# deadskull7/One-Stop-for-COVID-19-Infection-and-Lung-Segmentation-plus-Classification

Measured on AMD Instinct MI355X. Metric: CT images/sec (fwd+bwd) U-Net 512x512x1 bs16, higher is better.
Workload: dtype f32 storage / accumulate / parameters; conv products as a two-term fp16 split (3 fp16 MFMAs per multiply, ~2^-22 per product; --algo 2 = strict fp32); 1 GPU; U-Net infection seg (task1 graph T1:853-916), 512x512x1, batch 16/GPU, fp32, fwd+loss+bwd+Keras-Adam; BASELINE.json configs[1]; storage=fp32, global_batch=16, parallelism=dp1, deterministic=False, bn_fold=2

## Files before the change

### include/unet_hip.h

```cpp
#ifndef UNET_HIP_H
#define UNET_HIP_H
#include <stddef.h>
#include <stdint.h>

#ifdef __cplusplus
extern "C" {
#endif

#define UNET_ABI_VERSION 16

typedef struct unet_ctx unet_ctx;
typedef struct unet_model unet_model;
typedef uint16_t unet_bf16;
enum { UNET_DTYPE_F32 = 0, UNET_DTYPE_BF16 = 1 };

enum { UNET_OK = 0, UNET_E_ARG = -1, UNET_E_HIP = -2, UNET_E_SHAPE = -3, UNET_E_STATE = -4, UNET_E_NODEV = -5 };

enum { UNET_ALGO_AUTO = 0, UNET_ALGO_NAIVE = 1, UNET_ALGO_MFMA = 2 };

int32_t unet_abi_version(void);
int32_t unet_ctx_create(int32_t device_id, unet_ctx** out);
void unet_ctx_destroy(unet_ctx* ctx);
const char* unet_last_error(const unet_ctx* ctx);
int32_t unet_ctx_set_profiling(unet_ctx* ctx, int32_t on);
enum { UNET_OPT_RELU_BITS = 1, UNET_OPT_BN_FOLD = 2, UNET_OPT_ENC_BN_FUSED = 3, UNET_OPT_BN_CONCAT_ANALYTIC = 4, UNET_OPT_BN_FUSE_STATS = 5, UNET_OPT_DETERMINISTIC = 6,
       UNET_OPT_HEAD_FUSED = 7, UNET_OPT_SKIP_RAW = 8, UNET_OPT_POOL_SUMS_FUSED = 9, UNET_OPT_HEAD_BWD_FUSED = 10, UNET_OPT_CONV_PP = 13 };
int32_t unet_ctx_set_option(unet_ctx* ctx, int32_t option, int32_t value);
int32_t unet_ctx_get_option(unet_ctx* ctx, int32_t option);

enum { UNET_ACT_NONE = 0, UNET_ACT_RELU = 1, UNET_ACT_ELU = 2 };
enum { UNET_MASK_NONE = 0, UNET_MASK_RELU = 1, UNET_MASK_ELU = 2, UNET_MASK_ELU_DROP = 3, UNET_MASK_RELU_BITS = 9  };

size_t unet_conv3x3_w_ws_floats(int32_t cin, int32_t cout);
int32_t unet_conv3x3_pick_algo(int32_t algo, int32_t wd, int32_t cin, int32_t cout);
double unet_conv3x3_exec_ratio(int32_t algo, int32_t h, int32_t wd, int32_t cin, int32_t cout);
double unet_conv3x3_wgrad_exec_ratio(int32_t algo, int32_t h, int32_t wd, int32_t cin, int32_t cout);
int32_t unet_request_bn_stats(unet_ctx*, int32_t c);
int32_t unet_relu_bits_supported(int32_t algo, int32_t h, int32_t wd, int32_t cin, int32_t cout);
size_t unet_relu_bits_bytes(int32_t n, int32_t h, int32_t wd, int32_t c);
int32_t unet_request_relu_bits(unet_ctx*, void* bits);
int32_t unet_allow_k_slices(unet_ctx*);
int32_t unet_ctx_max_kernel_scratch_bytes(unet_ctx*);
int32_t unet_conv3x3_fwd(unet_ctx*, const float* x, const float* w, const float* bias, float* y,
                         int32_t n, int32_t h, int32_t wd, int32_t cin, int32_t cout,
                         int32_t act, float drop_rate, uint64_t drop_seed, int32_t algo, float* w_ws, void* stream);
int32_t unet_conv3x3_fwd_ld(unet_ctx*, const float* x, const float* w, const float* bias, float* y, int32_t ldy,
                            int32_t n, int32_t h, int32_t wd, int32_t cin, int32_t cout, int32_t act, int32_t algo, float* w_ws, void* stream);
int32_t unet_conv3x3_bwd_data(unet_ctx*, const float* dy, const float* w, const float* mask_src,
                              int32_t mask_mode, float mask_rate, uint64_t mask_seed,
                              float* dx, float* wt_ws, int32_t n, int32_t h, int32_t wd,
                              int32_t cin, int32_t cout, int32_t algo, void* stream);
int32_t unet_conv3x3_bnfold_supported(int32_t algo, int32_t h, int32_t wd, int32_t cin, int32_t cout);
size_t unet_conv3x3_bnfold_ws_floats(int32_t n, int32_t cin, int32_t cout);
int32_t unet_conv3x3_bnfold_fwd(unet_ctx*, const float* x, const float* bnp, const float* w, const float* bias, float* y, int32_t n, int32_t h,
                                int32_t wd, int32_t cin, int32_t cout, int32_t act, int32_t algo, float* ws, void* stream);
int32_t unet_conv3x3_bnfold_bwd_weights(unet_ctx*, const float* x, const float* bnp, const float* dy, const float* w, float* dw, float* db,
                                        double* bn_bwd_sums, void* gws, size_t gws_bytes, float* ws, int32_t n, int32_t h, int32_t wd,
                                        int32_t cin, int32_t cout, int32_t algo, void* stream);
size_t unet_conv3x3_bwd_weights_ws_bytes(int32_t n, int32_t h, int32_t wd, int32_t cin, int32_t cout);
int32_t unet_conv3x3_bwd_weights(unet_ctx*, const float* x, const float* dy, float* dw, float* db,
                                 void* ws, size_t ws_bytes, int32_t n, int32_t h, int32_t wd,
                                 int32_t cin, int32_t cout, int32_t algo, void* stream);

int32_t unet_convT2x2_fwd(unet_ctx*, const float* x, const float* w, const float* bias, float* y,
                          int32_t ldy, int32_t n, int32_t h, int32_t wd, int32_t cin, int32_t cout,
                          int32_t algo, void* stream);
int32_t unet_convT2x2_bwd_data(unet_ctx*, const float* dy, int32_t lddy, const float* w,
                               const float* relu_src, float* dx, int32_t n, int32_t h, int32_t wd,
                               int32_t cin, int32_t cout, int32_t algo, void* stream);
size_t unet_convT2x2_bwd_weights_ws_bytes(int32_t n, int32_t h, int32_t wd, int32_t cin, int32_t cout);
int32_t unet_convT2x2_bwd_weights(unet_ctx*, const float* x, const float* dy, int32_t lddy,
                                  float* dw, float* db, void* ws, size_t ws_bytes, int32_t n,
                                  int32_t h, int32_t wd, int32_t cin, int32_t cout, int32_t algo,
                                  void* stream);

int32_t unet_bn_stats(unet_ctx*, const float* x, int32_t ldx, double* sums, int64_t pixels,
                      int32_t c, void* stream);
int32_t unet_bn_stats_concat(unet_ctx*, const float* x_up, int32_t ldx, const double* src_sums, double src_count, const float* src_gamma,
                             const float* src_beta, double* sums, int64_t pixels, int32_t c_up, int32_t c_skip, void* stream);
int32_t unet_bn_finalize_train(unet_ctx*, const double* sums, double count, const float* gamma,
                               const float* beta, float* moving_mean, float* moving_var,
                               float* bnp, int32_t c, void* stream);
int32_t unet_bn_finalize_infer(unet_ctx*, const float* gamma, const float* beta,
                               const float* moving_mean, const float* moving_var, float* bnp,
                               int32_t c, void* stream);
int32_t unet_bn_apply(unet_ctx*, const float* x, int32_t ldx, const float* bnp, float* y,
                      int32_t ldy, int64_t pixels, int32_t c, void* stream);
int32_t unet_bn_bwd_stats(unet_ctx*, const float* dy, int32_t lddy, const float* x, int32_t ldx,
                          const float* bnp, double* sums, int64_t pixels, int32_t c, void* stream);
int32_t unet_bn_bwd_param_grads(unet_ctx*, const double* sums, float* dgamma, float* dbeta,
                                int32_t c, void* stream);
int32_t unet_bn_bwd_apply(unet_ctx*, const float* dy, int32_t lddy, const float* x, int32_t ldx,
                          const float* bnp, const double* sums, double count, int32_t mask_mode,
                          float mask_rate, uint64_t mask_seed, float* dx, int32_t lddx, int64_t pixels,
                          int32_t c, void* stream);

int32_t unet_maxpool2x2_dropout_fwd(unet_ctx*, const float* x, int32_t ldx, float* y, int32_t n,
                                    int32_t h, int32_t wd, int32_t c, float rate, uint64_t seed,
                                    void* stream);
int32_t unet_maxpool2x2_dropout_bwd(unet_ctx*, const float* x, int32_t ldx, const float* dy,
                                    float* dx, int32_t lddx, int32_t n, int32_t h, int32_t wd,
                                    int32_t c, float rate, uint64_t seed, int32_t accumulate,
                                    void* stream);

int32_t unet_bn_apply_maxpool_dropout_fwd(unet_ctx*, const float* x, int32_t ldx, const float* bnp, float* y,
                                          int32_t ldy, float* pooled, int32_t n, int32_t h, int32_t wd,
                                          int32_t c, float rate, uint64_t seed, void* stream);
int32_t unet_maxpool2x2_dropout_bwd_bnstats(unet_ctx*, const float* y, int32_t ldy, const float* dy, float* dx,
                                            int32_t lddx, const float* gamma, const float* beta, double* sums,
                                            int32_t n, int32_t h, int32_t wd, int32_t c, float rate,
                                            uint64_t seed, void* stream);
int32_t unet_maxpool2x2_dropout_bwd_sums(unet_ctx*, const float* pooled, const float* dy_pooled, const float* gamma, const float* beta, double* sums,
                                         int32_t n, int32_t h, int32_t wd, int32_t c, float rate, uint64_t seed, void* stream);
int32_t unet_bn_bwd_skip_term(unet_ctx*, double* sums, const double* dec_sum_dyxhat, const float* dec_invstd, const float* dec_gamma,
                              const float* gamma, int32_t c, double frac, void* stream);
int32_t unet_bn_maxpool_bwd_apply(unet_ctx*, const float* x, int32_t ldx, const float* bnp, const double* sums, double count, const float* g_skip,
                                  int32_t ldg, const float* dy_pooled, float* dx, int32_t lddx, int32_t n, int32_t h, int32_t wd, int32_t c,
                                  float rate, uint64_t seed, void* stream);

enum { UNET_LOSS_BCE_DICE = 0, UNET_LOSS_BCE = 1, UNET_LOSS_DICE = 2, UNET_LOSS_TVERSKY = 3, UNET_LOSS_WEIGHTED_BCE_DICE = 4 };
int32_t unet_loss_weight_map(unet_ctx*, const float* y_true, float* weight, int32_t n, int32_t h, int32_t wd, void* stream);
int32_t unet_head_fwd_ex(unet_ctx*, const float* x, const float* w, const float* bias, float* p, const float* y_true, const float* weight_map, double* loss_sums,
                         int64_t pixels, int32_t cin, void* stream);
int32_t unet_head_fwd_bf16_ex(unet_ctx*, const unet_bf16* x, const float* w, const float* bias, float* p, const float* y_true, const float* weight_map,
                              double* loss_sums, int64_t pixels, int32_t cin, void* stream);

int32_t unet_head_fwd(unet_ctx*, const float* x, const float* w, const float* bias, float* p,
                      const float* y_true, double* loss_sums, int64_t pixels, int32_t cin,
                      void* stream);
int32_t unet_loss_finalize(unet_ctx*, const double* loss_sums, double count, float* loss_out,
                           void* stream);
int32_t unet_head_bwd(unet_ctx*, const float* x, const float* w, const float* p, const float* y_true,
                      const double* loss_sums, double count, float* dx, float* dw, float* db,
                      int64_t pixels, int32_t cin, int32_t relu_mask, void* stream);
int32_t unet_loss_finalize_ex(unet_ctx*, const double* loss_sums, double count, int32_t loss, float alpha, float beta, float* loss_out, void* stream);
int32_t unet_head_bwd_ex(unet_ctx*, const float* x, const float* w, const float* p, const float* y_true, const double* loss_sums, double count,
                         int32_t loss, float alpha, float beta, const float* weight_map, float* dx, float* dw, float* db, int64_t pixels, int32_t cin, int32_t relu_mask,
                         void* stream);

int32_t unet_conv3x3_bwd_data_pool_sums_supported(unet_ctx*, int32_t algo, int32_t wd, int32_t cin, int32_t cout);
int32_t unet_conv3x3_bwd_data_pool_sums(unet_ctx*, const float* dy, const float* w, const float* pooled, const float* gamma, const float* beta, float rate,
                                        float* dx, double* sums, float* wt_ws, int32_t n, int32_t h, int32_t wd, int32_t cin, int32_t cout, void* stream);

int32_t unet_conv3x3_head_supported(unet_ctx*, int32_t algo, int32_t w, int32_t cin, int32_t cout);
int32_t unet_conv3x3_head_fwd(unet_ctx*, const float* x, const float* w, const float* bias, float* y, const float* w_head, const float* b_head, float* p,
                              const float* y_true, double* loss_sums, double* head_sums, int32_t n, int32_t h, int32_t wd, int32_t cin, float* w_ws, void* stream);
int32_t unet_head_dy(unet_ctx*, const float* p, const float* y_true, const double* loss_sums, double count, const double* head_sums, const float* w_head,
                     const void* relu_bits, const float* y, float* dy, float* dw_head, float* db_head, int32_t n, int32_t h, int32_t wd, void* stream);
int32_t unet_head_bwd_stream_supported(unet_ctx*, int32_t algo, int32_t wd, int32_t cin);
int32_t unet_head_dzm(unet_ctx*, const float* p, const float* y_true, const double* loss_sums, double count, const double* head_sums, const void* relu_bits, void* dzm,
                      float* dw_head, float* db_head, int32_t n, int32_t h, int32_t wd, void* stream);
int32_t unet_conv3x3_head_fwd_ex(unet_ctx*, const float* x, const float* w, const float* bias, float* y, const float* w_head, const float* b_head, float* p,
                                 const float* y_true, const float* weight_map, double* loss_sums, double* head_sums, int32_t n, int32_t h, int32_t wd, int32_t cin,
                                 float* w_ws, void* stream);
int32_t unet_head_dy_ex(unet_ctx*, const float* p, const float* y_true, const double* loss_sums, double count, const double* head_sums, int32_t loss, float alpha,
                        float beta, const float* weight_map, const float* w_head, const void* relu_bits, const float* y, float* dy, float* dw_head, float* db_head, int32_t n, int32_t h,
                        int32_t wd, void* stream);
int32_t unet_head_dzm_ex(unet_ctx*, const float* p, const float* y_true, const double* loss_sums, double count, const double* head_sums, int32_t loss, float alpha,
                         float beta, const float* weight_map, const void* relu_bits, void* dzm, float* dw_head, float* db_head, int32_t n, int32_t h, int32_t wd, void* stream);
int32_t unet_conv3x3_bwd_data_dzm(unet_ctx*, const void* dzm, const float* w, const float* w_head, const void* relu_bits_in, float* dx, float* wt_ws, int32_t n, int32_t h,
                                  int32_t wd, int32_t cin, void* stream);
int32_t unet_conv3x3_bwd_weights_dzm(unet_ctx*, const float* x, const void* dzm, const float* w_head, float* dw, float* db, void* ws, size_t ws_bytes, int32_t n, int32_t h,
                                     int32_t wd, int32_t cin, void* stream);

int32_t unet_adam_keras(unet_ctx*, float* p, const float* g, float* m, float* v, int64_t count,
                        float lr_t, float b1, float b2, float eps, float grad_scale, void* stream);

int32_t unet_seg_metrics_sweep(unet_ctx*, const float* p, const float* gt, const float* thresholds,
                               int32_t nthr, double* out, int64_t count, void* stream);

int32_t unet_gather_samples(unet_ctx*, const float* src, const int64_t* idx, float* dst, int64_t n,
                            int64_t sample_floats, void* stream);

int32_t unet_augment_samples(unet_ctx*, const float* src_img, const float* src_mask, const int64_t* idx, const float* mats, float* dst_img, float* dst_mask,
                             int64_t n, int32_t h, int32_t w, int32_t c, void* stream);

enum { UNET_FEAT_OUT_F32 = 0, UNET_FEAT_OUT_F64 = 1 };
int32_t unet_feat_col_mean(unet_ctx*, const float* x, int64_t ldx, int64_t n, int64_t d, double* mu, void* stream);
size_t unet_feat_gemm_nt_workspace(int64_t m, int64_t p, int64_t d, int32_t sym);
int32_t unet_feat_gemm_nt(unet_ctx*, const float* a, int64_t lda, const double* mu_a, const float* b, int64_t ldb, const double* mu_b, int64_t m,
                          int64_t p, int64_t d, int32_t sym, void* c, int64_t ldc, int32_t c_dtype, void* ws, size_t ws_bytes, void* stream);
size_t unet_feat_gemm_tn_workspace(int64_t k, int64_t d, int64_t n);
int32_t unet_feat_gemm_tn(unet_ctx*, const float* w, int64_t ldw, const float* x, int64_t ldx, const double* mu, int64_t n, int64_t k, int64_t d,
                          void* out, int64_t ldo, int32_t out_dtype, void* ws, size_t ws_bytes, void* stream);
int32_t unet_kmeans_step(unet_ctx*, const float* pts, int64_t ldp, int64_t n, int64_t p, const double* centres, int32_t k, int32_t* labels,
                         double* dist, double* sums, int64_t* counts, double* inertia, void* stream);
size_t unet_cluster_route_workspace(int64_t n, int64_t d, int32_t k);
int32_t unet_cluster_route(unet_ctx*, const void* tap, int32_t tap_bf16, int64_t n, int32_t h, int32_t w, int32_t c, int64_t ld,
                           const float* comps_hwc, const float* mu_hwc, int32_t k, const double* centres, int32_t nc,
                           float* proj, int32_t* labels, double* dist, void* ws, size_t ws_bytes, void* stream);

int32_t unet_zero(unet_ctx*, void* ptr, size_t bytes, void* stream);
int32_t unet_copy_slice(unet_ctx*, const float* src, int32_t lds, float* dst, int32_t ldd, int64_t pixels, int32_t c, void* stream);
int32_t unet_accum_slices(unet_ctx*, const float* const* srcs, const int32_t* lds, int32_t nsrc, float* dst, int32_t ldd,
                          int64_t pixels, int32_t c, int32_t accumulate, void* stream);

int32_t unet_cast_f32_to_bf16(unet_ctx*, const float* src, unet_bf16* dst, int64_t count, void* stream);
int32_t unet_cast_bf16_to_f32(unet_ctx*, const unet_bf16* src, float* dst, int64_t count, void* stream);
int32_t unet_conv3x3_fwd_bf16(unet_ctx*, const unet_bf16* x, const float* w, const float* bias, unet_bf16* y, int32_t n, int32_t h, int32_t wd,
                              int32_t cin, int32_t cout, int32_t act, float drop_rate, uint64_t drop_seed, void* w_ws, void* stream);
int32_t unet_conv3x3_first_fwd_bf16(unet_ctx*, const float* x, const float* w, const float* bias, unet_bf16* y, int32_t n, int32_t h,
                                    int32_t wd, int32_t cout, int32_t act, float drop_rate, uint64_t drop_seed, void* stream);
int32_t unet_conv3x3_bwd_data_bf16(unet_ctx*, const unet_bf16* dy, const float* w, const unet_bf16* mask_src, int32_t mask_mode, float mask_rate,
                                   uint64_t mask_seed, unet_bf16* dx, void* w_ws, int32_t n, int32_t h, int32_t wd, int32_t cin, int32_t cout,
                                   void* stream);
size_t unet_conv3x3_bwd_weights_ws_bytes_bf16(int32_t n, int32_t h, int32_t wd, int32_t cin, int32_t cout);
int32_t unet_conv3x3_bwd_weights_bf16(unet_ctx*, const unet_bf16* x, const unet_bf16* dy, float* dw, float* db, void* ws, size_t ws_bytes,
                                      int32_t n, int32_t h, int32_t wd, int32_t cin, int32_t cout, void* stream);
int32_t unet_conv3x3_first_bwd_weights_bf16(unet_ctx*, const float* x, const unet_bf16* dy, float* dw, float* db, void* ws, size_t ws_bytes,
                                            int32_t n, int32_t h, int32_t wd, int32_t cout, void* stream);
int32_t unet_convT2x2_fwd_bf16(unet_ctx*, const unet_bf16* x, const float* w, const float* bias, unet_bf16* y, int32_t ldy, int32_t n, int32_t h,
                               int32_t wd, int32_t cin, int32_t cout, void* w_ws, void* stream);
int32_t unet_convT2x2_bwd_data_bf16(unet_ctx*, const unet_bf16* dy, int32_t lddy, const float* w, const unet_bf16* relu_src, unet_bf16* dx,
                                    int32_t n, int32_t h, int32_t wd, int32_t cin, int32_t cout, void* w_ws, void* stream);
size_t unet_convT2x2_bwd_weights_ws_bytes_bf16(int32_t n, int32_t h, int32_t wd, int32_t cin, int32_t cout);
int32_t unet_convT2x2_bwd_weights_bf16(unet_ctx*, const unet_bf16* x, const unet_bf16* dy, int32_t lddy, float* dw, float* db, void* ws,
                                       size_t ws_bytes, int32_t n, int32_t h, int32_t wd, int32_t cin, int32_t cout, void* stream);
int32_t unet_bn_stats_bf16(unet_ctx*, const unet_bf16* x, int32_t ldx, double* sums, int64_t pixels, int32_t c, void* stream);
int32_t unet_bn_stats_concat_bf16(unet_ctx*, const unet_bf16* x_up, int32_t ldx, const double* src_sums, double src_count, const float* src_gamma,
                                  const float* src_beta, double* sums, int64_t pixels, int32_t c_up, int32_t c_skip, void* stream);
int32_t unet_bn_apply_bf16(unet_ctx*, const unet_bf16* x, int32_t ldx, const float* bnp, unet_bf16* y, int32_t ldy, int64_t pixels, int32_t c,
                           void* stream);
int32_t unet_bn_bwd_stats_bf16(unet_ctx*, const unet_bf16* dy, int32_t lddy, const unet_bf16* x, int32_t ldx, const float* bnp, double* sums,
                               int64_t pixels, int32_t c, void* stream);
int32_t unet_bn_bwd_apply_bf16(unet_ctx*, const unet_bf16* dy, int32_t lddy, const unet_bf16* x, int32_t ldx, const float* bnp, const double* sums,
// ... 191 lines not shown
```

### one-stop-for-covid-19-infection-and-lung-segmentation-plus-classification_amd/_lib.py

```python
from __future__ import annotations

import ctypes as C
import os

_HERE = os.path.dirname(os.path.abspath(__file__))
LIB_PATH = os.environ.get("COVIDSEG_AMD_LIB") or os.path.join(_HERE, "libunet_hip.so")
ABI_VERSION = 16
COMM_HANDLE_BYTES, COMM_MAX_WORLD, COMM_MAX_DOUBLES = 64, 8, 2048

ALGO_AUTO, ALGO_NAIVE, ALGO_MFMA = 0, 1, 2
OPTIONS = {"relu_bits": 1, "bn_fold": 2, "enc_bn_fused": 3, "bn_concat_analytic": 4, "bn_fuse_stats": 5, "deterministic": 6, "head_fused": 7, "skip_raw": 8, "pool_sums_fused": 9, "head_bwd_fused": 10, "conv_pp": 13}
ARCH_UNET, ARCH_UNETPP, ARCH_CLASSIFIER = 0, 1, 2
LOSSES = {"bce_dice_loss": 0, "binary_crossentropy": 1, "dice_loss": 2, "tversky_loss": 3, "weighted_bce_dice_loss": 4}
DTYPE_F32, DTYPE_BF16 = 0, 1
ACT_NONE, ACT_RELU, ACT_ELU = 0, 1, 2
MORPH_OPS = {"dilate": 0, "erode": 1, "open": 2, "close": 3}
MORPH_MAX_ITERATIONS = 64
INTENSITY_MAX_EDGES = 63
MASK_NONE, MASK_RELU, MASK_ELU, MASK_ELU_DROP = 0, 1, 2, 3
PROG_FWD_TRAIN, PROG_BWD, PROG_FWD_INFER = 0, 1, 2
SYNC_BN_FWD, SYNC_LOSS, SYNC_BN_BWD, SYNC_GRAD_BUCKET = 0, 1, 2, 3

f32p = C.POINTER(C.c_float)
f64p = C.POINTER(C.c_double)
vp = C.c_void_p
i32, i64, u64, f32, f64, sz = C.c_int32, C.c_int64, C.c_uint64, C.c_float, C.c_double, C.c_size_t


class SyncPoint(C.Structure):
    _fields_ = [("after_op", i32), ("kind", i32), ("ptr", vp), ("count", i64), ("use_op", i32), ("reserved", i32)]


RENDER_MAX_TILES, RENDER_MAX_LAYERS = 64, 4


class RenderTile(C.Structure):
    _fields_ = [("axis", i32), ("index", i32), ("x0", i32), ("y0", i32), ("w", i32), ("h", i32)]


class RenderLayer(C.Structure):
    _fields_ = [("labels", vp), ("palette", vp), ("dtype", i32), ("palette_size", i32), ("fill_alpha", i32), ("outline_alpha", i32)]


_PROTOS = {
    "unet_abi_version": (i32, []),
    "unet_ctx_create": (i32, [i32, C.POINTER(vp)]),
    "unet_ctx_destroy": (None, [vp]),
    "unet_last_error": (C.c_char_p, [vp]),
    "unet_ctx_set_profiling": (i32, [vp, i32]),
    "unet_ctx_set_option": (i32, [vp, i32, i32]),
    "unet_ctx_get_option": (i32, [vp, i32]),
    "unet_conv3x3_w_ws_floats": (sz, [i32, i32]),
    "unet_conv3x3_pick_algo": (i32, [i32, i32, i32, i32]),
    "unet_conv3x3_exec_ratio": (f64, [i32, i32, i32, i32, i32]),
    "unet_conv3x3_wgrad_exec_ratio": (f64, [i32, i32, i32, i32, i32]),
    "unet_request_bn_stats": (i32, [vp, i32]),
    "unet_relu_bits_supported": (i32, [i32, i32, i32, i32, i32]),
    "unet_relu_bits_bytes": (sz, [i32, i32, i32, i32]),
    "unet_request_relu_bits": (i32, [vp, vp]),
    "unet_allow_k_slices": (i32, [vp]),
    "unet_ctx_max_kernel_scratch_bytes": (i32, [vp]),
    "unet_conv3x3_fwd": (i32, [vp, vp, vp, vp, vp, i32, i32, i32, i32, i32, i32, f32, u64, i32, vp, vp]),
    "unet_conv3x3_fwd_ld": (i32, [vp, vp, vp, vp, vp, i32, i32, i32, i32, i32, i32, i32, i32, vp, vp]),
    "unet_conv3x3_bwd_data": (i32, [vp, vp, vp, vp, i32, f32, u64, vp, vp, i32, i32, i32, i32, i32, i32, vp]),
    "unet_conv3x3_bwd_weights_ws_bytes": (sz, [i32, i32, i32, i32, i32]),
    "unet_conv3x3_bwd_weights": (i32, [vp, vp, vp, vp, vp, vp, sz, i32, i32, i32, i32, i32, i32, vp]),
    "unet_convT2x2_fwd": (i32, [vp, vp, vp, vp, vp, i32, i32, i32, i32, i32, i32, i32, vp]),
    "unet_convT2x2_bwd_data": (i32, [vp, vp, i32, vp, vp, vp, i32, i32, i32, i32, i32, i32, vp]),
    "unet_convT2x2_bwd_weights_ws_bytes": (sz, [i32, i32, i32, i32, i32]),
    "unet_convT2x2_bwd_weights": (i32, [vp, vp, vp, i32, vp, vp, vp, sz, i32, i32, i32, i32, i32, i32, vp]),
    "unet_cast_f32_to_bf16": (i32, [vp, vp, vp, i64, vp]),
    "unet_cast_bf16_to_f32": (i32, [vp, vp, vp, i64, vp]),
    "unet_conv3x3_fwd_bf16": (i32, [vp, vp, vp, vp, vp, i32, i32, i32, i32, i32, i32, f32, u64, vp, vp]),
    "unet_conv3x3_first_fwd_bf16": (i32, [vp, vp, vp, vp, vp, i32, i32, i32, i32, i32, f32, u64, vp]),
    "unet_conv3x3_bwd_data_bf16": (i32, [vp, vp, vp, vp, i32, f32, u64, vp, vp, i32, i32, i32, i32, i32, vp]),
    "unet_conv3x3_bwd_weights_ws_bytes_bf16": (sz, [i32, i32, i32, i32, i32]),
    "unet_conv3x3_bwd_weights_bf16": (i32, [vp, vp, vp, vp, vp, vp, sz, i32, i32, i32, i32, i32, vp]),
    "unet_conv3x3_first_bwd_weights_bf16": (i32, [vp, vp, vp, vp, vp, vp, sz, i32, i32, i32, i32, vp]),
    "unet_convT2x2_fwd_bf16": (i32, [vp, vp, vp, vp, vp, i32, i32, i32, i32, i32, i32, vp, vp]),
    "unet_convT2x2_bwd_data_bf16": (i32, [vp, vp, i32, vp, vp, vp, i32, i32, i32, i32, i32, vp, vp]),
    "unet_convT2x2_bwd_weights_ws_bytes_bf16": (sz, [i32, i32, i32, i32, i32]),
    "unet_convT2x2_bwd_weights_bf16": (i32, [vp, vp, vp, i32, vp, vp, vp, sz, i32, i32, i32, i32, i32, vp]),
    "unet_bn_stats": (i32, [vp, vp, i32, vp, i64, i32, vp]),
    "unet_bn_stats_bf16": (i32, [vp, vp, i32, vp, i64, i32, vp]),
    "unet_conv3x3_bnfold_supported": (i32, [i32, i32, i32, i32, i32]),
    "unet_conv3x3_bnfold_ws_floats": (sz, [i32, i32, i32]),
    "unet_conv3x3_bnfold_fwd": (i32, [vp, vp, vp, vp, vp, vp, i32, i32, i32, i32, i32, i32, i32, vp, vp]),
    "unet_conv3x3_bnfold_bwd_weights": (i32, [vp, vp, vp, vp, vp, vp, vp, vp, vp, sz, vp, i32, i32, i32, i32, i32, i32, vp]),
    "unet_bn_stats_concat": (i32, [vp, vp, i32, vp, f64, vp, vp, vp, i64, i32, i32, vp]),
    "unet_bn_stats_concat_bf16": (i32, [vp, vp, i32, vp, f64, vp, vp, vp, i64, i32, i32, vp]),
    "unet_bn_finalize_train": (i32, [vp, vp, f64, vp, vp, vp, vp, vp, i32, vp]),
    "unet_bn_finalize_infer": (i32, [vp, vp, vp, vp, vp, vp, i32, vp]),
    "unet_bn_apply": (i32, [vp, vp, i32, vp, vp, i32, i64, i32, vp]),
    "unet_bn_apply_bf16": (i32, [vp, vp, i32, vp, vp, i32, i64, i32, vp]),
    "unet_bn_bwd_stats": (i32, [vp, vp, i32, vp, i32, vp, vp, i64, i32, vp]),
    "unet_bn_bwd_stats_bf16": (i32, [vp, vp, i32, vp, i32, vp, vp, i64, i32, vp]),
    "unet_bn_bwd_param_grads": (i32, [vp, vp, vp, vp, i32, vp]),
    "unet_bn_bwd_apply": (i32, [vp, vp, i32, vp, i32, vp, vp, f64, i32, f32, u64, vp, i32, i64, i32, vp]),
    "unet_bn_bwd_apply_bf16": (i32, [vp, vp, i32, vp, i32, vp, vp, f64, i32, f32, u64, vp, i32, i64, i32, vp]),
    "unet_maxpool2x2_dropout_fwd": (i32, [vp, vp, i32, vp, i32, i32, i32, i32, f32, u64, vp]),
    "unet_maxpool2x2_dropout_fwd_bf16": (i32, [vp, vp, i32, vp, i32, i32, i32, i32, f32, u64, vp]),
    "unet_maxpool2x2_dropout_bwd": (i32, [vp, vp, i32, vp, vp, i32, i32, i32, i32, i32, f32, u64, i32, vp]),
    "unet_maxpool2x2_dropout_bwd_bf16": (i32, [vp, vp, i32, vp, vp, i32, i32, i32, i32, i32, f32, u64, i32, vp]),
    "unet_bn_apply_maxpool_dropout_fwd": (i32, [vp, vp, i32, vp, vp, i32, vp, i32, i32, i32, i32, f32, u64, vp]),
    "unet_bn_apply_maxpool_dropout_fwd_bf16": (i32, [vp, vp, i32, vp, vp, i32, vp, i32, i32, i32, i32, f32, u64, vp]),
    "unet_maxpool2x2_dropout_bwd_bnstats": (i32, [vp, vp, i32, vp, vp, i32, vp, vp, vp, i32, i32, i32, i32, f32, u64, vp]),
    "unet_maxpool2x2_dropout_bwd_sums": (i32, [vp, vp, vp, vp, vp, vp, i32, i32, i32, i32, f32, u64, vp]),
    "unet_maxpool2x2_dropout_bwd_sums_bf16": (i32, [vp, vp, vp, vp, vp, vp, i32, i32, i32, i32, f32, u64, vp]),
    "unet_bn_maxpool_bwd_apply_bf16": (i32, [vp, vp, i32, vp, vp, f64, vp, i32, vp, vp, i32, i32, i32, i32, i32, f32, u64, vp]),
    "unet_bn_bwd_skip_term": (i32, [vp, vp, vp, vp, vp, vp, i32, f64, vp]),
    "unet_bn_maxpool_bwd_apply": (i32, [vp, vp, i32, vp, vp, f64, vp, i32, vp, vp, i32, i32, i32, i32, i32, f32, u64, vp]),
    "unet_maxpool2x2_dropout_bwd_bnstats_bf16": (i32, [vp, vp, i32, vp, vp, i32, vp, vp, vp, i32, i32, i32, i32, f32, u64, vp]),
    "unet_head_fwd": (i32, [vp, vp, vp, vp, vp, vp, vp, i64, i32, vp]),
    "unet_head_fwd_bf16": (i32, [vp, vp, vp, vp, vp, vp, vp, i64, i32, vp]),
    "unet_loss_finalize": (i32, [vp, vp, f64, vp, vp]),
    "unet_head_bwd": (i32, [vp, vp, vp, vp, vp, vp, f64, vp, vp, vp, i64, i32, i32, vp]),
    "unet_head_bwd_bf16": (i32, [vp, vp, vp, vp, vp, vp, f64, vp, vp, vp, i64, i32, i32, vp]),
    "unet_loss_finalize_ex": (i32, [vp, vp, f64, i32, f32, f32, vp, vp]),
    "unet_head_bwd_ex": (i32, [vp, vp, vp, vp, vp, vp, f64, i32, f32, f32, vp, vp, vp, vp, i64, i32, i32, vp]),
    "unet_head_bwd_bf16_ex": (i32, [vp, vp, vp, vp, vp, vp, f64, i32, f32, f32, vp, vp, vp, vp, i64, i32, i32, vp]),
    "unet_head_fwd_ex": (i32, [vp, vp, vp, vp, vp, vp, vp, vp, i64, i32, vp]),
    "unet_head_fwd_bf16_ex": (i32, [vp, vp, vp, vp, vp, vp, vp, vp, i64, i32, vp]),
    "unet_loss_weight_map": (i32, [vp, vp, vp, i32, i32, i32, vp]),
    "unet_conv3x3_head_fwd_ex": (i32, [vp, vp, vp, vp, vp, vp, vp, vp, vp, vp, vp, vp, i32, i32, i32, i32, vp, vp]),
    "unet_adam_keras": (i32, [vp, vp, vp, vp, vp, i64, f32, f32, f32, f32, f32, vp]),
    "unet_seg_metrics_sweep": (i32, [vp, vp, vp, vp, i32, vp, i64, vp]),
    "unet_gather_samples": (i32, [vp, vp, vp, vp, i64, i64, vp]),
    "unet_augment_samples": (i32, [vp, vp, vp, vp, vp, vp, vp, i64, i32, i32, i32, vp]),
    "unet_feat_col_mean": (i32, [vp, vp, i64, i64, i64, vp, vp]),
    "unet_feat_gemm_nt_workspace": (sz, [i64, i64, i64, i32]),
    "unet_feat_gemm_nt": (i32, [vp, vp, i64, vp, vp, i64, vp, i64, i64, i64, i32, vp, i64, i32, vp, sz, vp]),
    "unet_feat_gemm_tn_workspace": (sz, [i64, i64, i64]),
    "unet_feat_gemm_tn": (i32, [vp, vp, i64, vp, i64, vp, i64, i64, i64, vp, i64, i32, vp, sz, vp]),
    "unet_kmeans_step": (i32, [vp, vp, i64, i64, i64, vp, i32, vp, vp, vp, vp, vp, vp]),
    "unet_cluster_route_workspace": (sz, [i64, i64, i32]),
    "unet_cluster_route": (i32, [vp, vp, i32, i64, i32, i32, i32, i64, vp, vp, i32, vp, i32, vp, vp, vp, vp, sz, vp]),
    "unet_conv3x3_head_supported": (i32, [vp, i32, i32, i32, i32]),
    "unet_conv3x3_head_fwd": (i32, [vp, vp, vp, vp, vp, vp, vp, vp, vp, vp, vp, i32, i32, i32, i32, vp, vp]),
    "unet_conv3x3_bwd_data_pool_sums_supported": (i32, [vp, i32, i32, i32, i32]),
    "unet_conv3x3_bwd_data_pool_sums": (i32, [vp, vp, vp, vp, vp, vp, f32, vp, vp, vp, i32, i32, i32, i32, i32, vp]),
    "unet_head_dy": (i32, [vp, vp, vp, vp, f64, vp, vp, vp, vp, vp, vp, vp, i32, i32, i32, vp]),
    "unet_head_bwd_stream_supported": (i32, [vp, i32, i32, i32]),
    "unet_head_dzm": (i32, [vp, vp, vp, vp, f64, vp, vp, vp, vp, vp, i32, i32, i32, vp]),
    "unet_head_dy_ex": (i32, [vp, vp, vp, vp, f64, vp, i32, f32, f32, vp, vp, vp, vp, vp, vp, vp, i32, i32, i32, vp]),
    "unet_head_dzm_ex": (i32, [vp, vp, vp, vp, f64, vp, i32, f32, f32, vp, vp, vp, vp, vp, i32, i32, i32, vp]),
    "unet_conv3x3_bwd_data_dzm": (i32, [vp, vp, vp, vp, vp, vp, vp, i32, i32, i32, i32, vp]),
    "unet_conv3x3_bwd_weights_dzm": (i32, [vp, vp, vp, vp, vp, vp, vp, sz, i32, i32, i32, i32, vp]),
    "unet_zero": (i32, [vp, vp, sz, vp]),
    "unet_comm_create": (i32, [vp, i32, i32, vp, vp]),
    "unet_comm_connect": (i32, [vp, vp]),
    "unet_comm_set_timeout_ms": (i32, [vp, i32]),
    "unet_comm_allreduce_f64": (i32, [vp, vp, i32, vp]),
    "unet_comm_status": (i32, [vp, vp, vp]),
    "unet_comm_destroy": (None, [vp]),
    "unet_copy_slice": (i32, [vp, vp, i32, vp, i32, i64, i32, vp]),
    "unet_copy_slice_bf16": (i32, [vp, vp, i32, vp, i32, i64, i32, vp]),
    "unet_accum_slices": (i32, [vp, C.POINTER(vp), C.POINTER(i32), i32, vp, i32, i64, i32, i32, vp]),
    "unet_accum_slices_bf16": (i32, [vp, C.POINTER(vp), C.POINTER(i32), i32, vp, i32, i64, i32, i32, vp]),
    "unet_dense_ws_bytes": (sz, [i32, i32, i32]),
    "unet_dense_fwd": (i32, [vp, vp, vp, vp, vp, i32, i32, i32, i32, f32, u64, vp, sz, vp]),
    "unet_dense_fwd_bf16": (i32, [vp, vp, vp, vp, vp, i32, i32, i32, i32, f32, u64, vp, sz, vp]),
    "unet_dense_bwd": (i32, [vp, vp, vp, vp, vp, vp, i32, i32, i32, vp]),
    "unet_dense_bwd_bf16": (i32, [vp, vp, vp, vp, vp, vp, i32, i32, i32, vp]),
    "unet_cls_head_fwd": (i32, [vp, vp, vp, vp, vp, vp, f32, f32, vp, i32, i32, vp]),
    "unet_cls_loss_finalize": (i32, [vp, vp, f64, vp, vp]),
    "unet_cls_head_bwd": (i32, [vp, vp, vp, vp, vp, f32, f32, f64, f32, vp, vp, vp, vp, i32, i32, vp]),
    "unet_pre_minmax_ws_bytes": (sz, [i32]),
    "unet_pre_minmax_to_u8": (i32, [vp, vp, vp, i32, i64, vp, sz, vp]),
    "unet_pre_unit_to_u8": (i32, [vp, vp, vp, i64, vp]),
    "unet_pre_u8_to_unit": (i32, [vp, vp, vp, i64, vp]),
    "unet_pre_clahe_ws_bytes": (sz, [i32, i32, i32]),
    "unet_pre_clahe_u8": (i32, [vp, vp, vp, i32, i32, i32, f32, i32, i32, vp, sz, vp]),
    "unet_pre_resize_u8": (i32, [vp, vp, i32, i32, i32, vp, vp, i32, i32, i32, i32, i32, vp]),
    "unet_pre_contours_u8": (i32, [vp, vp, i32, i32, i32, i32, vp, vp, vp, i32]),
    "unet_vol_slices_ws_bytes": (sz, [i32, i32]),
    "unet_vol_slices_f64": (i32, [vp, vp, i32, i32, i32, i32, i32, f64, f64, i32, i32, i32, vp, vp, vp, vp, vp, vp, sz, vp]),
    "unet_vol_paste_back": (i32, [vp, vp, i32, i32, vp, vp, i32, vp]),
    "unet_vol_unslice": (i32, [vp, vp, i32, f32, i32, i32, i32, i32, i32, vp, vp, vp]),
    "unet_vol_label_ws_bytes": (sz, [i32, i32, i32]),
    "unet_vol_label": (i32, [vp, vp, i32, i32, i32, i32, vp, vp, vp, sz, vp]),
    "unet_vol_component_stats": (i32, [vp, vp, i32, i32, i32, i32, vp, vp]),
    "unet_vol_filter_components": (i32, [vp, vp, vp, i32, i32, i32, i32, i32, i32, vp, vp, vp]),
    "unet_vol_confusion": (i32, [vp, vp, vp, i32, i32, i32, vp, vp]),
    "unet_vol_surface": (i32, [vp, vp, i32, i32, i32, i32, vp, vp, vp]),
    "unet_vol_edt_ws_bytes": (sz, [i32, i32, i32]),
    "unet_vol_edt_sq": (i32, [vp, vp, i32, i32, i32, i32, vp, vp, vp, sz, vp]),
    "unet_vol_sqrt_f64": (i32, [vp, vp, i64, vp]),
    "unet_vol_surface_distances": (i32, [vp, vp, vp, i32, i32, i32, vp, vp, i64, vp, sz, vp]),
    "unet_vol_lesion_overlap": (i32, [vp, vp, i32, vp, i32, i32, i32, i32, vp, vp, vp]),
    "unet_vol_label_planar": (i32, [vp, vp, i32, i32, i32, i32, vp, vp, vp, sz, vp]),
    "unet_vol_morph_ws_bytes": (sz, [i32, i32, i32]),
    "unet_vol_morph": (i32, [vp, vp, i32, i32, i32, i32, i32, i32, i32, i32, vp, vp, vp, sz, vp]),
    "unet_vol_ball": (i32, [vp, vp, i32, i32, i32, f64, i32, vp, vp, vp]),
    "unet_vol_fill_holes_ws_bytes": (sz, [i32, i32, i32]),
    "unet_vol_fill_holes": (i32, [vp, vp, i32, i32, i32, i32, i32, vp, vp, vp, sz, vp]),
    "unet_vol_dihedral": (i32, [vp, vp, i32, i32, i32, vp, vp]),
    "unet_vol_canvas_axpy": (i32, [vp, vp, f32, vp, i64, i32, vp]),
    "unet_vol_canvas_div": (i32, [vp, vp, f32, i64, vp]),
    "unet_vol_unslice_prob": (i32, [vp, vp, i32, i32, i32, i32, i32, i32, vp, vp]),
    "unet_vol_vote_pack": (i32, [vp, vp, i32, i32, vp, i64, vp]),
    "unet_vol_vote_reduce": (i32, [vp, vp, i32, i32, i32, i32, i32, vp, vp, vp, vp, vp, vp, vp]),
    "unet_vol_intensity_bands": (i32, [vp, vp, i32, i32, i32, i32, i32, f64, f64, vp, vp, i32, vp, vp, i32, vp, vp, vp, vp]),
    "unet_vol_intensity_gather": (i32, [vp, vp, i32, i32, i32, i32, i32, f64, f64, vp, vp, i32, vp, vp, vp, i64, vp, vp]),
    "unet_vol_group_moments_ws_bytes": (sz, [i64, i32]),
    "unet_vol_group_moments": (i32, [vp, vp, vp, i32, vp, vp, sz, vp]),
    "unet_vol_side_assign": (i32, [vp, vp, vp, vp, i32, i32, i32, i32, i32, vp, vp, vp]),
    "unet_vol_side_table": (i32, [vp, vp, vp, vp, i32, i32, i32, i32, vp, vp, vp, vp]),
    "unet_vol_project": (i32, [vp, vp, i32, i32, i32, i32, i32, f64, f64, i32, i32, i32, i32, vp, vp, vp, i32, vp, vp]),
    "unet_vol_render": (i32, [vp, vp, i32, i32, i32, i32, i32, f64, f64, vp, f64, f64, vp, i32, i32, i32, vp, i32, vp, i32, vp, i32, i32, vp]),
    "unet_vol_resample_nearest": (i32, [vp, vp, i32, i32, i32, i32, vp, i32, u64, vp, i32, i32, i32, vp]),
    "unet_vol_resample_linear": (i32, [vp, vp, i32, i32, i32, i32, i32, f64, f64, vp, i32, f64, vp, i32, i32, i32, i32, vp]),
    "unet_model_create": (i32, [vp, i32, i32, i32, i32, i32, i32, i32, i32, C.POINTER(vp)]),
    "unet_model_dtype": (i32, [vp]),
    "unet_model_tap_elem_bytes": (i32, [vp, C.c_char_p, i32]),
    "unet_model_destroy": (None, [vp]),
    "unet_model_set_loss_out": (C.c_int32, [vp, vp]),
    "unet_model_param_count": (i64, [vp]),
    "unet_model_state_count": (i64, [vp]),
    "unet_model_workspace_bytes": (sz, [vp, i32]),
    "unet_model_tensor_info": (i32, [vp, C.c_char_p, C.POINTER(i32), C.POINTER(i64), C.POINTER(i64)]),
    "unet_model_bind": (i32, [vp, vp, vp, vp, vp, vp, vp, sz]),
    "unet_model_set_io": (i32, [vp, vp, vp, vp]),
    "unet_model_set_dropout": (i32, [vp, f32, u64]),
    "unet_model_set_class_weights": (i32, [vp, f32, f32]),
    "unet_model_set_loss": (i32, [vp, i32, f32, f32]),
    "unet_model_num_ops": (i32, [vp, i32]),
    "unet_model_sync_points": (i32, [vp, i32, C.POINTER(SyncPoint), i32]),
    "unet_model_run": (i32, [vp, i32, i32, i32, vp]),
# ... 92 lines not shown
```

### one-stop-for-covid-19-infection-and-lung-segmentation-plus-classification_amd/csrc/common.h

```cpp
#pragma once
#include <hip/hip_runtime.h>
#include <stdint.h>
#include <stdio.h>
#include <set>
#include <string>

#include "../../include/unet_hip.h"

constexpr int UNET_BN_SLOTS = 64, UNET_BN_SLOTS_DET = 1024, UNET_BN_SLOT_DOUBLES = 2048;
struct unet_loss_sel { int32_t kind = UNET_LOSS_BCE_DICE; float alpha = 0.5f, beta = 0.5f; };
inline bool unet_loss_sel_ok(const unet_loss_sel& ls, const float* wm = nullptr, bool need_map = true) {
  if (ls.kind < UNET_LOSS_BCE_DICE || ls.kind > UNET_LOSS_WEIGHTED_BCE_DICE) return false;
  if (ls.kind == UNET_LOSS_TVERSKY && !(ls.alpha > 0.0f && ls.beta > 0.0f && ls.alpha < 1e30f && ls.beta < 1e30f)) return false;
  return !need_map || (ls.kind == UNET_LOSS_WEIGHTED_BCE_DICE) == (wm != nullptr);
}
constexpr int UNET_HEAD_SUMS = 100;
struct unet_ctx {
  int device = 0;
  int num_cu = 256;
  int profiling = 0;
  int opt_relu_bits = 1;
  int opt_bn_fold = 2;
  int opt_enc_bn_fused = 1;
  int opt_bn_concat_analytic = 1;
  int opt_bn_fuse_stats = 1;
  int opt_pool_sums_fused = 1;
  int opt_skip_raw = 1;
  int opt_head_fused = 1;
  int opt_head_bwd_fused = 1;
  int opt_conv_pp = 1;
  int opt_deterministic = 0;
  double* bn_slots = nullptr;
  int bn_nslots() const { return opt_deterministic ? UNET_BN_SLOTS_DET : UNET_BN_SLOTS; }
  void* convt_img = nullptr;
  size_t convt_img_bytes = 0;
  int k_slices_ok = 0;
  void* splitk_ws = nullptr;
  size_t splitk_ws_bytes = 0;
  int stats_req_c = 0;
  const void* stats_in_slots = nullptr;
  int stats_in_slots_c = 0;
  bool stats_in_slots_xs = false;
  unsigned long long* signs_req = nullptr;
  const void* signs_done = nullptr;
  std::set<const void*> big_lds_kernels;
  std::set<const void*> noted_kernels;
  int max_scratch_bytes = 0;
  std::string err;
};

#define UNET_FAIL(ctx, code, ...)                         \
  do {                                                    \
    char _b[512];                                         \
    snprintf(_b, sizeof(_b), __VA_ARGS__);                \
    if (ctx) (ctx)->err = _b;                             \
    return (code);                                        \
  } while (0)

#define UNET_CHECK_LAUNCH(ctx, what)                                              \
  do {                                                                            \
    hipError_t _e = hipGetLastError();                                            \
    if (_e != hipSuccess) UNET_FAIL(ctx, UNET_E_HIP, "%s: %s", what, hipGetErrorString(_e)); \
  } while (0)

#define UNET_HIP(ctx, expr)                                                       \
  do {                                                                            \
    hipError_t _e = (expr);                                                       \
    if (_e != hipSuccess) UNET_FAIL(ctx, UNET_E_HIP, "%s: %s", #expr, hipGetErrorString(_e)); \
  } while (0)

static inline int32_t unet_big_lds(unet_ctx* ctx, const void* kernel, size_t bytes, const char* what) {
  if (ctx->big_lds_kernels.count(kernel)) return UNET_OK;
  if (hipFuncSetAttribute(kernel, hipFuncAttributeMaxDynamicSharedMemorySize, (int)bytes) != hipSuccess) UNET_FAIL(ctx, UNET_E_HIP, "%s: cannot reserve %zu bytes of LDS", what, bytes);
  ctx->big_lds_kernels.insert(kernel);
  return UNET_OK;
}
static inline void unet_note_kernel(unet_ctx* ctx, const void* kernel) {
  if (ctx->noted_kernels.count(kernel)) return;
  ctx->noted_kernels.insert(kernel);
  hipFuncAttributes at;
  if (hipFuncGetAttributes(&at, kernel) == hipSuccess && (int)at.localSizeBytes > ctx->max_scratch_bytes) ctx->max_scratch_bytes = (int)at.localSizeBytes;
}
#define UNET_BIG_LDS(ctx, kern, bytes, what) do { int32_t _r = unet_big_lds(ctx, reinterpret_cast<const void*>(kern), bytes, what); if (_r) return _r; } while (0)

static inline hipStream_t as_stream(void* s) { return reinterpret_cast<hipStream_t>(s); }
static inline int64_t cdiv64(int64_t a, int64_t b) { return (a + b - 1) / b; }

__device__ __forceinline__ float wave_sum(float v) {
#pragma unroll
  for (int o = 32; o > 0; o >>= 1) v += __shfl_xor(v, o, 64);
  return v;
}

constexpr int UNET_XW = 4;
__device__ __forceinline__ void xsum_add(double* row, int idx, float t) {
  unsigned long long* acc = reinterpret_cast<unsigned long long*>(row) + (size_t)UNET_XW * idx;
  const int eb = (int)((__float_as_uint(t) >> 23) & 0xFF);
  if (eb == 0) return;
  const int e = eb - 127;
  if (e >= 60) { atomicMax(reinterpret_cast<long long*>(acc + 3), 1LL << 62); return; }
  if (e >= 39) {
    atomicAdd(acc + 3, (unsigned long long)__double2ll_rd((double)t * (1.0 / 65536.0)));
    return;
  }
  const int w = min(max((e - 23 + 80) >> 5, 0), 2);
  const double sc = __longlong_as_double((long long)(1023 + 80 - 32 * w) << 52);
  const long long q = __double2ll_rd((double)t * sc);
  atomicAdd(acc + w, (unsigned long long)(q & 0xFFFFFFFFll));
  atomicAdd(acc + w + 1, (unsigned long long)(q >> 32));
}
__device__ __forceinline__ double xsum_take(double* slots, int idx, int nslots) {
  long long S0 = 0, S1 = 0, S2 = 0, S3 = 0; bool bad = false;
// ... 60 lines not shown
__device__ __forceinline__ __amdgpu_buffer_rsrc_t make_rsrc(const float* base, long long bytes) {
  return __builtin_amdgcn_make_buffer_rsrc(const_cast<float*>(base), 0, (int)bytes, 0x00020000);
}

typedef __bf16 unet_bf16x8 __attribute__((ext_vector_type(8)));
typedef __bf16 unet_bf16x2 __attribute__((ext_vector_type(2)));
typedef float unet_f32x2 __attribute__((ext_vector_type(2)));
typedef float unet_f32x16 __attribute__((ext_vector_type(16)));
__device__ __forceinline__ unsigned pack_bf16x2(float lo, float hi) {
  return __builtin_bit_cast(unsigned, __builtin_convertvector((unet_f32x2){lo, hi}, unet_bf16x2));
}
__device__ __forceinline__ float bf16_lo(unsigned u) { return __uint_as_float(u << 16); }
__device__ __forceinline__ float bf16_hi(unsigned u) { return __uint_as_float(u & 0xFFFF0000u); }
__device__ __forceinline__ float4 ld4(const float* p) { return *reinterpret_cast<const float4*>(p); }
__device__ __forceinline__ void st4(float* p, float4 v) { *reinterpret_cast<float4*>(p) = v; }
__device__ __forceinline__ float4 ld4(const unet_bf16* p) {
  const uint2 u = *reinterpret_cast<const uint2*>(p);
  return make_float4(bf16_lo(u.x), bf16_hi(u.x), bf16_lo(u.y), bf16_hi(u.y));
}
__device__ __forceinline__ void st4(unet_bf16* p, float4 v) { *reinterpret_cast<uint2*>(p) = make_uint2(pack_bf16x2(v.x, v.y), pack_bf16x2(v.z, v.w)); }
__device__ __forceinline__ float ld1(const float* p) { return *p; }
__device__ __forceinline__ float ld1(const unet_bf16* p) { return __uint_as_float((unsigned)*p << 16); }
__device__ __forceinline__ void st1(float* p, float v) { *p = v; }
__device__ __forceinline__ void st1(unet_bf16* p, float v) { *p = (unet_bf16)(pack_bf16x2(v, 0.f) & 0xFFFFu); }

__device__ __forceinline__ uint4 philox4x32(uint64_t ctr, uint64_t seed) {
  uint32_t c0 = (uint32_t)ctr, c1 = (uint32_t)(ctr >> 32), c2 = 0x243F6A88u, c3 = 0x85A308D3u;
  uint32_t k0 = (uint32_t)seed, k1 = (uint32_t)(seed >> 32);
#pragma unroll
  for (int r = 0; r < 10; ++r) {
    uint32_t hi0 = __umulhi(0xD2511F53u, c0), lo0 = 0xD2511F53u * c0;
    uint32_t hi1 = __umulhi(0xCD9E8D57u, c2), lo1 = 0xCD9E8D57u * c2;
    uint32_t n0 = hi1 ^ c1 ^ k0, n1 = lo1, n2 = hi0 ^ c3 ^ k1, n3 = lo0;
    c0 = n0; c1 = n1; c2 = n2; c3 = n3;
    k0 += 0x9E3779B9u; k1 += 0xBB67AE85u;
  }
  return make_uint4(c0, c1, c2, c3);
}
__device__ __forceinline__ float u32_to_unit(uint32_t u) { return (float)(u >> 8) * (1.0f / 16777216.0f); }

__device__ __forceinline__ float4 keep_scale(long long quad_idx, float rate, uint64_t seed) {
  uint4 r = philox4x32((uint64_t)quad_idx, seed);
  float s = 1.0f / (1.0f - rate);
  return make_float4(u32_to_unit(r.x) >= rate ? s : 0.f, u32_to_unit(r.y) >= rate ? s : 0.f,
                     u32_to_unit(r.z) >= rate ? s : 0.f, u32_to_unit(r.w) >= rate ? s : 0.f);
}

enum { ACT_NONE = 0, ACT_RELU = 1, ACT_ELU = 2 };
__device__ __forceinline__ float apply_act(float v, int act) {
  if (act == ACT_RELU) return fmaxf(v, 0.0f);
  if (act == ACT_ELU) return v > 0.0f ? v : expm1f(v);
  return v;
}
enum { MASK_NONE = 0, MASK_RELU = 1, MASK_ELU = 2, MASK_ELU_DROP = 3 };
enum { MASK_BIAS_TAB = 4 };
enum { MASK_BN_BWD = 5 };
enum { MASK_BN_BWD_ELU = 6, MASK_BN_BWD_ELU_DROP = 7 };
enum { MASK_BN_BWD_RELU = 8 };
enum { MASK_RELU_BITS = 9 };
enum { MASK_POOL_SUMS = 10 };
int32_t k_bn_bwd_coef(unet_ctx*, const float* bnp, const double* sums, double count, float* coef, int c, hipStream_t s);
__device__ __forceinline__ float mask_factor(float m, int mode, float ks , float rate) {
  if (mode == MASK_RELU) return m > 0.0f ? 1.0f : 0.0f;
  if (mode == MASK_ELU) return m > 0.0f ? 1.0f : m + 1.0f;
  if (mode == MASK_ELU_DROP) { const float a = m * (1.0f - rate); return ks * (a > 0.0f ? 1.0f : a + 1.0f); }
  return 1.0f;
}

size_t bn_fold_scratch_floats(int cin, int cout);
int32_t k_bn_fold_prepare(unet_ctx*, const float* w, const float* bias, const float* scale, const float* shift, int cin, int cout, float* scratch, hipStream_t s, bool want_scaled = true);
size_t wgrad_bn_fold_scratch_floats(int n, int cout);
bool wgrad_bn_fold_supported(int cout);
int32_t k_wgrad_bn_fold_fix(unet_ctx*, const float* dy, int n, int h, int wd, int cin, int cout, const float* scale, const float* shift, float* dw, const float* db, float* scratch,
                            hipStream_t s, const float* w = nullptr, const float* mean = nullptr, const float* istd = nullptr, double* bn_bwd_sums = nullptr,
                            const float* pre_s = nullptr, const float* pre_t = nullptr,
                            float* dgamma = nullptr, float* dbeta = nullptr);
int32_t k_wgrad_bn_fold_fix_bf16(unet_ctx*, const unet_bf16* dy, int n, int h, int wd, int cin, int cout, const float* scale, const float* shift, float* dw, const float* db,
                                 float* scratch, hipStream_t s, const float* w = nullptr, const float* mean = nullptr, const float* istd = nullptr, double* bn_bwd_sums = nullptr);
constexpr int UNET_PREP_MAX = 36;
bool h2_conv3x3_selected(int algo, int K, int M);
bool pp_conv3x3_selected(const unet_ctx* ctx, int K, int M, int n, int h, int wd, const float* mask, int mask_mode, int act, float rate, int ldy);
int32_t k_conv3x3_pp_fwd(unet_ctx*, const float* x, const void* wimg, const float* bias, const float* mask, int mask_mode, float* y, int ldy, int n, int h, int wd, int K, int M,
                         int act, hipStream_t s, bool vdy = false);
size_t h2_wimg_bytes(int K, int M);
int32_t k_h2_weights(unet_ctx*, const float* w, void* img, int cin, int cout, int flip, hipStream_t s, const float* cs = nullptr);
int32_t k_h2_weights_multi(unet_ctx*, const float* const* w, void* const* img, const int* cin, const int* cout, const int* flip, int count, hipStream_t s);
int32_t k_h2_weights_bound(unet_ctx*, const float* w, const float* cs, void* img, int cin, int cout, hipStream_t s);
int32_t k_h2_prep_multi(unet_ctx*, const float* const* w, const float* const* cs, void* const* img, const int* cin, const int* cout, const int* kind, int count, hipStream_t s);
size_t h2_convT_img_bytes(int cin, int cout);
int32_t k_conv3x3_h2_fwd(unet_ctx*, const float* x, const void* wimg, const float* bias, const float* mask, int mask_mode, float* y, int n, int h, int wd, int K, int M,
                         int act, float rate, uint64_t seed, hipStream_t s, int mask_climit = 1 << 30, int ldy = 0);
int32_t k_slot_fold(unet_ctx*, double* sums, int count, hipStream_t s, bool xs = false);
int32_t k_enc_tail_finish(unet_ctx*, double* sums, const double* dec_sum_dyxhat, const float* dec_invstd, const float* dec_gamma, const float* gamma, float* dgamma, float* dbeta, int c,
                          double frac, hipStream_t s);
bool h2_pool_sums_selected(const unet_ctx* ctx, int algo, int wd, int K, int M);
int32_t k_conv3x3_h2_dgrad_pool_sums(unet_ctx*, const float* dy, const void* wimg, const float* pooled, const float* gamma, const float* beta, float rate, float* dx, double* sums,
                                     int n, int h, int wd, int K, int M, hipStream_t s);
int32_t k_bn_finalize_compose(unet_ctx*, int training, const double* sums, double count, const float* gamma, const float* beta, float* mm, float* mv, float* bnp, int c,
                              const float* enc_bnp, float* comp, hipStream_t s);
int32_t k_loss_finalize(unet_ctx*, const double* loss_sums, double count, float* loss_out, float* loss_out2, hipStream_t s, unet_loss_sel ls = {});
int32_t k_cls_loss_finalize(unet_ctx*, const double* sums, double count, float* out, float* out2, hipStream_t s);
int32_t k_bn_compose(unet_ctx*, const float* bnp_dec, const float* bnp_enc, float* comp, int c, hipStream_t s);
struct h2_head_args { const float* w = nullptr; const float* b = nullptr; float* p = nullptr; const float* t = nullptr; double* slots = nullptr; float aux = 0.0f; const float* wm = nullptr; };
bool h2_conv3x3_head_selected(const unet_ctx* ctx, int algo, int wd, int K, int M);
int32_t k_conv3x3_h2_head_fwd(unet_ctx*, const float* x, const void* wimg, const float* bias, float* y, const float* wh, const float* bh, float* p, const float* t,
                              int n, int h, int wd, int K, hipStream_t s, const float* wm = nullptr);
int32_t k_head_fold(unet_ctx*, double* loss_sums, double* head_sums, hipStream_t s, bool weighted = false);
int32_t k_loss_weight_map(unet_ctx*, const float* y_true, float* weight, int n, int h, int wd, hipStream_t s);
int32_t k_head_dy(unet_ctx*, const float* p, const float* t, const double* loss_sums, double count, const double* head_sums, const float* w, const unsigned long long* bits,
                  const float* y, float* dy, float* dw, float* db, int n, int h, int wd, hipStream_t s, unet_loss_sel ls = {}, const float* wm = nullptr);
int32_t k_bn_maxpool_bwd_apply_k1(unet_ctx*, const float* x, int ldx, const float* bnp, const double* sums, double count, const float* g_skip, int ldg, const float* skip_k1,
                                  const float* dy_pooled, float* dx, int lddx, int n, int h, int wd, int c, float rate, uint64_t seed, hipStream_t s);
bool h2_convT_selected(const unet_ctx* ctx, int algo, int cin, int cout);
int32_t k_convT_h2_fwd(unet_ctx*, const float* x, const float* w, const float* bias, float* y, int ldy, int n, int h, int wd, int cin, int cout, hipStream_t s, const void* prepared = nullptr);
int32_t k_convT_h2_dgrad(unet_ctx*, const float* dy, int lddy, const float* w, const float* mask, float* dx, int n, int h, int wd, int cin, int cout, hipStream_t s, int mask_bits = 0,
                         const void* prepared = nullptr);
bool h2_wgrad_selected(int algo, int cin, int cout);
bool h2_wgrad_c16_selected(int algo, int wd, int cin, int cout);
size_t h2_wgrad_c16_ws_bytes(int n, int h, int wd);
int32_t k_wgrad_c16_gather(unet_ctx*, const float* G, float* dw, float* db, hipStream_t s);
int32_t k_conv3x3_h2_wgrad_c16(unet_ctx*, const float* x, const float* dy, float* dw, float* db, void* ws, size_t ws_bytes, int n, int h, int wd, hipStream_t s);
size_t h2_wgrad_ws_bytes(int n, int h, int wd, int cin, int cout);
int32_t k_conv3x3_h2_wgrad(unet_ctx*, const float* x, const float* dy, float* dw, float* db, void* ws, size_t ws_bytes, int n, int h, int wd, int cin, int cout, hipStream_t s);
int32_t k_head_dzm(unet_ctx*, const float* p, const float* t, const double* loss_sums, double count, const double* head_sums, const unsigned long long* bits, void* dzm, float* dw,
                   float* db, int n, int h, int wd, hipStream_t s, unet_loss_sel ls = {}, const float* wm = nullptr);
bool h2_head_bwd_selected(const unet_ctx* ctx, int algo, int wd, int cin);
int32_t k_conv3x3_h2_dgrad_dzm(unet_ctx*, const void* dzm, const void* wimg, const float* mask, int mask_mode, float* dx, int n, int h, int wd, int M, hipStream_t s);
int32_t k_conv3x3_h2_wgrad_dzm(unet_ctx*, const float* x, const void* dzm, const float* w_head, float* dw, float* db, void* ws, size_t ws_bytes, int n, int h, int wd, int cin,
                               hipStream_t s);
int32_t k_conv3x3_naive_fwd(unet_ctx*, const float* x, const float* w, const float* bias, const float* mask, int mask_mode,
                            float* y, int n, int h, int wd, int cin, int cout, int act, float rate, uint64_t seed, hipStream_t s);
bool c1_relu_bits_supported(int wd, int cout);
int32_t k_conv3x3_c1_fwd_bits(unet_ctx*, const float* x, const float* w, const float* bias, float* y, unsigned long long* signs, int n, int h, int wd, int cout, hipStream_t s);
int32_t k_conv3x3_c1_fwd(unet_ctx*, const float* x, const float* w, const float* bias, float* y, int n, int h,
                         int wd, int cout, int act, float rate, uint64_t seed, hipStream_t s);
size_t c1_wgrad_ws_bytes(int cout);
int32_t k_conv3x3_c1_wgrad(unet_ctx*, const float* x, const float* dy, float* dw, float* db, void* ws, size_t ws_bytes, int n, int h,
                           int wd, int cout, hipStream_t s);
int32_t k_flip_transpose_w3x3(unet_ctx*, const float* w, float* wt, int cin, int cout, hipStream_t s);
int32_t k_conv3x3_naive_wgrad(unet_ctx*, const float* x, const float* dy, float* dw, float* db, int n, int h,
                              int wd, int cin, int cout, hipStream_t s);
int32_t k_convT_naive_fwd(unet_ctx*, const float* x, const float* w, const float* bias, float* y, int ldy, int n,
                          int h, int wd, int cin, int cout, hipStream_t s);
int32_t k_convT_naive_dgrad(unet_ctx*, const float* dy, int lddy, const float* w, const float* mask, float* dx,
                            int n, int h, int wd, int cin, int cout, hipStream_t s);
int32_t k_convT_naive_wgrad(unet_ctx*, const float* x, const float* dy, int lddy, float* dw, float* db, int n,
                            int h, int wd, int cin, int cout, hipStream_t s);
bool mfma_conv3x3_supported(int cin, int cout);
int32_t k_conv3x3_mfma_fwd(unet_ctx*, const float* x, const float* w, const float* bias, const float* mask, int mask_mode,
                           float* y, int n, int h, int wd, int cin, int cout, int act, float rate, uint64_t seed, hipStream_t s);
bool mfma_wgrad_supported(int ca, int cb);
bool mfma_convT_supported(int cin, int cout);
int32_t k_convT_mfma_fwd(unet_ctx*, const float* x, const float* w, const float* bias, float* y, int ldy, int n, int h, int wd,
                         int cin, int cout, hipStream_t s);
int32_t k_convT_mfma_dgrad(unet_ctx*, const float* dy, int lddy, const float* w, const float* mask, float* dx, int n, int h, int wd,
                           int cin, int cout, hipStream_t s);
size_t mfma_convT_wgrad_ws_bytes(int n, int h, int wd, int cin, int cout);
bool h2_convT_wgrad_selected(int algo, int cin, int cout);
size_t h2_convT_wgrad_ws_bytes(int n, int h, int wd, int cin, int cout);
int32_t k_convT_h2_wgrad(unet_ctx*, const float* x, const float* dy, int lddy, float* dw, float* db, void* ws, size_t ws_bytes, int n, int h, int wd, int cin, int cout,
                         hipStream_t s);
int32_t k_convT_mfma_wgrad(unet_ctx*, const float* x, const float* dy, int lddy, float* dw, float* db, void* ws, size_t ws_bytes, int n,
                           int h, int wd, int cin, int cout, hipStream_t s);
size_t mfma_wgrad_ws_bytes(int n, int h, int wd, int cin, int cout);
int32_t k_conv3x3_mfma_wgrad(unet_ctx*, const float* x, const float* dy, float* dw, float* db, void* ws,
                             size_t ws_bytes, int n, int h, int wd, int cin, int cout, hipStream_t s);
bool bf16_conv3x3_supported(int cin, int cout);
bool bf16_convT_supported(int cin, int cout);
bool bf16_wgrad_supported(int ca, int cb);
int32_t k_conv3x3_bf16_fwd(unet_ctx*, const unet_bf16* x, const float* w, const float* bias, const unet_bf16* mask, int mask_mode, unet_bf16* y, int n, int h,
                           int wd, int cin, int cout, int act, float rate, uint64_t seed, unet_bf16* wimg, int flip, hipStream_t s,
                           const unet_bf16* prepared = nullptr);
struct unet_wimg_prep { const float* w; unet_bf16* img; long long tap_stride, sk, sm, total8; int nb, nchunks, flip, m; };
struct unet_wimg_prep_list { unet_wimg_prep item[UNET_PREP_MAX]; int n; };
int32_t k_wimg_multi(unet_ctx*, unet_wimg_prep_list* L, const int* cin, const int* cout, hipStream_t s);
int32_t k_convT_bf16_fwd(unet_ctx*, const unet_bf16* x, const float* w, const float* bias, unet_bf16* y, int ldy, int n, int h, int wd, int cin, int cout,
                         unet_bf16* wimg, hipStream_t s);
int32_t k_convT_bf16_dgrad(unet_ctx*, const unet_bf16* dy, int lddy, const float* w, const unet_bf16* mask, unet_bf16* dx, int n, int h, int wd, int cin,
                           int cout, unet_bf16* wimg, hipStream_t s);
size_t bf16_wgrad_ws_bytes(int n, int h, int wd, int cin, int cout);
size_t bf16_convT_wgrad_ws_bytes(int n, int h, int wd, int cin, int cout);
int32_t k_conv3x3_bf16_wgrad(unet_ctx*, const unet_bf16* x, const unet_bf16* dy, float* dw, float* db, void* ws, size_t ws_bytes, int n, int h, int wd,
                             int cin, int cout, hipStream_t s);
int32_t k_convT_bf16_wgrad(unet_ctx*, const unet_bf16* x, const unet_bf16* dy, int lddy, float* dw, float* db, void* ws, size_t ws_bytes, int n, int h,
                           int wd, int cin, int cout, hipStream_t s);
size_t wgrad_reduce_scratch_floats(int taps, int ca, int cb, int cbias, int nslabs);
int32_t k_wgrad_reduce(unet_ctx*, float* part, int nslabs, int taps, int ca, int cb, int cbias, float* dw, float* db, hipStream_t s);
int32_t k_vol_label(unet_ctx*, const uint8_t* mask, int X, int Y, int Z, int connectivity, int planar, int invert, int32_t* labels, int32_t* n_out, void* ws, size_t ws_bytes,
                    hipStream_t s);
int32_t k_conv3x3_c1_fwd_bf16(unet_ctx*, const float* x, const float* w, const float* bias, unet_bf16* y, int n, int h, int wd, int cout, int act,
                              float rate, uint64_t seed, hipStream_t s);
int32_t k_conv3x3_c1_wgrad_bf16(unet_ctx*, const float* x, const unet_bf16* dy, float* dw, float* db, void* ws, size_t ws_bytes, int n, int h, int wd,
                                int cout, hipStream_t s);
```

### one-stop-for-covid-19-infection-and-lung-segmentation-plus-classification_amd/csrc/kernels_conv_naive.hip

```cpp
#include "common.h"

namespace {
constexpr int TPB = 256;

__global__ __launch_bounds__(TPB) void conv3x3_naive_kernel(const float* __restrict__ x, const float* __restrict__ w,
                                                            const float* __restrict__ bias, const float* __restrict__ mask, int mask_mode,
                                                            float* __restrict__ y, int N, int H, int W, int Cin, int Cout, int act,
                                                            float rate, unsigned long long seed) {
  const long long total = (long long)N * H * W * Cout;
  for (long long idx = (long long)blockIdx.x * TPB + threadIdx.x; idx < total; idx += (long long)gridDim.x * TPB) {
    int co = (int)(idx % Cout); long long pix = idx / Cout;
    int j = (int)(pix % W); long long t = pix / W; int i = (int)(t % H); long long n = t / H;
    float acc = bias ? bias[co] : 0.0f;
    for (int a = 0; a < 3; ++a) {
      int ii = i + a - 1; if (ii < 0 || ii >= H) continue;
      for (int b = 0; b < 3; ++b) {
        int jj = j + b - 1; if (jj < 0 || jj >= W) continue;
        const float* xp = x + ((n * H + ii) * W + jj) * (long long)Cin;
        const float* wp = w + (long long)((a * 3 + b) * Cin) * Cout + co;
        for (int ci = 0; ci < Cin; ++ci) acc = fmaf(xp[ci], wp[(long long)ci * Cout], acc);
      }
    }
    acc = apply_act(acc, act);
    float ks = 1.0f;
// ... 329 lines not shown
}

int32_t k_conv3x3_naive_fwd(unet_ctx* ctx, const float* x, const float* w, const float* bias, const float* mask, int mask_mode, float* y,
                            int n, int h, int wd, int cin, int cout, int act, float rate, uint64_t seed, hipStream_t s) {
  long long total = (long long)n * h * wd * cout;
  if (!mask) mask_mode = MASK_NONE;
  hipLaunchKernelGGL(conv3x3_naive_kernel, dim3(grid_for(total, 1 << 20)), dim3(TPB), 0, s, x, w, bias, mask, mask_mode, y, n, h, wd, cin, cout, act,
                     rate, (unsigned long long)seed);
  UNET_CHECK_LAUNCH(ctx, "conv3x3_naive_fwd"); return UNET_OK;
}

template <typename T>
static int32_t c1_fwd_impl(unet_ctx* ctx, const float* x, const float* w, const float* bias, T* y, int n, int h, int wd,
                         int cout, int act, float rate, uint64_t seed, hipStream_t s) {
  if ((cout & 3) || TPB % (cout / 4) || (long long)n * h * wd >= (1LL << 31)) UNET_FAIL(ctx, UNET_E_SHAPE, "conv3x3_c1: cout=%d / %d x %d x %d pixels unsupported", cout, n, h, wd);
  long long threads = (long long)n * h * wd * (cout / 4);
  if ((wd & 3) == 0) {
    hipLaunchKernelGGL(conv3x3_c1x4_kernel<T>, dim3(grid_for(threads / 4, 4096)), dim3(TPB), 0, s, x, w, bias, y, n, h, wd, cout, act, rate, (unsigned long long)seed);
    UNET_CHECK_LAUNCH(ctx, "conv3x3_c1x4_fwd"); return UNET_OK;
  }
  hipLaunchKernelGGL(conv3x3_c1_kernel<T>, dim3(grid_for(threads / 2 + 1, 2048)), dim3(TPB), 0, s, x, w, bias, y, n, h, wd, cout, act, rate,
                     (unsigned long long)seed);
  UNET_CHECK_LAUNCH(ctx, "conv3x3_c1_fwd"); return UNET_OK;
}
int32_t k_conv3x3_c1_fwd(unet_ctx* ctx, const float* x, const float* w, const float* bias, float* y, int n, int h, int wd, int cout, int act, float rate,
                         uint64_t seed, hipStream_t s) { return c1_fwd_impl(ctx, x, w, bias, y, n, h, wd, cout, act, rate, seed, s); }
bool c1_relu_bits_supported(int wd, int cout) { return cout == 32 && wd >= 8 && (wd & 7) == 0; }
int32_t k_conv3x3_c1_fwd_bits(unet_ctx* ctx, const float* x, const float* w, const float* bias, float* y, unsigned long long* signs, int n, int h, int wd, int cout, hipStream_t s) {
  if (!c1_relu_bits_supported(wd, cout) || !signs || (long long)n * h * wd >= (1LL << 31)) UNET_FAIL(ctx, UNET_E_SHAPE, "conv3x3_c1 + sign bits: cout=%d W=%d unsupported", cout, wd);
  const long long items = (long long)n * ((h + 3) / 4) * (wd / 8);
  hipLaunchKernelGGL(conv3x3_c1_bits_kernel, dim3(grid_for(items * 64, 4096)), dim3(TPB), 0, s, x, w, bias, y, signs, n, h, wd);
  UNET_CHECK_LAUNCH(ctx, "conv3x3_c1_bits_fwd"); return UNET_OK;
}
int32_t k_conv3x3_c1_fwd_bf16(unet_ctx* ctx, const float* x, const float* w, const float* bias, unet_bf16* y, int n, int h, int wd, int cout, int act,
                              float rate, uint64_t seed, hipStream_t s) { return c1_fwd_impl(ctx, x, w, bias, y, n, h, wd, cout, act, rate, seed, s); }

int32_t k_flip_transpose_w3x3(unet_ctx* ctx, const float* w, float* wt, int cin, int cout, hipStream_t s) {
  hipLaunchKernelGGL(flip_transpose_kernel, dim3(grid_for(9LL * cin * cout, 2048)), dim3(TPB), 0, s, w, wt, cin, cout);
  UNET_CHECK_LAUNCH(ctx, "flip_transpose"); return UNET_OK;
}

int32_t k_conv3x3_naive_wgrad(unet_ctx* ctx, const float* x, const float* dy, float* dw, float* db, int n, int h, int wd,
                              int cin, int cout, hipStream_t s) {
  UNET_HIP(ctx, hipMemsetAsync(dw, 0, sizeof(float) * 9 * cin * cout, s));
  UNET_HIP(ctx, hipMemsetAsync(db, 0, sizeof(float) * cout, s));
  long long outs = (long long)(9 * cin + 1) * cout, pixels = (long long)n * h * wd;
  int gx = (int)cdiv64(outs, TPB);
  long long want = (1 << 18) / (outs < 1 ? 1 : outs) + 1;
  int gy = (int)std::min<long long>(std::max<long long>(want, 1), std::max<long long>(pixels / 64, 1));
  hipLaunchKernelGGL(conv3x3_naive_wgrad_kernel, dim3(gx, gy), dim3(TPB), 0, s, x, dy, dw, db, n, h, wd, cin, cout);
  UNET_CHECK_LAUNCH(ctx, "conv3x3_naive_wgrad"); return UNET_OK;
}

int32_t k_convT_naive_fwd(unet_ctx* ctx, const float* x, const float* w, const float* bias, float* y, int ldy, int n, int h,
                          int wd, int cin, int cout, hipStream_t s) {
  long long total = (long long)n * 4 * h * wd * cout;
  hipLaunchKernelGGL(convT_naive_fwd_kernel, dim3(grid_for(total, 1 << 20)), dim3(TPB), 0, s, x, w, bias, y, ldy, n, h, wd, cin, cout);
  UNET_CHECK_LAUNCH(ctx, "convT_naive_fwd"); return UNET_OK;
}

int32_t k_convT_naive_dgrad(unet_ctx* ctx, const float* dy, int lddy, const float* w, const float* mask, float* dx, int n,
                            int h, int wd, int cin, int cout, hipStream_t s) {
  long long total = (long long)n * h * wd * cin;
  dim3 g(grid_for(total, 1 << 20)), b(TPB);
  if (mask) hipLaunchKernelGGL(convT_naive_dgrad_kernel<true>, g, b, 0, s, dy, lddy, w, mask, dx, n, h, wd, cin, cout);
  else hipLaunchKernelGGL(convT_naive_dgrad_kernel<false>, g, b, 0, s, dy, lddy, w, mask, dx, n, h, wd, cin, cout);
  UNET_CHECK_LAUNCH(ctx, "convT_naive_dgrad"); return UNET_OK;
}

int32_t k_convT_naive_wgrad(unet_ctx* ctx, const float* x, const float* dy, int lddy, float* dw, float* db, int n, int h,
                            int wd, int cin, int cout, hipStream_t s) {
  UNET_HIP(ctx, hipMemsetAsync(dw, 0, sizeof(float) * 4 * cin * cout, s));
  UNET_HIP(ctx, hipMemsetAsync(db, 0, sizeof(float) * cout, s));
  long long outs = 4LL * cout * (cin + 1), pixels = (long long)n * h * wd;
  int gx = (int)cdiv64(outs, TPB);
  long long want = (1 << 18) / outs + 1;
  int gy = (int)std::min<long long>(std::max<long long>(want, 1), std::max<long long>(pixels / 64, 1));
  hipLaunchKernelGGL(convT_naive_wgrad_kernel, dim3(gx, gy), dim3(TPB), 0, s, x, dy, lddy, dw, db, n, h, wd, cin, cout);
  UNET_CHECK_LAUNCH(ctx, "convT_naive_wgrad"); return UNET_OK;
}

size_t c1_wgrad_ws_bytes(int cout) { return (size_t)(C1_BLOCKS + 32) * 10 * cout * sizeof(float); }

template <typename T>
static int32_t c1_wgrad_impl(unet_ctx* ctx, const float* x, const T* dy, float* dw, float* db, void* ws, size_t ws_bytes, int n, int h,
                           int wd, int cout, hipStream_t s) {
  if ((cout & 3) || TPB % (cout / 4) || (cout / 4) > 64 || (long long)n * h * wd >= (1LL << 31)) UNET_FAIL(ctx, UNET_E_SHAPE, "conv3x3_c1_wgrad: cout=%d unsupported", cout);
  if (!ws || ws_bytes < c1_wgrad_ws_bytes(cout)) UNET_FAIL(ctx, UNET_E_ARG, "conv3x3_c1_wgrad: workspace too small");
  long long groups = ((long long)n * h * wd * (cout / 4) + TPB - 1) / TPB;
  int blocks = (int)std::min<long long>(C1_BLOCKS, std::max<long long>(groups, 1));
  if ((wd & 3) == 0) hipLaunchKernelGGL((conv3x3_c1_wgrad_kernel<T, true>), dim3(blocks), dim3(TPB), 0, s, x, dy, static_cast<float*>(ws), n, h, wd, cout);
  else hipLaunchKernelGGL((conv3x3_c1_wgrad_kernel<T, false>), dim3(blocks), dim3(TPB), 0, s, x, dy, static_cast<float*>(ws), n, h, wd, cout);
  float* part = static_cast<float*>(ws); float* part2 = part + (size_t)C1_BLOCKS * 10 * cout;
  const int ngroups = (blocks + 31) / 32;
  hipLaunchKernelGGL(reduce_c1_kernel, dim3((10 * cout + 127) / 128, ngroups), dim3(128), 0, s, part, part2, nullptr, blocks, 32, cout, 0);
  hipLaunchKernelGGL(reduce_c1_kernel, dim3((10 * cout + 127) / 128, 1), dim3(128), 0, s, part2, dw, db, ngroups, ngroups, cout, 1);
  UNET_CHECK_LAUNCH(ctx, "conv3x3_c1_wgrad"); return UNET_OK;
}
int32_t k_conv3x3_c1_wgrad(unet_ctx* ctx, const float* x, const float* dy, float* dw, float* db, void* ws, size_t ws_bytes, int n, int h, int wd, int cout,
                           hipStream_t s) { return c1_wgrad_impl(ctx, x, dy, dw, db, ws, ws_bytes, n, h, wd, cout, s); }
int32_t k_conv3x3_c1_wgrad_bf16(unet_ctx* ctx, const float* x, const unet_bf16* dy, float* dw, float* db, void* ws, size_t ws_bytes, int n, int h, int wd,
                                int cout, hipStream_t s) { return c1_wgrad_impl(ctx, x, dy, dw, db, ws, ws_bytes, n, h, wd, cout, s); }
```

### one-stop-for-covid-19-infection-and-lung-segmentation-plus-classification_amd/csrc/kernels_conv_pp.hip

```cpp
#include <type_traits>

#include "common.h"

#ifndef PP_TRACE
#define PP_TRACE 0
#endif
#ifndef PP_MID
#define PP_MID 2
#endif
#ifndef PP_STORE_AUX
#define PP_STORE_AUX 2
#endif
#ifndef PP_EXP
#define PP_EXP 0
#endif
#if PP_TRACE
__device__ unsigned long long pp_trace[256 * 2 * 40 * 12];
#define PP_STAMP(i) do { if (lane == 0 && wave == 0 && it < 40 && blockIdx.x < 256) pp_trace[((blockIdx.x * 2 + half) * 40 + it) * 12 + (i)] = __builtin_readcyclecounter(); } while (0)
extern "C" int32_t unet_debug_pp_trace(unsigned long long* host, int n) { return hipMemcpyFromSymbol(host, HIP_SYMBOL(pp_trace), (size_t)n * 8) == hipSuccess ? 0 : 1; }
#else
#define PP_STAMP(i) do { } while (0)
#endif

namespace {

typedef _Float16 f16x8 __attribute__((ext_vector_type(8)));
typedef unet_f32x16 f32x16;
constexpr int PP_HEADER = 256;

__device__ __forceinline__ float pp_pow2f(int e) { return __uint_as_float((unsigned)(e + 127) << 23); }
__device__ __forceinline__ f16x8 pp_frag(const char* p) { return *reinterpret_cast<const f16x8*>(p); }
__device__ __forceinline__ int pp_cell(int p, int c) { return p * 128 + ((c ^ (p & 7)) << 4); }

template <int KC, bool BITS, bool VDY>
__global__ __launch_bounds__(512, 2) void conv_pp_kernel(const float* __restrict__ x, const unet_bf16* __restrict__ wimg_hdr, const float* __restrict__ bias,
                                                         const float* __restrict__ mask, float* __restrict__ y, int ldy, int N, int H, int W, int act, int mask_mode,
                                                         int tiles_x, int tiles_y, int total_tiles, double* __restrict__ stats, int stats_c,
                                                         unsigned long long* __restrict__ signs, int xs) {
  constexpr int RW = 2, TH = 8, PWD = 34, NPIX = (TH + 2) * PWD, K = 16 * KC, M = 32;
  constexpr int HS = NPIX * 16;
  constexpr int PLANE = 2 * HS, CHUNK = 2 * PLANE + 32;
  constexpr int IN_HALF = KC * CHUNK;
  constexpr int W_BYTES = 9 * 2048, W_ALL = KC * W_BYTES;
  constexpr int PPC = 4 * KC, PPIECES = NPIX * PPC, PL = (PPIECES + 255) / 256;
  static_assert(256 % PPC == 0, "a thread's pieces are the same 16 bytes of 256 / PPC pixels apart");
  extern __shared__ __attribute__((aligned(16))) char smem[];
  const int tid = threadIdx.x & 255, lane = threadIdx.x & 63, l31 = lane & 31, hi = lane >> 5;
  const int wave8 = __builtin_amdgcn_readfirstlane(threadIdx.x >> 6);
  const int half = wave8 >> 2, wave = wave8 & 3;
  char* const s_w = smem;
  char* const s_in = smem + W_ALL + half * IN_HALF;
  char* const s_out = smem + W_ALL + 2 * IN_HALF + wave * 4096;
  float* const s_amax = reinterpret_cast<float*>(smem + W_ALL + 2 * IN_HALF + 4 * 4096) + half * 4;
  float* const s_bias = reinterpret_cast<float*>(smem + W_ALL + 2 * IN_HALF + 4 * 4096) + 8;
  float* const s_stat = s_bias + 32;
  float* const s_tab = s_stat + 8 * 2 * 32;

  const int per = gridDim.x >> 3, xcd = blockIdx.x & 7, j = blockIdx.x >> 3;
  const int tpx = (total_tiles + 7) >> 3;
  const int t_beg = xcd * tpx, t_end = min(t_beg + tpx, total_tiles);
  const int slots = 2 * per, iters = (tpx + slots - 1) / slots;
  const int t0 = t_beg + j * 2 + half;

  const int pc = tid % PPC, pix0 = tid / PPC;
  const int dst0 = (pc >> 2) * CHUNK + ((pc & 3) >> 1) * HS + pix0 * 16 + (pc & 1) * 8;
  int rel[PL];
#pragma unroll
  for (int k = 0; k < PL; ++k) {
    const int pix = pix0 + k * (256 / PPC), r = pix / PWD, col = pix - r * PWD;
    rel[k] = pix < NPIX ? (VDY ? (r * W + col) * 8 : ((r * W + col) * K + pc * 4) * 4) : UNET_OOB;
  }
  constexpr int XPP = VDY ? 2 : K;
  const long long lead = (long long)(W + 1) * XPP;
  const __amdgpu_buffer_rsrc_t rs_x = make_rsrc(x - lead, ((long long)N * H * W * XPP + lead) * 4);
  const __amdgpu_buffer_rsrc_t rs_y = make_rsrc(y, (((long long)N * H * W - 1) * ldy + M) * 4);
  const int st_lane = ((lane >> 3) * ldy + (lane & 7) * 4) * 4;

  unet_u32x4 pregA[PL];
  struct pos { int n, y0, x0; };
  auto tile_pos = [&](int t) __attribute__((always_inline)) {
    pos p; const int tx = t % tiles_x; const int t2 = t / tiles_x;
    const int ty = t2 % tiles_y; p.n = t2 / tiles_y; p.x0 = tx * 32; p.y0 = ty * TH;
    return p;
  };
  const int d_x = (slots % tiles_x) * 32, d_y = ((slots / tiles_x) % tiles_y) * TH, d_n = slots / (tiles_x * tiles_y);
  auto advance = [&](pos p) __attribute__((always_inline)) {
    p.x0 += d_x; if (p.x0 >= tiles_x * 32) { p.x0 -= tiles_x * 32; p.y0 += TH; }
    p.y0 += d_y; if (p.y0 >= tiles_y * TH) { p.y0 -= tiles_y * TH; p.n += 1; }
    p.n += d_n;
    return p;
  };
  auto issue_loads = [&](pos p, unet_u32x4 (&preg)[PL]) __attribute__((always_inline)) {
    const int soff = (((p.n * H + p.y0) * W + p.x0) * XPP) * 4;
    int off[PL];
    if (p.y0 > 0 && p.y0 + TH < H && p.x0 > 0 && p.x0 + 32 < W) {
#pragma unroll
      for (int k = 0; k < PL; ++k) off[k] = rel[k];
    } else {
#pragma unroll
      for (int k = 0; k < PL; ++k) {
        const int pix = pix0 + k * (256 / PPC), r = pix / PWD, col = pix - r * PWD;
        const bool ok = (unsigned)(p.y0 - 1 + r) < (unsigned)H && (unsigned)(p.x0 - 1 + col) < (unsigned)W;
        off[k] = ok ? rel[k] : UNET_OOB;
      }
    }
#pragma unroll
    for (int k = 0; k < PL; ++k) {
      asm volatile("" : "+v"(off[k]));
      if (VDY) { const unet_u32x2 v = __builtin_amdgcn_raw_buffer_load_b64(rs_x, off[k], soff, 0); preg[k][0] = v[0]; preg[k][1] = v[1]; }
      else preg[k] = __builtin_amdgcn_raw_buffer_load_b128(rs_x, off[k], soff, 0);
    }
  };

  {
    const __amdgpu_buffer_rsrc_t rs_w = __builtin_amdgcn_make_buffer_rsrc(const_cast<unet_bf16*>(wimg_hdr), 0, PP_HEADER + W_ALL, 0x00020000);
    constexpr int WP = W_ALL / 16;
#pragma unroll
    for (int k = 0; k < (WP + 511) / 512; ++k) {
      const int idx = (int)threadIdx.x + k * 512;
      const unet_u32x4 v = __builtin_amdgcn_raw_buffer_load_b128(rs_w, idx < WP ? PP_HEADER + idx * 16 : UNET_OOB, 0, 0);
      if (idx < WP) *reinterpret_cast<unet_u32x4*>(s_w + idx * 16) = v;
    }
    if (threadIdx.x < 32) s_bias[threadIdx.x] = bias ? bias[threadIdx.x] : 0.f;
    if (!BITS && mask_mode == MASK_BIAS_TAB) s_tab[threadIdx.x] = mask[threadIdx.x];
  }
  const float w_unscale = *reinterpret_cast<const float*>(wimg_hdr);
  pos p_prev = {0, 0, 0}, p_cur = tile_pos(t0), p_next = advance(p_cur);
  if (t0 < t_end) issue_loads(p_cur, pregA);
  __syncthreads();
  if (half) { __builtin_amdgcn_s_barrier(); __builtin_amdgcn_s_barrier(); }

  f32x16 acc[RW];
#pragma unroll
  for (int r = 0; r < RW; ++r)
#pragma unroll
    for (int i = 0; i < 16; ++i) acc[r][i] = 0.f;
  float vprev[RW][16];
  float4 st1 = make_float4(0.f, 0.f, 0.f, 0.f), st2 = st1;
  int e_prev = 0, e_cur = 0;
  constexpr bool bits_mask = BITS;
  const bool tab_mask = !BITS && mask_mode == MASK_BIAS_TAB;
  unsigned mpre[BITS ? RW : 1][4];
  const __amdgpu_buffer_rsrc_t rs_m = make_rsrc(mask, BITS ? (long long)N * H * (W >> 3) * 32 : 0);
  float4 t4s[4];
  int sg_lo = 0, sg_hi = 0;

  auto eslice = [&](const int sl) __attribute__((always_inline)) {
    const int pn = p_prev.n, py0 = p_prev.y0, px0 = p_prev.x0;
    const int r = sl < 9 ? 0 : 1, q = sl - r * 9;
    const int py = py0 + wave * RW + r;
    if (py >= H) return;
    if (q == 0) {
#pragma unroll
      for (int qq = 0; qq < 4; ++qq)
        *reinterpret_cast<float4*>(s_out + pp_cell(l31, hi * 4 + qq)) = make_float4(vprev[r][qq * 4], vprev[r][qq * 4 + 1], vprev[r][qq * 4 + 2], vprev[r][qq * 4 + 3]);
    } else if (q == 1) {
#pragma unroll
      for (int jj = 0; jj < 4; ++jj) t4s[jj] = *reinterpret_cast<const float4*>(s_out + pp_cell(jj * 8 + (lane >> 3), lane & 7));
    }
    if (q >= 2 && (q & 1) == 0) {
      const int jj = (q - 2) >> 1;
      const int pxj = px0 + jj * 8 + (lane >> 3);
      const float4 t4 = t4s[jj];
      if (signs) {
        const unsigned long long b[4] = {__builtin_amdgcn_ballot_w64(t4.x > 0.f), __builtin_amdgcn_ballot_w64(t4.y > 0.f), __builtin_amdgcn_ballot_w64(t4.z > 0.f), __builtin_amdgcn_ballot_w64(t4.w > 0.f)};
#pragma unroll
        for (int k = 0; k < 4; ++k) {
          unet_writelane(sg_lo, (unsigned)b[k], jj * 4 + k);
          unet_writelane(sg_hi, (unsigned)(b[k] >> 32), jj * 4 + k);
        }
        if (jj == 3) {
          const int cells = min(4, (W - px0) >> 3);
          if (lane < 4 * cells)
            signs[(((long long)pn * H + py) * (W >> 3) + (px0 >> 3)) * 4 + lane] = ((unsigned long long)(unsigned)sg_hi << 32) | (unsigned)sg_lo;
        }
      }
      const bool ok = pxj < W;
      const int row_off = (((pn * H + py) * W + px0 + jj * 8) * ldy) * 4;
      __builtin_amdgcn_raw_buffer_store_b128(__builtin_bit_cast(unet_u32x4, t4), rs_y, ok ? st_lane : UNET_OOB, row_off, PP_STORE_AUX);
      if (stats) {
        const float kf = ok ? 1.f : 0.f;
        st1.x = fmaf(kf, t4.x, st1.x); st1.y = fmaf(kf, t4.y, st1.y); st1.z = fmaf(kf, t4.z, st1.z); st1.w = fmaf(kf, t4.w, st1.w);
        const float ux = kf * t4.x, uy = kf * t4.y, uz = kf * t4.z, uw = kf * t4.w;
        st2.x = fmaf(ux, t4.x, st2.x); st2.y = fmaf(uy, t4.y, st2.y); st2.z = fmaf(uz, t4.z, st2.z); st2.w = fmaf(uw, t4.w, st2.w);
      }
    }
  };

  auto mphase = [&](auto HC_, auto HP_, const int it) __attribute__((always_inline)) {
    constexpr bool HC = decltype(HC_)::value, HP = decltype(HP_)::value;
    f16x8 px[2][RW + 2], wf[2][2];
    auto ld_row = [&](int ch, int kx, int rr) __attribute__((always_inline)) {
#pragma unroll
      for (int p = 0; p < 2; ++p) px[p][rr] = pp_frag(s_in + ch * CHUNK + p * PLANE + hi * HS + ((wave * RW + rr) * PWD + l31 + kx) * 16);
    };
    auto ld_w = [&](int s_) __attribute__((always_inline)) {
      const int ch = s_ / 9, kx = (s_ / 3) % 3, ky = s_ % 3;
#pragma unroll
      for (int p = 0; p < 2; ++p) wf[s_ & 1][p] = pp_frag(s_w + ch * W_BYTES + (((ky * 3 + kx) * 2 + p) * 2 + hi) * 512 + l31 * 16);
    };
    if (HC) {
#pragma unroll
      for (int r = 0; r < RW; ++r)
#pragma unroll
        for (int i = 0; i < 16; ++i) acc[r][i] = 0.f;
      ld_row(0, 0, 0); ld_row(0, 0, 1); ld_w(0);
    }
#pragma unroll
    for (int s_ = 0; s_ < 9 * KC; ++s_) {
      if (HC) {
        const int ky = s_ % 3;
        if (s_ + 1 < 9 * KC) {
          const int s1 = s_ + 1, ch1 = s1 / 9, kx1 = (s1 / 3) % 3, ky1 = s1 % 3;
          ld_w(s1);
          if (ky1 == 0) { ld_row(ch1, kx1, 0); ld_row(ch1, kx1, 1); }
          else ld_row(ch1, kx1, ky1 + 1);
        }
#pragma unroll
        for (int pr = 0; pr < 3; ++pr) {
          constexpr int PW[3] = {0, 1, 0}, PX[3] = {1, 0, 0};
#pragma unroll
          for (int r = 0; r < RW; ++r) acc[r] = __builtin_amdgcn_mfma_f32_32x32x16_f16(wf[s_ & 1][PW[pr]], px[PX[pr]][r + ky], acc[r], 0, 0, 0);
        }
      }
      if (HP) eslice(s_ * 18 / (9 * KC));
      __builtin_amdgcn_sched_barrier(0);
      if (s_ == PP_MID) {
        PP_STAMP(7);
        __builtin_amdgcn_s_barrier();
        PP_STAMP(8);
        __builtin_amdgcn_sched_barrier(0);
      }
    }
  };

  auto body = [&](const int it, unet_u32x4 (&preg)[PL]) __attribute__((always_inline)) {
    const int t_cur = t0 + it * slots, t_next = t_cur + slots, t_prev = t_cur - slots;
    const bool have_cur = it < iters && t_cur < t_end, have_next = it + 1 < iters && t_next < t_end, have_prev = it >= 1 && t_prev < t_end;
    auto output_values = [&]() __attribute__((always_inline)) {
    {
        const int py0 = p_prev.y0, px0 = p_prev.x0;
        const float unscale = pp_pow2f(-e_prev) * w_unscale;
        const int px_ = px0 + l31;
        const bool border = tab_mask && (py0 == 0 || py0 + TH >= H || px0 == 0 || px0 + 32 >= W);
        float bv[16];
#pragma unroll
        for (int q = 0; q < 4; ++q) {
          const float4 b4 = *reinterpret_cast<const float4*>(s_bias + hi * 16 + q * 4);
          bv[q * 4] = b4.x; bv[q * 4 + 1] = b4.y; bv[q * 4 + 2] = b4.z; bv[q * 4 + 3] = b4.w;
        }
#pragma unroll
        for (int r = 0; r < RW; ++r) {
          const int py = py0 + wave * RW + r;
          if (border && (py == 0 || py == H - 1 || px_ == 0 || px_ == W - 1)) {
            const int cls = (((py == 0) | ((py == H - 1) << 1)) << 2) | ((px_ == 0) | ((px_ == W - 1) << 1));
            const float* tb = s_tab + cls * M + hi * 16;
#pragma unroll
            for (int q = 0; q < 4; ++q) {
              const float4 b4 = *reinterpret_cast<const float4*>(tb + q * 4);
              vprev[r][q * 4] = fmaf(acc[r][q * 4], unscale, b4.x); vprev[r][q * 4 + 1] = fmaf(acc[r][q * 4 + 1], unscale, b4.y);
              vprev[r][q * 4 + 2] = fmaf(acc[r][q * 4 + 2], unscale, b4.z); vprev[r][q * 4 + 3] = fmaf(acc[r][q * 4 + 3], unscale, b4.w);
            }
          } else {
#pragma unroll
            for (int i = 0; i < 16; ++i) vprev[r][i] = fmaf(acc[r][i], unscale, bv[i]);
          }
          if (act == ACT_RELU) {
#pragma unroll
            for (int i = 0; i < 16; ++i) vprev[r][i] = fmaxf(vprev[r][i], 0.f);
          }
          if (bits_mask) {
            const unsigned sh = (l31 & 3) * 8 + hi * 4;
#pragma unroll
            for (int qq = 0; qq < 4; ++qq)
#pragma unroll
              for (int k = 0; k < 4; ++k) vprev[r][qq * 4 + k] = __uint_as_float(__float_as_uint(vprev[r][qq * 4 + k]) & (unsigned)__builtin_amdgcn_sbfe((int)mpre[BITS ? r : 0][k], sh + qq, 1u));
          }
        }
      }
    };
    PP_STAMP(0);
    if (have_cur) {
      float mx = 0.f;
#pragma unroll
      for (int k = 0; k < PL; ++k) {
        if (VDY) { mx = fmaxf(mx, preg[k][1] ? fabsf(__uint_as_float(preg[k][0])) : 0.f); continue; }
        asm("v_max3_f32 %0, |%1|, |%2|, %0" : "+v"(mx) : "v"(preg[k][0]), "v"(preg[k][1]));
        asm("v_max3_f32 %0, |%1|, |%2|, %0" : "+v"(mx) : "v"(preg[k][2]), "v"(preg[k][3]));
      }
      mx = wave_max_nonneg(mx);
      if (lane == 0) s_amax[wave] = mx;
    }
    asm volatile("s_waitcnt lgkmcnt(0)" ::: "memory");
    PP_STAMP(1);
    __builtin_amdgcn_s_barrier();
    PP_STAMP(2);
    if (BITS && have_prev) output_values();
    if (have_cur) {
      const float4 m4 = *reinterpret_cast<const float4*>(s_amax);
      const float mx = fmaxf(fmaxf(m4.x, m4.y), fmaxf(m4.z, m4.w));
      const int eb = __builtin_amdgcn_readfirstlane((int)((__float_as_uint(mx) >> 23) & 0xFF));
      e_cur = min(138 - eb, 120);
      const float sc = pp_pow2f(e_cur);
#pragma unroll
      for (int k = 0; k < PL; ++k) {
        if (pix0 + k * (256 / PPC) < NPIX) {
          unsigned h0, m0, h1, m1;
          if (VDY) {
            unsigned hh, mm;
            split2_scaled(__uint_as_float(preg[k][0]), __uint_as_float(preg[k][0]), sc, hh, mm);
            const unsigned nib = preg[k][1] >> (pc * 4);
            const unsigned k01 = h2_pair_mask(nib, 0), k23 = h2_pair_mask(nib, 2);
            h0 = hh & k01; h1 = hh & k23; m0 = mm & k01; m1 = mm & k23;
          } else {
          split2_scaled(__uint_as_float(preg[k][0]), __uint_as_float(preg[k][1]), sc, h0, m0);
          split2_scaled(__uint_as_float(preg[k][2]), __uint_as_float(preg[k][3]), sc, h1, m1);
          }
          *reinterpret_cast<uint2*>(s_in + dst0 + k * (256 / PPC) * 16) = make_uint2(h0, h1);
          *reinterpret_cast<uint2*>(s_in + dst0 + k * (256 / PPC) * 16 + PLANE) = make_uint2(m0, m1);
        }
      }
    }
    PP_STAMP(3);
    if (bits_mask && have_cur) {
#pragma unroll
      for (int r = 0; r < RW; ++r) {
        const int py = p_cur.y0 + wave * RW + r;
        const bool ok = py < H && p_cur.x0 + (l31 & ~7) < W;
        const int mo = ok ? (((p_cur.n * H + py) * (W >> 3) + (p_cur.x0 >> 3) + (l31 >> 3)) * 32 + ((l31 >> 2) & 1) * 4) : UNET_OOB;
#pragma unroll
        for (int k = 0; k < 4; ++k) mpre[BITS ? r : 0][k] = __builtin_amdgcn_raw_buffer_load_b32(rs_m, mo, k * 8, 0);
      }
    }
    __builtin_amdgcn_sched_barrier(0);
    if (have_next && (PP_EXP & 2) == 0) issue_loads(p_next, preg);
    __builtin_amdgcn_sched_barrier(0);
    PP_STAMP(4);
    if (!BITS && have_prev) output_values();
    asm volatile("s_waitcnt lgkmcnt(0)" ::: "memory");
    PP_STAMP(5);
    __builtin_amdgcn_s_barrier();
    PP_STAMP(6);
    __builtin_amdgcn_sched_barrier(0);
    if (have_cur && have_prev) mphase(std::true_type{}, std::true_type{}, it);
    else if (have_cur) mphase(std::true_type{}, std::false_type{}, it);
    else if (have_prev) mphase(std::false_type{}, std::true_type{}, it);
    else { PP_STAMP(7); __builtin_amdgcn_s_barrier(); PP_STAMP(8); }
    asm volatile("s_waitcnt lgkmcnt(0)" ::: "memory");
    __builtin_amdgcn_sched_barrier(0);
    PP_STAMP(9);
    __builtin_amdgcn_s_barrier();
    PP_STAMP(10);
    e_prev = e_cur; p_prev = p_cur; p_cur = p_next; p_next = advance(p_next);
  };
  for (int it = 0; it <= iters; ++it) body(it, pregA);
  if (!half) { __builtin_amdgcn_s_barrier(); __builtin_amdgcn_s_barrier(); }

  if (stats) {
    float sv[8] = {st1.x, st1.y, st1.z, st1.w, st2.x, st2.y, st2.z, st2.w};
#pragma unroll
    for (int i = 0; i < 8; ++i) { sv[i] += __shfl_xor(sv[i], 8); sv[i] += __shfl_xor(sv[i], 16); sv[i] += __shfl_xor(sv[i], 32); }
    if (lane < 8) {
#pragma unroll
      for (int i = 0; i < 4; ++i) { s_stat[(wave8 * 2 + 0) * 32 + lane * 4 + i] = sv[i]; s_stat[(wave8 * 2 + 1) * 32 + lane * 4 + i] = sv[4 + i]; }
    }
    __syncthreads();
    if (threadIdx.x < 64) {
      const int kind = threadIdx.x >> 5, c32 = threadIdx.x & 31;
      float t = 0.f;
#pragma unroll
      for (int wv = 0; wv < 8; ++wv) t += s_stat[(wv * 2 + kind) * 32 + c32];
      double* const row = stats + (size_t)(blockIdx.x % UNET_BN_SLOTS) * UNET_BN_SLOT_DOUBLES;
      if (xs) xsum_add(row, (kind ? stats_c : 0) + c32, t); else atomicAdd(row + (kind ? stats_c : 0) + c32, (double)t);
    }
  }
}

}

bool pp_conv3x3_selected(const unet_ctx* ctx, int K, int M, int n, int h, int wd, const float* mask, int mask_mode, int act, float rate, int ldy) {
  if (!ctx || !ctx->opt_conv_pp) return false;
  if (K != 32 || M != 32 || rate != 0.0f || (act != ACT_NONE && act != ACT_RELU)) return false;
  if (mask && mask_mode != MASK_BIAS_TAB && mask_mode != MASK_RELU_BITS) return false;
  if (mask && mask_mode == MASK_RELU_BITS && (wd & 7)) return false;
  if (ldy < M || (ldy & 3)) return false;
  const long long tiles = (long long)((wd + 31) / 32) * ((h + 7) / 8) * n;
  if (tiles < 4LL * 2 * ctx->num_cu && ctx->opt_conv_pp < 2) return false;
  if ((long long)n * h * wd * K * 4 + (long long)(wd + 1) * K * 4 >= (1LL << 31)) return false;
  if ((long long)n * h * wd * ldy * 4 >= (1LL << 31)) return false;
  return true;
}

int32_t k_conv3x3_pp_fwd(unet_ctx* ctx, const float* x, const void* wimg, const float* bias, const float* mask, int mask_mode, float* y, int ldy, int n, int h, int wd, int K, int M,
                         int act, hipStream_t s, bool vdy) {
  if (K != 32 || M != 32) UNET_FAIL(ctx, UNET_E_SHAPE, "conv pp: K=%d M=%d", K, M);
  constexpr int KC = 2;
  ctx->k_slices_ok = 0;
  if (!mask) mask_mode = MASK_NONE;
  const int tiles_x = (wd + 31) / 32, tiles_y = (h + 7) / 8;
  const long long total = (long long)tiles_x * tiles_y * n;
  double* stats = nullptr; int stats_c = 0;
  if (ctx->stats_req_c > 0) {
    const int c = ctx->stats_req_c; ctx->stats_req_c = 0;
    const int xw = ctx->opt_deterministic ? UNET_XW : 1;
    if ((mask_mode == MASK_NONE || mask_mode == MASK_BIAS_TAB) && 2 * c * xw <= UNET_BN_SLOT_DOUBLES && c == M && ctx->bn_slots) {
      stats = ctx->bn_slots; stats_c = c; ctx->stats_in_slots = y; ctx->stats_in_slots_c = c; ctx->stats_in_slots_xs = ctx->opt_deterministic != 0;
    }
  }
  unsigned long long* signs = nullptr;
  if (ctx->signs_req) {
    unsigned long long* q = ctx->signs_req; ctx->signs_req = nullptr;
    if (act == ACT_RELU && (mask_mode == MASK_NONE || mask_mode == MASK_BIAS_TAB) && !(wd & 7)) { signs = q; ctx->signs_done = q; }
  }
  constexpr int NPIX = 340, CHUNK = 4 * NPIX * 16 + 32;
  constexpr size_t smem = (size_t)KC * 9 * 2048 + 2 * (size_t)KC * CHUNK + 4 * 4096 + 32 + 128 + 8 * 2 * 32 * 4 + 16 * 32 * 4;
  if (vdy && (stats || signs || bias || act != ACT_NONE || mask_mode == MASK_BIAS_TAB)) UNET_FAIL(ctx, UNET_E_ARG, "conv pp behind the head's {dz, mask} stream: a plain data-gradient launch only");
  auto kern = vdy ? (mask_mode == MASK_RELU_BITS ? conv_pp_kernel<KC, true, true> : conv_pp_kernel<KC, false, true>)
                  : (mask_mode == MASK_RELU_BITS ? conv_pp_kernel<KC, true, false> : conv_pp_kernel<KC, false, false>);
  UNET_BIG_LDS(ctx, kern, smem, "conv_pp");
  unet_note_kernel(ctx, reinterpret_cast<const void*>(kern));
  const unsigned grid = (unsigned)(ctx->num_cu & ~7);
  hipLaunchKernelGGL(kern, dim3(grid), dim3(512), smem, s, x, static_cast<const unet_bf16*>(wimg), bias, mask, y, ldy, n, h, wd, act, mask_mode, tiles_x, tiles_y, (int)total, stats,
                     stats_c, signs, ctx->opt_deterministic ? 1 : 0);
  UNET_CHECK_LAUNCH(ctx, "conv_pp");
  return UNET_OK;
}
```

### one-stop-for-covid-19-infection-and-lung-segmentation-plus-classification_amd/csrc/model.hip

```cpp
#include <algorithm>
#include <functional>
#include <map>
#include <set>
#include <string>
#include <vector>

#include "common.h"

extern "C" {

int32_t unet_abi_version(void) { return UNET_ABI_VERSION; }

int32_t unet_ctx_create(int32_t device_id, unet_ctx** out) {
  if (!out) return UNET_E_ARG;
  *out = nullptr;
  int ndev = 0;
  if (hipGetDeviceCount(&ndev) != hipSuccess || ndev <= 0 || device_id < 0 || device_id >= ndev) return UNET_E_NODEV;
  hipDeviceProp_t prop;
  if (hipGetDeviceProperties(&prop, device_id) != hipSuccess) return UNET_E_NODEV;
  if (std::string(prop.gcnArchName).rfind("gfx950", 0) != 0) return UNET_E_NODEV;
  unet_ctx* c = new unet_ctx();
  c->device = device_id;
  c->num_cu = prop.multiProcessorCount;
  const size_t sb = sizeof(double) * UNET_BN_SLOTS_DET * UNET_BN_SLOT_DOUBLES;
  int prev = 0;
  (void)hipGetDevice(&prev);
  if (hipSetDevice(device_id) != hipSuccess || hipMalloc(reinterpret_cast<void**>(&c->bn_slots), sb) != hipSuccess ||
      hipMemset(c->bn_slots, 0, sb) != hipSuccess) { (void)hipSetDevice(prev); delete c; return UNET_E_HIP; }
  c->convt_img_bytes = (size_t)8 << 20;
  if (hipMalloc(&c->convt_img, c->convt_img_bytes) != hipSuccess) { c->convt_img = nullptr; c->convt_img_bytes = 0; }
  c->splitk_ws_bytes = (size_t)32 << 20;
  if (hipMalloc(&c->splitk_ws, c->splitk_ws_bytes) != hipSuccess) { c->splitk_ws = nullptr; c->splitk_ws_bytes = 0; }
  (void)hipSetDevice(prev);
  *out = c;
  return UNET_OK;
}

void unet_ctx_destroy(unet_ctx* ctx) {
  if (ctx && ctx->bn_slots) (void)hipFree(ctx->bn_slots);
  if (ctx && ctx->convt_img) (void)hipFree(ctx->convt_img);
  if (ctx && ctx->splitk_ws) (void)hipFree(ctx->splitk_ws);
  delete ctx;
}
const char* unet_last_error(const unet_ctx* ctx) { return ctx ? ctx->err.c_str() : "null ctx"; }
int32_t unet_ctx_set_profiling(unet_ctx* ctx, int32_t on) { if (!ctx) return UNET_E_ARG; ctx->profiling = on; return UNET_OK; }

static int* ctx_option(unet_ctx* ctx, int32_t option) {
  switch (option) {
    case UNET_OPT_RELU_BITS: return &ctx->opt_relu_bits;
    case UNET_OPT_BN_FOLD: return &ctx->opt_bn_fold;
    case UNET_OPT_ENC_BN_FUSED: return &ctx->opt_enc_bn_fused;
    case UNET_OPT_BN_CONCAT_ANALYTIC: return &ctx->opt_bn_concat_analytic;
    case UNET_OPT_BN_FUSE_STATS: return &ctx->opt_bn_fuse_stats;
    case UNET_OPT_DETERMINISTIC: return &ctx->opt_deterministic;
    case UNET_OPT_HEAD_FUSED: return &ctx->opt_head_fused;
    case UNET_OPT_SKIP_RAW: return &ctx->opt_skip_raw;
    case UNET_OPT_POOL_SUMS_FUSED: return &ctx->opt_pool_sums_fused;
    case UNET_OPT_HEAD_BWD_FUSED: return &ctx->opt_head_bwd_fused;
    case UNET_OPT_CONV_PP: return &ctx->opt_conv_pp;
    default: return nullptr;
  }
}
int32_t unet_ctx_set_option(unet_ctx* ctx, int32_t option, int32_t value) {
  if (!ctx) return UNET_E_ARG;
  int* p = ctx_option(ctx, option);
  const int hi = option == UNET_OPT_BN_FOLD ? 3 : option == UNET_OPT_CONV_PP ? 2 : 1;
  if (!p || value < 0 || value > hi) UNET_FAIL(ctx, UNET_E_ARG, "ctx_set_option: option %d value %d", option, value);
  *p = value;
  return UNET_OK;
}
int32_t unet_ctx_get_option(unet_ctx* ctx, int32_t option) {
  if (!ctx) return UNET_E_ARG;
  const int* p = ctx_option(ctx, option);
  if (!p) UNET_FAIL(ctx, UNET_E_ARG, "ctx_get_option: unknown option %d", option);
  return *p;
}

}

static bool use_mfma(int algo, int cin, int cout) {
  if (algo == UNET_ALGO_NAIVE) return false;
  return mfma_conv3x3_supported(cin, cout);
}
static bool use_h2(int algo, int cin, int cout, const void* uws) { return uws && h2_conv3x3_selected(algo, cin, cout); }

static int32_t conv3x3_fwd_dispatch(unet_ctx* ctx, const float* x, const float* w, const float* bias, const float* mask, int mask_mode,
                                    float* y, int n, int h, int wd, int cin, int cout, int act, float rate, uint64_t seed, int algo,
                                    hipStream_t s, float* uws = nullptr, int flip = 0, const float* prepared = nullptr, int ldy = 0) {
  if (ldy && ldy != cout && !(use_h2(algo, cin, cout, uws) && prepared)) UNET_FAIL(ctx, UNET_E_STATE, "conv3x3: a strided output (ldy %d) exists on the h2 kernels with a prepared image only", ldy);
  if (use_h2(algo, cin, cout, uws)) {
    if (prepared) return k_conv3x3_h2_fwd(ctx, x, prepared, bias, mask, mask_mode, y, n, h, wd, cin, cout, act, rate, seed, s, 1 << 30, ldy);
    int32_t r = flip ? k_h2_weights(ctx, w, uws, cout, cin, 1, s) : k_h2_weights(ctx, w, uws, cin, cout, 0, s);
    if (r) return r;
    return k_conv3x3_h2_fwd(ctx, x, uws, bias, mask, mask_mode, y, n, h, wd, cin, cout, act, rate, seed, s);
  }
  if (mask_mode >= MASK_BIAS_TAB) UNET_FAIL(ctx, UNET_E_STATE, "conv3x3: the folded-BatchNorm / bit-mask epilogues exist on the h2 kernels only (cin=%d cout=%d algo=%d)", cin, cout, algo);
  if (flip) {
    if (!uws) UNET_FAIL(ctx, UNET_E_ARG, "conv3x3 data gradient: needs the weight scratch");
    int32_t r = k_flip_transpose_w3x3(ctx, w, uws, cout, cin, s);
    if (r) return r;
    w = uws;
  }
  if (use_mfma(algo, cin, cout)) return k_conv3x3_mfma_fwd(ctx, x, w, bias, mask, mask_mode, y, n, h, wd, cin, cout, act, rate, seed, s);
  if (cin == 1 && !mask && algo != UNET_ALGO_NAIVE && (cout % 4) == 0 && 256 % (cout / 4) == 0) {
    if (ctx->signs_req && act == ACT_RELU && rate == 0.0f && c1_relu_bits_supported(wd, cout)) {
      unsigned long long* q = ctx->signs_req; ctx->signs_req = nullptr;
      int32_t r = k_conv3x3_c1_fwd_bits(ctx, x, w, bias, y, q, n, h, wd, cout, s);
      if (!r) ctx->signs_done = q;
      return r;
    }
    return k_conv3x3_c1_fwd(ctx, x, w, bias, y, n, h, wd, cout, act, rate, seed, s);
  }
  return k_conv3x3_naive_fwd(ctx, x, w, bias, mask, mask_mode, y, n, h, wd, cin, cout, act, rate, seed, s);
}

static int32_t conv3x3_wgrad_dispatch(unet_ctx* ctx, const float* x, const float* dy, float* dw, float* db, void* ws,
                                      size_t ws_bytes, int n, int h, int wd, int cin, int cout, int algo, hipStream_t s) {
  if (algo != UNET_ALGO_NAIVE && mfma_wgrad_supported(cin, cout) && ws && ws_bytes >= mfma_wgrad_ws_bytes(n, h, wd, cin, cout)) {
    if (h2_wgrad_c16_selected(algo, wd, cin, cout) && ws_bytes >= h2_wgrad_c16_ws_bytes(n, h, wd))
      return k_conv3x3_h2_wgrad_c16(ctx, x, dy, dw, db, ws, ws_bytes, n, h, wd, s);
    if (h2_wgrad_selected(algo, cin, cout) && ws_bytes >= h2_wgrad_ws_bytes(n, h, wd, cin, cout))
      return k_conv3x3_h2_wgrad(ctx, x, dy, dw, db, ws, ws_bytes, n, h, wd, cin, cout, s);
    return k_conv3x3_mfma_wgrad(ctx, x, dy, dw, db, ws, ws_bytes, n, h, wd, cin, cout, s);
  }
  if (cin == 1 && algo != UNET_ALGO_NAIVE && (cout % 4) == 0 && 256 % (cout / 4) == 0 && cout <= 256 && ws && ws_bytes >= c1_wgrad_ws_bytes(cout))
    return k_conv3x3_c1_wgrad(ctx, x, dy, dw, db, ws, ws_bytes, n, h, wd, cout, s);
  return k_conv3x3_naive_wgrad(ctx, x, dy, dw, db, n, h, wd, cin, cout, s);
}

extern "C" {

int32_t unet_request_bn_stats(unet_ctx* ctx, int32_t c) {
  if (!ctx || c < 0) UNET_FAIL(ctx, UNET_E_ARG, "request_bn_stats: bad args");
  ctx->stats_req_c = ctx->opt_bn_fuse_stats ? c : 0;
  return UNET_OK;
}

int32_t unet_relu_bits_supported(int32_t algo, int32_t h, int32_t wd, int32_t cin, int32_t cout) {
  if (cin < 1 || cout < 1 || (cout & 31) || (wd & 7) || h < 1) return 0;
  if (cin == 1) return algo == UNET_ALGO_AUTO && c1_relu_bits_supported(wd, cout) ? 1 : 0;
  return h2_conv3x3_selected(algo, cin, cout) ? 1 : 0;
}
// ... 50 lines not shown
  ctx->signs_req = nullptr;
  if (!r && armed && ctx->signs_done != armed) UNET_FAIL(ctx, UNET_E_SHAPE, "conv3x3_head_fwd: armed with unet_request_relu_bits but the launch did not write them");
  if (!r && y_true) r = k_head_fold(ctx, loss_sums, head_sums, as_stream(stream), weight_map != nullptr);
  return r;
}
int32_t unet_conv3x3_head_fwd(unet_ctx* ctx, const float* x, const float* w, const float* bias, float* y, const float* w_head, const float* b_head, float* p, const float* y_true,
                              double* loss_sums, double* head_sums, int32_t n, int32_t h, int32_t wd, int32_t cin, float* w_ws, void* stream) {
  return unet_conv3x3_head_fwd_ex(ctx, x, w, bias, y, w_head, b_head, p, y_true, nullptr, loss_sums, head_sums, n, h, wd, cin, w_ws, stream);
}
int32_t unet_head_bwd_stream_supported(unet_ctx* ctx, int32_t algo, int32_t wd, int32_t cin) {
  return ctx && cin == 32 && h2_head_bwd_selected(ctx, algo, wd, cin) && h2_wgrad_selected(algo, cin, 32) ? 1 : 0;
}
int32_t unet_head_dzm(unet_ctx* ctx, const float* p, const float* y_true, const double* loss_sums, double count, const double* head_sums, const void* relu_bits, void* dzm,
                      float* dw_head, float* db_head, int32_t n, int32_t h, int32_t wd, void* stream) {
  if (!ctx) return UNET_E_ARG;
  return k_head_dzm(ctx, p, y_true, loss_sums, count, head_sums, static_cast<const unsigned long long*>(relu_bits), dzm, dw_head, db_head, n, h, wd, as_stream(stream));
}
int32_t unet_head_dzm_ex(unet_ctx* ctx, const float* p, const float* y_true, const double* loss_sums, double count, const double* head_sums, int32_t loss, float alpha,
                         float beta, const float* weight_map, const void* relu_bits, void* dzm, float* dw_head, float* db_head, int32_t n, int32_t h, int32_t wd, void* stream) {
  if (!ctx) return UNET_E_ARG;
  return k_head_dzm(ctx, p, y_true, loss_sums, count, head_sums, static_cast<const unsigned long long*>(relu_bits), dzm, dw_head, db_head, n, h, wd, as_stream(stream),
                    unet_loss_sel{loss, alpha, beta}, weight_map);
}
int32_t unet_conv3x3_bwd_data_dzm(unet_ctx* ctx, const void* dzm, const float* w, const float* w_head, const void* relu_bits_in, float* dx, float* wt_ws, int32_t n, int32_t h,
                                  int32_t wd, int32_t cin, void* stream) {
  if (!ctx || !dzm || !w || !w_head || !dx || !wt_ws || n < 1 || h < 1 || wd < 1) UNET_FAIL(ctx, UNET_E_ARG, "conv3x3_bwd_data_dzm: bad args");
  if (!unet_head_bwd_stream_supported(ctx, UNET_ALGO_AUTO, wd, cin)) UNET_FAIL(ctx, UNET_E_SHAPE, "conv3x3_bwd_data_dzm: not supported here (unet_head_bwd_stream_supported)");
  int32_t r = k_h2_weights(ctx, w, wt_ws, cin, 32, 1, as_stream(stream), w_head);
  if (!r) r = k_conv3x3_h2_dgrad_dzm(ctx, dzm, wt_ws, static_cast<const float*>(relu_bits_in), relu_bits_in ? MASK_RELU_BITS : MASK_NONE, dx, n, h, wd, cin, as_stream(stream));
  ctx->k_slices_ok = 0;
  return r;
}
int32_t unet_conv3x3_bwd_weights_dzm(unet_ctx* ctx, const float* x, const void* dzm, const float* w_head, float* dw, float* db, void* ws, size_t ws_bytes, int32_t n, int32_t h,
                                     int32_t wd, int32_t cin, void* stream) {
  if (!ctx || !x || !dzm || !w_head || !dw || !db || n < 1 || h < 1 || wd < 1) UNET_FAIL(ctx, UNET_E_ARG, "conv3x3_bwd_weights_dzm: bad args");
  if (!unet_head_bwd_stream_supported(ctx, UNET_ALGO_AUTO, wd, cin)) UNET_FAIL(ctx, UNET_E_SHAPE, "conv3x3_bwd_weights_dzm: not supported here (unet_head_bwd_stream_supported)");
  return k_conv3x3_h2_wgrad_dzm(ctx, x, dzm, w_head, dw, db, ws, ws_bytes, n, h, wd, cin, as_stream(stream));
}
int32_t unet_head_dy(unet_ctx* ctx, const float* p, const float* y_true, const double* loss_sums, double count, const double* head_sums, const float* w_head, const void* relu_bits,
                     const float* y, float* dy, float* dw_head, float* db_head, int32_t n, int32_t h, int32_t wd, void* stream) {
  if (!ctx) return UNET_E_ARG;
  return k_head_dy(ctx, p, y_true, loss_sums, count, head_sums, w_head, static_cast<const unsigned long long*>(relu_bits), y, dy, dw_head, db_head, n, h, wd, as_stream(stream));
}
int32_t unet_head_dy_ex(unet_ctx* ctx, const float* p, const float* y_true, const double* loss_sums, double count, const double* head_sums, int32_t loss, float alpha,
                        float beta, const float* weight_map, const float* w_head, const void* relu_bits, const float* y, float* dy, float* dw_head, float* db_head,
                        int32_t n, int32_t h, int32_t wd, void* stream) {
  if (!ctx) return UNET_E_ARG;
  return k_head_dy(ctx, p, y_true, loss_sums, count, head_sums, w_head, static_cast<const unsigned long long*>(relu_bits), y, dy, dw_head, db_head, n, h, wd, as_stream(stream),
                   unet_loss_sel{loss, alpha, beta}, weight_map);
}

int32_t unet_conv3x3_pick_algo(int32_t algo, int32_t wd, int32_t cin, int32_t cout) {
  (void)wd;
  if (h2_conv3x3_selected(algo, cin, cout)) return UNET_ALGO_AUTO;
  if (algo != UNET_ALGO_NAIVE && mfma_conv3x3_supported(cin, cout)) return UNET_ALGO_MFMA;
  return UNET_ALGO_NAIVE;
}

double unet_conv3x3_exec_ratio(int32_t algo, int32_t h, int32_t wd, int32_t cin, int32_t cout) {
  (void)h; (void)wd;
  return h2_conv3x3_selected(algo, cin, cout) ? 3.0 * 157.3 / 2500.0 : 1.0;
}

double unet_conv3x3_wgrad_exec_ratio(int32_t algo, int32_t h, int32_t wd, int32_t cin, int32_t cout) {
  (void)h; (void)wd;
  if (algo == UNET_ALGO_NAIVE || !mfma_wgrad_supported(cin, cout)) return 1.0;
  return h2_wgrad_selected(algo, cin, cout) ? 3.0 * 157.3 / 2500.0 : 1.0;
}

size_t unet_conv3x3_w_ws_floats(int32_t cin, int32_t cout) { return cin > 0 && cout > 0 ? (size_t)16 * std::max(cin, 32) * std::max(cout, 32) + 64 : 0; }

int32_t unet_conv3x3_bwd_data(unet_ctx* ctx, const float* dy, const float* w, const float* mask_src, int32_t mask_mode, float mask_rate,
                              uint64_t mask_seed, float* dx, float* wt_ws, int32_t n, int32_t h, int32_t wd, int32_t cin, int32_t cout,
                              int32_t algo, void* stream) {
  if (!ctx || !dy || !w || !dx || !wt_ws || n < 1 || h < 1 || wd < 1 || cin < 1 || cout < 1 || mask_mode < 0 || (mask_mode > 3 && mask_mode != MASK_RELU_BITS) ||
      (mask_mode != MASK_NONE && !mask_src) || mask_rate < 0 || mask_rate >= 1)
    UNET_FAIL(ctx, UNET_E_ARG, "conv3x3_bwd_data: bad args");
  if (mask_mode == MASK_RELU_BITS && !unet_relu_bits_supported(algo, h, wd, cout, cin))
    UNET_FAIL(ctx, UNET_E_SHAPE, "conv3x3_bwd_data: no bit-mask form for h=%d w=%d cin=%d cout=%d algo=%d (unet_relu_bits_supported(algo, h, w, cout, cin))", h, wd, cin, cout, algo);
  const int32_t r = conv3x3_fwd_dispatch(ctx, dy, w, nullptr, mask_src, mask_mode, dx, n, h, wd, cout, cin, ACT_NONE, mask_rate, mask_seed, algo,
                                         as_stream(stream), wt_ws, 1);
  ctx->k_slices_ok = 0;
  return r;
}

int32_t unet_conv3x3_bwd_data_pool_sums_supported(unet_ctx* ctx, int32_t algo, int32_t wd, int32_t cin, int32_t cout) { return ctx && h2_pool_sums_selected(ctx, algo, wd, cout, cin) ? 1 : 0; }
int32_t unet_conv3x3_bwd_data_pool_sums(unet_ctx* ctx, const float* dy, const float* w, const float* pooled, const float* gamma, const float* beta, float rate, float* dx, double* sums,
                                        float* wt_ws, int32_t n, int32_t h, int32_t wd, int32_t cin, int32_t cout, void* stream) {
  if (!ctx || !dy || !w || !pooled || !gamma || !beta || !dx || !sums || !wt_ws || n < 1 || h < 1 || wd < 1) UNET_FAIL(ctx, UNET_E_ARG, "conv3x3_bwd_data_pool_sums: bad args");
  if (!h2_pool_sums_selected(ctx, UNET_ALGO_AUTO, wd, cout, cin)) UNET_FAIL(ctx, UNET_E_SHAPE, "conv3x3_bwd_data_pool_sums: not supported here (unet_conv3x3_bwd_data_pool_sums_supported)");
  int32_t r = k_h2_weights(ctx, w, wt_ws, cin, cout, 1, as_stream(stream));
  if (r) return r;
  return k_conv3x3_h2_dgrad_pool_sums(ctx, dy, wt_ws, pooled, gamma, beta, rate, dx, sums, n, h, wd, cout, cin, as_stream(stream));
}

int32_t unet_conv3x3_bnfold_supported(int32_t algo, int32_t h, int32_t wd, int32_t cin, int32_t cout) {
  return (h >= 1 && wd >= 1 && cin >= 1 && cout >= 1 && h2_conv3x3_selected(algo, cin, cout) && (cout % 16) == 0 && wgrad_bn_fold_supported(cout)) ? 1 : 0;
}
size_t unet_conv3x3_bnfold_ws_floats(int32_t n, int32_t cin, int32_t cout) {
  if (n < 1 || cin < 1 || cout < 1) return 0;
  return bn_fold_scratch_floats(cin, cout) + unet_conv3x3_w_ws_floats(cin, cout) + wgrad_bn_fold_scratch_floats(n, cout);
}
int32_t unet_conv3x3_bnfold_fwd(unet_ctx* ctx, const float* x, const float* bnp, const float* w, const float* bias, float* y, int32_t n, int32_t h, int32_t wd,
                                int32_t cin, int32_t cout, int32_t act, int32_t algo, float* ws, void* stream) {
  if (!ctx || !x || !bnp || !w || !y || !ws || n < 1 || act < 0 || act > ACT_RELU) UNET_FAIL(ctx, UNET_E_ARG, "conv3x3_bnfold_fwd: bad args");
  if (!unet_conv3x3_bnfold_supported(algo, h, wd, cin, cout)) UNET_FAIL(ctx, UNET_E_SHAPE, "conv3x3_bnfold_fwd: no folded form for h=%d w=%d cin=%d cout=%d (unet_conv3x3_bnfold_supported)", h, wd, cin, cout);
  hipStream_t s = as_stream(stream);
  float* u = ws + bn_fold_scratch_floats(cin, cout);
  int32_t r = k_bn_fold_prepare(ctx, w, bias, bnp, bnp + cin, cin, cout, ws, s, false);
  if (r) return r;
  r = k_h2_weights(ctx, w, u, cin, cout, 0, s, bnp);
  if (r) return r;
  const float* tab = ws + (size_t)9 * cin * cout;
  r = k_conv3x3_h2_fwd(ctx, x, u, tab, tab, MASK_BIAS_TAB, y, n, h, wd, cin, cout, act, 0.0f, 0, s);
  ctx->k_slices_ok = 0;
  return r;
}
int32_t unet_conv3x3_bnfold_bwd_weights(unet_ctx* ctx, const float* x, const float* bnp, const float* dy, const float* w, float* dw, float* db, double* bn_bwd_sums, void* gws,
                                        size_t gws_bytes, float* ws, int32_t n, int32_t h, int32_t wd, int32_t cin, int32_t cout, int32_t algo, void* stream) {
  if (!ctx || !x || !bnp || !dy || !dw || !db || !ws || n < 1 || h < 1 || wd < 1 || cin < 1) UNET_FAIL(ctx, UNET_E_ARG, "conv3x3_bnfold_bwd_weights: bad args");
  if (!wgrad_bn_fold_supported(cout)) UNET_FAIL(ctx, UNET_E_SHAPE, "conv3x3_bnfold_bwd_weights: cout=%d (needs a divisor of 256)", cout);
  hipStream_t s = as_stream(stream);
  int32_t r = conv3x3_wgrad_dispatch(ctx, x, dy, dw, db, gws, gws_bytes, n, h, wd, cin, cout, algo, s);
  if (r) return r;
  if (bn_bwd_sums && !w) UNET_FAIL(ctx, UNET_E_ARG, "conv3x3_bnfold_bwd_weights: bn_bwd_sums needs the kernel w");
  return k_wgrad_bn_fold_fix(ctx, dy, n, h, wd, cin, cout, bnp, bnp + cin, dw, db, ws + bn_fold_scratch_floats(cin, cout) + unet_conv3x3_w_ws_floats(cin, cout), s,
                             bn_bwd_sums ? w : nullptr, bn_bwd_sums ? bnp + 2 * cin : nullptr, bn_bwd_sums ? bnp + 3 * cin : nullptr, bn_bwd_sums);
}

size_t unet_conv3x3_bwd_weights_ws_bytes(int32_t n, int32_t h, int32_t wd, int32_t cin, int32_t cout) {
  if (cin == 1 && (cout % 4) == 0 && 256 % (cout / 4) == 0 && cout <= 256) return c1_wgrad_ws_bytes(cout);
  return mfma_wgrad_supported(cin, cout) ? mfma_wgrad_ws_bytes(n, h, wd, cin, cout) : 0;
}

int32_t unet_conv3x3_bwd_weights(unet_ctx* ctx, const float* x, const float* dy, float* dw, float* db, void* ws, size_t ws_bytes,
                                 int32_t n, int32_t h, int32_t wd, int32_t cin, int32_t cout, int32_t algo, void* stream) {
  if (!ctx || !x || !dy || !dw || !db || n < 1 || h < 1 || wd < 1 || cin < 1 || cout < 1) UNET_FAIL(ctx, UNET_E_ARG, "conv3x3_bwd_weights: bad args");
  return conv3x3_wgrad_dispatch(ctx, x, dy, dw, db, ws, ws_bytes, n, h, wd, cin, cout, algo, as_stream(stream));
}

int32_t unet_convT2x2_fwd(unet_ctx* ctx, const float* x, const float* w, const float* bias, float* y, int32_t ldy, int32_t n,
                          int32_t h, int32_t wd, int32_t cin, int32_t cout, int32_t algo, void* stream) {
  if (!ctx || !x || !w || !y || ldy < cout || n < 1 || h < 1 || wd < 1) UNET_FAIL(ctx, UNET_E_ARG, "convT_fwd: bad args");
  if (h2_convT_selected(ctx, algo, cin, cout)) return k_convT_h2_fwd(ctx, x, w, bias, y, ldy, n, h, wd, cin, cout, as_stream(stream));
  if (algo != UNET_ALGO_NAIVE && mfma_convT_supported(cin, cout)) return k_convT_mfma_fwd(ctx, x, w, bias, y, ldy, n, h, wd, cin, cout, as_stream(stream));
  return k_convT_naive_fwd(ctx, x, w, bias, y, ldy, n, h, wd, cin, cout, as_stream(stream));
}

int32_t unet_convT2x2_bwd_data(unet_ctx* ctx, const float* dy, int32_t lddy, const float* w, const float* relu_src, float* dx,
                               int32_t n, int32_t h, int32_t wd, int32_t cin, int32_t cout, int32_t algo, void* stream) {
  if (!ctx || !dy || !w || !dx || lddy < cout) UNET_FAIL(ctx, UNET_E_ARG, "convT_bwd_data: bad args");
  if (h2_convT_selected(ctx, algo, cin, cout)) return k_convT_h2_dgrad(ctx, dy, lddy, w, relu_src, dx, n, h, wd, cin, cout, as_stream(stream));
  if (algo != UNET_ALGO_NAIVE && mfma_convT_supported(cin, cout)) return k_convT_mfma_dgrad(ctx, dy, lddy, w, relu_src, dx, n, h, wd, cin, cout, as_stream(stream));
  return k_convT_naive_dgrad(ctx, dy, lddy, w, relu_src, dx, n, h, wd, cin, cout, as_stream(stream));
}

size_t unet_convT2x2_bwd_weights_ws_bytes(int32_t n, int32_t h, int32_t wd, int32_t cin, int32_t cout) {
  return std::max(mfma_convT_supported(cin, cout) ? mfma_convT_wgrad_ws_bytes(n, h, wd, cin, cout) : 0, h2_convT_wgrad_ws_bytes(n, h, wd, cin, cout));
}

int32_t unet_convT2x2_bwd_weights(unet_ctx* ctx, const float* x, const float* dy, int32_t lddy, float* dw, float* db, void* ws,
                                  size_t ws_bytes, int32_t n, int32_t h, int32_t wd, int32_t cin, int32_t cout, int32_t algo,
                                  void* stream) {
  if (!ctx || !x || !dy || !dw || !db || lddy < cout) UNET_FAIL(ctx, UNET_E_ARG, "convT_bwd_weights: bad args");
  const bool can = mfma_convT_supported(cin, cout) && ws && ws_bytes >= mfma_convT_wgrad_ws_bytes(n, h, wd, cin, cout);
  if (h2_convT_wgrad_selected(algo, cin, cout) && ws && ws_bytes >= h2_convT_wgrad_ws_bytes(n, h, wd, cin, cout))
// ... 14 lines not shown
  return k_conv3x3_c1_fwd_bf16(ctx, x, w, bias, y, n, h, wd, cout, act, drop_rate, drop_seed, as_stream(stream));
}
int32_t unet_conv3x3_bwd_data_bf16(unet_ctx* ctx, const unet_bf16* dy, const float* w, const unet_bf16* mask_src, int32_t mask_mode, float mask_rate,
                                   uint64_t mask_seed, unet_bf16* dx, void* w_ws, int32_t n, int32_t h, int32_t wd, int32_t cin, int32_t cout, void* stream) {
  if (!ctx || !dy || !w || !dx || !w_ws || n < 1 || h < 1 || wd < 1 || mask_mode < 0 || mask_mode > 3 || (mask_mode != MASK_NONE && !mask_src) || mask_rate < 0 || mask_rate >= 1)
    UNET_FAIL(ctx, UNET_E_ARG, "conv3x3_bwd_data_bf16: bad args");
  return k_conv3x3_bf16_fwd(ctx, dy, w, nullptr, mask_src, mask_mode, dx, n, h, wd, cout, cin, ACT_NONE, mask_rate, mask_seed, static_cast<unet_bf16*>(w_ws), 1, as_stream(stream));
}
size_t unet_conv3x3_bwd_weights_ws_bytes_bf16(int32_t n, int32_t h, int32_t wd, int32_t cin, int32_t cout) {
  if (cin == 1) return c1_wgrad_ws_bytes(cout);
  return bf16_wgrad_ws_bytes(n, h, wd, cin, cout);
}
int32_t unet_conv3x3_bwd_weights_bf16(unet_ctx* ctx, const unet_bf16* x, const unet_bf16* dy, float* dw, float* db, void* ws, size_t ws_bytes, int32_t n,
                                      int32_t h, int32_t wd, int32_t cin, int32_t cout, void* stream) {
  if (!ctx || !x || !dy || !dw || !db || n < 1 || h < 1 || wd < 1) UNET_FAIL(ctx, UNET_E_ARG, "conv3x3_bwd_weights_bf16: bad args");
  return k_conv3x3_bf16_wgrad(ctx, x, dy, dw, db, ws, ws_bytes, n, h, wd, cin, cout, as_stream(stream));
}
int32_t unet_conv3x3_first_bwd_weights_bf16(unet_ctx* ctx, const float* x, const unet_bf16* dy, float* dw, float* db, void* ws, size_t ws_bytes, int32_t n,
                                            int32_t h, int32_t wd, int32_t cout, void* stream) {
  if (!ctx || !x || !dy || !dw || !db || n < 1 || h < 1 || wd < 1) UNET_FAIL(ctx, UNET_E_ARG, "conv3x3_first_bwd_weights_bf16: bad args");
  return k_conv3x3_c1_wgrad_bf16(ctx, x, dy, dw, db, ws, ws_bytes, n, h, wd, cout, as_stream(stream));
}
int32_t unet_convT2x2_fwd_bf16(unet_ctx* ctx, const unet_bf16* x, const float* w, const float* bias, unet_bf16* y, int32_t ldy, int32_t n, int32_t h,
                               int32_t wd, int32_t cin, int32_t cout, void* w_ws, void* stream) {
  if (!ctx || !x || !w || !y || !w_ws || ldy < cout || (ldy & 7) || n < 1 || h < 1 || wd < 1) UNET_FAIL(ctx, UNET_E_ARG, "convT_fwd_bf16: bad args");
  return k_convT_bf16_fwd(ctx, x, w, bias, y, ldy, n, h, wd, cin, cout, static_cast<unet_bf16*>(w_ws), as_stream(stream));
}
int32_t unet_convT2x2_bwd_data_bf16(unet_ctx* ctx, const unet_bf16* dy, int32_t lddy, const float* w, const unet_bf16* relu_src, unet_bf16* dx, int32_t n,
                                    int32_t h, int32_t wd, int32_t cin, int32_t cout, void* w_ws, void* stream) {
  if (!ctx || !dy || !w || !dx || !w_ws || lddy < cout || (lddy & 7)) UNET_FAIL(ctx, UNET_E_ARG, "convT_bwd_data_bf16: bad args");
  return k_convT_bf16_dgrad(ctx, dy, lddy, w, relu_src, dx, n, h, wd, cin, cout, static_cast<unet_bf16*>(w_ws), as_stream(stream));
}
size_t unet_convT2x2_bwd_weights_ws_bytes_bf16(int32_t n, int32_t h, int32_t wd, int32_t cin, int32_t cout) { return bf16_convT_wgrad_ws_bytes(n, h, wd, cin, cout); }
int32_t unet_convT2x2_bwd_weights_bf16(unet_ctx* ctx, const unet_bf16* x, const unet_bf16* dy, int32_t lddy, float* dw, float* db, void* ws, size_t ws_bytes,
                                       int32_t n, int32_t h, int32_t wd, int32_t cin, int32_t cout, void* stream) {
  if (!ctx || !x || !dy || !dw || !db || lddy < cout || (lddy & 7)) UNET_FAIL(ctx, UNET_E_ARG, "convT_bwd_weights_bf16: bad args");
  return k_convT_bf16_wgrad(ctx, x, dy, lddy, dw, db, ws, ws_bytes, n, h, wd, cin, cout, as_stream(stream));
}

}

namespace {

struct Layer { std::string name; int kind; int cin, cout; };
struct TInfo { int is_state; int64_t off, count; };
struct Buf { size_t off = 0; int ld = 0, n = 0, h = 0, w = 0, c = 0; size_t chan_off = 0; int f32 = 0; };

struct Op {
  std::string name;
  std::function<int32_t(hipStream_t)> run;
  double flops = 0, bytes = 0, ms = 0;
  int64_t calls = 0;
};

}

struct unet_model {
  unet_ctx* ctx = nullptr;
  int arch = 0, in_ch = 1, N = 0, H = 0, W = 0, world = 1, algo = 0;
  int dt = UNET_DTYPE_F32;
  std::vector<Layer> layers;
  std::map<std::string, TInfo> tinfo;
  int64_t n_params = 0, n_state = 0;
  float *params = nullptr, *grads = nullptr, *adam_m = nullptr, *adam_v = nullptr, *state = nullptr;
  char* ws = nullptr; size_t ws_bytes = 0;
  const float *x = nullptr, *yt = nullptr; float* pout = nullptr; float* loss_out2 = nullptr;
  float drop_rate = 0.0f; uint64_t drop_seed = 0;
  float cw0 = 1.0f, cw1 = 1.0f;
  unet_loss_sel loss;
  size_t off_wmap = 0;
  bool weighted() const { return loss.kind == UNET_LOSS_WEIGHTED_BCE_DICE; }
  const float* wmap() const { return weighted() ? reinterpret_cast<const float*>(ws) + off_wmap : nullptr; }
  size_t off_dense_ws = 0, dense_ws_bytes = 0;
  std::map<std::string, Buf> act, grad;
  size_t ws_floats_infer = 0, ws_floats_train = 0;
  size_t off_bn_sums = 0, bn_sums_doubles = 0;
  size_t off_bn_bsums = 0;
  std::map<std::string, size_t> bn_sum_off, bn_bsum_off, bnp_off;
  size_t off_loss_sums = 0, off_loss_out = 0, off_wt = 0, off_wgrad_ws = 0; size_t wgrad_ws_bytes = 0;
  size_t off_first_tmp = 0;
  bool skip_raw = false; std::map<std::string, size_t> bn_comp_off; size_t off_tap_tmp = 0;
  std::set<std::string> pool_sums_fused;
  bool c9b_virtual = false;
  bool head_bwd_fused = false;
  size_t off_head_sums = 0; bool head_fused = false;
  std::map<std::string, size_t> sign_off;
  std::map<std::string, size_t> wprep_f, wprep_b;
  std::map<std::string, size_t> fold_off, fold_g_off, fold_c_off;
  std::map<std::string, std::pair<std::string, int>> folded_bn;
  std::map<std::string, size_t> skip_k1_off;
  std::vector<Op> prog[3];
  std::vector<unet_sync_point> sync[3];
  struct SyncRef { int after_op, kind; bool in_ws; size_t off_bytes; int64_t count; int use_op = -1; };
  std::vector<SyncRef> syncref[3];

  float* wsf(size_t off) const { return reinterpret_cast<float*>(ws) + off; }
  double* wsd(size_t off_floats) const { return reinterpret_cast<double*>(reinterpret_cast<float*>(ws) + off_floats); }
  float* P(const std::string& n) const { auto& t = tinfo.at(n); return (t.is_state ? state : params) + t.off; }
  float* G(const std::string& n) const { auto& t = tinfo.at(n); return grads + t.off; }
  const float* A(const std::string& n) const { auto& b = act.at(n); return wsf(b.off + b.chan_off); }
  float* Aw(const std::string& n) const { auto& b = act.at(n); return wsf(b.off + b.chan_off); }
  float* D(const std::string& n) const { auto& b = grad.at(n); return wsf(b.off + b.chan_off); }
  int elem_bytes(const Buf& b) const { return (dt && !b.f32) ? 2 : 4; }
  void* bufptr(const Buf& b) const { return ws + b.off * 4 + b.chan_off * elem_bytes(b); }
  void* Av(const std::string& n) const { return bufptr(act.at(n)); }
  void* Dv(const std::string& n) const { return bufptr(grad.at(n)); }
};

namespace {

const int ENC[4] = {32, 64, 128, 256};

void assign_param_offsets(unet_model* m) {
  int64_t po = 0, so = 0;
  for (auto& l : m->layers) {
    if (l.kind == 2) {
      m->tinfo[l.name + "/gamma"] = {0, po, l.cout}; po += l.cout;
      m->tinfo[l.name + "/beta"] = {0, po, l.cout}; po += l.cout;
      m->tinfo[l.name + "/mean"] = {1, so, l.cout}; so += l.cout;
      m->tinfo[l.name + "/var"] = {1, so, l.cout}; so += l.cout;
    } else {
      int64_t kn = (l.kind == 0 ? 9 : l.kind == 1 ? 4 : 1) * (int64_t)l.cin * l.cout;
      m->tinfo[l.name + "/kernel"] = {0, po, kn}; po += kn;
      m->tinfo[l.name + "/bias"] = {0, po, l.cout}; po += l.cout;
    }
  }
  m->n_params = po; m->n_state = so;
}

void build_layers(unet_model* m) {
  auto& L = m->layers;
  int cprev = m->in_ch;
  for (int k = 1; k <= 4; ++k) {
    int c = ENC[k - 1];
    L.push_back({"c" + std::to_string(k) + "a", 0, cprev, c});
    L.push_back({"c" + std::to_string(k) + "b", 0, c, c});
    L.push_back({"bn" + std::to_string(k), 2, c, c});
    cprev = c;
  }
  L.push_back({"c5a", 0, 256, 512});
  L.push_back({"c5b", 0, 512, 512});
  cprev = 512;
  const int dec[4] = {256, 128, 64, 32};
  for (int k = 6; k <= 9; ++k) {
    int c = dec[k - 6];
    L.push_back({"u" + std::to_string(k), 1, cprev, c});
    L.push_back({"bn" + std::to_string(k), 2, 2 * c, 2 * c});
    L.push_back({"c" + std::to_string(k) + "a", 0, 2 * c, c});
    L.push_back({"c" + std::to_string(k) + "b", 0, c, c});
    cprev = c;
  }
  L.push_back({"out", 3, 32, 1});
  assign_param_offsets(m);
}

struct Carver {
  size_t cur = 0; int dt = 0;
  size_t take(size_t floats) { size_t o = cur; cur += (floats + 63) & ~size_t(63); return o; }
};

Buf mk(Carver& cv, int n, int h, int w, int c) { Buf b; const size_t el = (size_t)n * h * w * c; b.off = cv.take(cv.dt ? (el + 1) / 2 : el); b.ld = c; b.n = n; b.h = h; b.w = w; b.c = c; return b; }
Buf slice(const Buf& b, int c0, int c) { Buf s = b; s.chan_off = c0; s.c = c; return s; }

void plan_scratch(unet_model* m, Carver& cv) {
  size_t nd = 0;
  for (auto& l : m->layers) if (l.kind == 2) { m->bn_sum_off[l.name] = nd; nd += 2 * (size_t)l.cout; }
// ... 378 lines not shown
        const Buf ob = m->act.at("c9b"); const double px = (double)ob.n * ob.h * ob.w;
        ADD_OP(F, "conv3x3_fwd_head:c9b", 2.0 * 9 * c * c * px + 2.0 * c * px, 4.0 * px * (c + (m->c9b_virtual ? 0 : c)) + 4.0 * 9.0 * c * c + 8.0 * px + (training ? px * c / 8.0 : 0.0), {
          if (!m->pout) UNET_FAIL(ctx, UNET_E_STATE, "head_fwd: p_out not set (unet_model_set_io)");
          const auto so = training ? m->sign_off.find("c9b") : m->sign_off.end();
          unsigned long long* sg = so == m->sign_off.end() ? nullptr : reinterpret_cast<unsigned long long*>(m->wsf(so->second));
          ctx->signs_req = sg; ctx->signs_done = nullptr;
          int32_t r = k_conv3x3_h2_head_fwd(ctx, m->A("c9a"), m->wsf(m->wprep_f.at("c9b")), m->P("c9b/bias"), m->c9b_virtual ? nullptr : m->Aw("c9b"), m->P("out/kernel"), m->P("out/bias"),
                                            m->pout, m->yt, ob.n, ob.h, ob.w, c, s, m->yt ? m->wmap() : nullptr);
          ctx->signs_req = nullptr;
          if (!r && sg && ctx->signs_done != sg) UNET_FAIL(ctx, UNET_E_STATE, "conv3x3_fwd_head: the launch did not write the ReLU sign bits its backward was planned with");
          return r;
        });
      } else
      conv("c" + ks + "b", "c" + ks + "a", c, c);
      prev = "c" + ks + "b"; cprev = c;
    }
    const Buf hb = m->act.at("c9b");
    const int64_t hp = (int64_t)hb.n * hb.h * hb.w;
    if (m->head_fused) ADD_OP(F, "head_fold", 0, 0, {
      if (!m->yt) return UNET_OK;
      return k_head_fold(ctx, m->wsd(m->off_loss_sums), m->wsd(m->off_head_sums), s, m->weighted());
    });
    else
    ADD_OP(F, "head_fwd", 2.0 * 32 * hp, hp * (eb * 32 + 8.0), {
      if (!m->pout) UNET_FAIL(ctx, UNET_E_STATE, "head_fwd: p_out not set (unet_model_set_io)");
      if (dt) return unet_head_fwd_bf16_ex(ctx, CBF(m->Av("c9b")), m->P("out/kernel"), m->P("out/bias"), m->pout, m->yt, m->yt ? m->wmap() : nullptr, m->yt ? m->wsd(m->off_loss_sums) : nullptr,
                                           hp, hb.c, s);
      return unet_head_fwd_ex(ctx, m->A("c9b"), m->P("out/kernel"), m->P("out/bias"), m->pout, m->yt, m->yt ? m->wmap() : nullptr, m->yt ? m->wsd(m->off_loss_sums) : nullptr, hp, hb.c, s);
    });
    SY.push_back({(int)F.size() - 1, 1, true, m->off_loss_sums * 4, m->weighted() ? 5 : 4});
    ADD_OP(F, "loss_finalize", 0, 0, {
      if (!m->yt) return UNET_OK;
      return k_loss_finalize(ctx, m->wsd(m->off_loss_sums), (double)hp * gcount, m->wsf(m->off_loss_out), m->loss_out2, s, m->loss);
    });
  }

  {
    auto& SY = m->syncref[UNET_PROG_BWD];
    size_t nb = 0;
    for (auto& kv : m->bn_bsum_off) nb = std::max(nb, kv.second);
    size_t bs_bytes = 0;
    for (auto& l : m->layers) if (l.kind == 2) bs_bytes += 2 * (size_t)l.cout * sizeof(double);
    ADD_OP(BW, "zero_bwd_sums", 0, 0, {
      int32_t r = unet_zero(ctx, m->wsf(m->off_bn_bsums), bs_bytes, s);
      if (r) return r;
      return unet_zero(ctx, m->G("out/kernel"), (size_t)(m->tinfo.at("out/kernel").count + 1) * sizeof(float), s);
    });
    const Buf hb = m->act.at("c9b");
    const int64_t hp = (int64_t)hb.n * hb.h * hb.w;
    if (!dt) ADD_OP(BW, "weight_images:bwd", 0, 0, { return prep_weights(1, s); });
    else ADD_OP(BW, "weight_images:bwd", 0, 0, { return prep_weights_bf16(1, s); });
    m->head_bwd_fused = m->head_fused && ctx->opt_head_bwd_fused && m->arch == UNET_ARCH_UNET && m->sign_off.count("c9b") && m->wprep_b.count("c9b") && h2_head_bwd_selected(ctx, algo, hb.w, 32) &&
                        h2_wgrad_selected(algo, 32, 32);
    if (m->head_bwd_fused) ADD_OP(BW, "head_dzm", 8.0 * hp, hp * (8.0 + 4.0 + 8.0), {
      if (!m->yt || !m->pout) UNET_FAIL(ctx, UNET_E_STATE, "head_dzm: io not set");
      return k_head_dzm(ctx, m->pout, m->yt, m->wsd(m->off_loss_sums), (double)hp * gcount, m->wsd(m->off_head_sums), reinterpret_cast<const unsigned long long*>(m->wsf(m->sign_off.at("c9b"))),
                        m->D("c9b"), m->G("out/kernel"), m->G("out/bias"), hb.n, hb.h, hb.w, s, m->loss, m->wmap());
    });
    else
    if (m->head_fused) ADD_OP(BW, "head_dy", 2.0 * 32 * hp, hp * (4.0 * 32 + 8.0 + 4.0), {
      if (!m->yt || !m->pout) UNET_FAIL(ctx, UNET_E_STATE, "head_dy: io not set");
      const auto so = m->sign_off.find("c9b");
      return k_head_dy(ctx, m->pout, m->yt, m->wsd(m->off_loss_sums), (double)hp * gcount, m->wsd(m->off_head_sums), m->P("out/kernel"),
                       so == m->sign_off.end() ? nullptr : reinterpret_cast<const unsigned long long*>(m->wsf(so->second)), m->A("c9b"), m->D("c9b"),
                       m->G("out/kernel"), m->G("out/bias"), hb.n, hb.h, hb.w, s, m->loss, m->wmap());
    });
    else
    ADD_OP(BW, "head_bwd", 4.0 * 32 * hp, hp * (eb * 64 + 8.0), {
      if (!m->yt || !m->pout) UNET_FAIL(ctx, UNET_E_STATE, "head_bwd: io not set");
      const unet_loss_sel& L = m->loss;
      if (dt) return unet_head_bwd_bf16_ex(ctx, CBF(m->Av("c9b")), m->P("out/kernel"), m->pout, m->yt, m->wsd(m->off_loss_sums), (double)hp * gcount, L.kind, L.alpha, L.beta, m->wmap(), WBF(m->Dv("c9b")),
                                        m->G("out/kernel"), m->G("out/bias"), hp, hb.c, 1, s);
      return unet_head_bwd_ex(ctx, m->A("c9b"), m->P("out/kernel"), m->pout, m->yt, m->wsd(m->off_loss_sums), (double)hp * gcount, L.kind, L.alpha, L.beta, m->wmap(), m->D("c9b"),
                           m->G("out/kernel"), m->G("out/bias"), hp, hb.c, 1, s);
    });
    std::vector<Op> DEF;
    auto flush_def = [&]() { for (auto& o : DEF) BW.push_back(std::move(o)); DEF.clear(); };
    auto conv_bwd = [&](const std::string& name, const std::string& in, int cin, int cout, bool want_dx, bool mask_in, const std::string& xraw = "", bool defer_wgrad = false) {
      const Buf ob = m->act.at(name);
      const double px = (double)ob.n * ob.h * ob.w;
      const std::string xsrc = xraw.empty() ? in : xraw;
      auto& WV = (defer_wgrad && xraw.empty()) ? DEF : BW;
      const bool hstream = name == "c9b" && m->head_bwd_fused;
      ADD_OP(WV, "conv3x3_wgrad:" + name, 2.0 * 9 * cin * cout * px, (hstream ? eb * px * cin + 8.0 * px : eb * px * (cin + cout)) + 4.0 * 9.0 * cin * cout, {
        if (dt) {
          if (in.empty()) return first_conv_wgrad_bf16(ctx, m, name, ob, cout, s);
          return k_conv3x3_bf16_wgrad(ctx, CBF(m->Av(xsrc)), CBF(m->Dv(name)), m->G(name + "/kernel"), m->G(name + "/bias"), m->wsf(m->off_wgrad_ws), m->wgrad_ws_bytes, ob.n, ob.h, ob.w,
                                      cin, cout, s);
        }
        const float* xin = xsrc.empty() ? m->x : m->A(xsrc);
        if (name == "c9b" && m->head_bwd_fused)
          return k_conv3x3_h2_wgrad_dzm(ctx, xin, m->D(name), m->P("out/kernel"), m->G(name + "/kernel"), m->G(name + "/bias"), m->wsf(m->off_wgrad_ws), m->wgrad_ws_bytes, ob.n, ob.h, ob.w, cin, s);
        return conv3x3_wgrad_dispatch(ctx, xin, m->D(name), m->G(name + "/kernel"), m->G(name + "/bias"), m->wsf(m->off_wgrad_ws), m->wgrad_ws_bytes,
                                      ob.n, ob.h, ob.w, cin, cout, algo, s);
      });
      if (!xraw.empty()) {
        const size_t go = m->fold_g_off.at(name), bo = m->bnp_off.at(in);
        const bool pg = !dt && m->fold_c_off.count(name) != 0;
        ADD_OP(BW, "wgrad_bn_fold_fix:" + name, 2.0 * 9 * cin * cout, 8.0 * 9 * cin * cout, {
          if (dt) return k_wgrad_bn_fold_fix_bf16(ctx, CBF(m->Dv(name)), ob.n, ob.h, ob.w, cin, cout, m->wsf(bo), m->wsf(bo) + cin, m->G(name + "/kernel"), m->G(name + "/bias"), m->wsf(go), s,
                                                  m->P(name + "/kernel"), m->wsf(bo) + 2 * cin, m->wsf(bo) + 3 * cin, m->wsd(m->off_bn_bsums) + m->bn_bsum_off.at(in));
          if (m->skip_raw) {
            const float* comp = m->wsf(m->bn_comp_off.at(in));
            return k_wgrad_bn_fold_fix(ctx, m->D(name), ob.n, ob.h, ob.w, cin, cout, comp, comp + cin, m->G(name + "/kernel"), m->G(name + "/bias"), m->wsf(go), s,
                                       m->P(name + "/kernel"), m->wsf(bo) + 2 * cin, m->wsf(bo) + 3 * cin, m->wsd(m->off_bn_bsums) + m->bn_bsum_off.at(in), comp + 2 * cin, comp + 3 * cin,
                                       pg ? m->G(in + "/gamma") : nullptr, pg ? m->G(in + "/beta") : nullptr);
          }
          return k_wgrad_bn_fold_fix(ctx, m->D(name), ob.n, ob.h, ob.w, cin, cout, m->wsf(bo), m->wsf(bo) + cin, m->G(name + "/kernel"), m->G(name + "/bias"), m->wsf(go), s,
                                     m->P(name + "/kernel"), m->wsf(bo) + 2 * cin, m->wsf(bo) + 3 * cin, m->wsd(m->off_bn_bsums) + m->bn_bsum_off.at(in), nullptr, nullptr,
                                     pg ? m->G(in + "/gamma") : nullptr, pg ? m->G(in + "/beta") : nullptr);
        });
      }
      if (!xraw.empty() && m->fold_c_off.count(name)) {
        const std::string bnn = in;
        const size_t so = m->bn_bsum_off.at(bnn), bo = m->bnp_off.at(bnn), co = m->fold_c_off.at(name);
        ADD_OP(BW, "bn_bwd_param_grads:" + bnn, 0, 0, {
          if (!dt) return UNET_OK;
          return unet_bn_bwd_param_grads(ctx, m->wsd(m->off_bn_bsums) + so, m->G(bnn + "/gamma"), m->G(bnn + "/beta"), cin, s);
        });
        SY.push_back({(int)BW.size() - 1, 2, true, m->off_bn_bsums * 4 + so * 8, 2 * (int64_t)cin});
        const size_t syi = SY.size() - 1;
        flush_def();
        SY[syi].use_op = (int)BW.size();
        ADD_OP(BW, "conv3x3_dgrad_bn_bwd:" + name, 2.0 * 9 * cin * cout * px, eb * px * (cout + 2 * cin) + 4.0 * 9.0 * cin * cout, {
          int32_t r = k_bn_bwd_coef(ctx, m->wsf(bo), m->wsd(m->off_bn_bsums) + so, px * gcount, m->wsf(co), cin, s);
          if (r) return r;
          if (dt) return k_conv3x3_bf16_fwd(ctx, CBF(m->Dv(name)), m->P(name + "/kernel"), m->wsf(co), CBF(m->Av(xraw)), MASK_BN_BWD, WBF(m->Dv(xraw)), ob.n, ob.h, ob.w, cout, cin, ACT_NONE, 0.0f, 0,
                                            WBF(static_cast<void*>(m->wsf(m->off_wt))), 1, s, CBF(static_cast<void*>(m->wsf(m->wprep_b.at(name)))));
          const int climit = m->skip_k1_off.count("bn" + std::to_string(10 - (name[1] - '0'))) ? cin / 2 : (1 << 30);
          return k_conv3x3_h2_fwd(ctx, m->D(name), m->wsf(m->wprep_b.at(name)), m->wsf(co), m->A(xraw), MASK_BN_BWD, m->D(xraw), ob.n, ob.h, ob.w, cout, cin, ACT_NONE, 0.0f, 0, s, climit);
        });
        return;
      }
      if (want_dx && !dt && !mask_in && in.size() == 2 && in[0] == 'p' && ctx->opt_enc_bn_fused && m->wprep_b.count(name) && h2_pool_sums_selected(ctx, algo, ob.w, cout, cin)) {
        const std::string bnn = "bn" + in.substr(1);
        const size_t so = m->bn_bsum_off.at(bnn);
        m->pool_sums_fused.insert(in);
        ADD_OP(BW, "conv3x3_dgrad_pool_sums:" + name, 2.0 * 9 * cin * cout * px, eb * px * (cout + 2 * cin) + 4.0 * 9.0 * cin * cout, {
          (void)so;
          return k_conv3x3_h2_dgrad_pool_sums(ctx, m->D(name), m->wsf(m->wprep_b.at(name)), m->A(in), m->P(bnn + "/gamma"), m->P(bnn + "/beta"), m->drop_rate, m->D(in),
                                              nullptr, ob.n, ob.h, ob.w, cout, cin, s);
        });
      } else
      if (want_dx) {
        const bool bits = mask_in && m->sign_off.count(in) != 0;
        ADD_OP(BW, "conv3x3_dgrad:" + name, 2.0 * 9 * cin * cout * px, (hstream ? 8.0 * px + eb * px * (cin + (mask_in ? (bits ? cin / 32.0 : cin) : 0)) : eb * px * (cout + cin + (mask_in ? (bits ? cin / 32.0 : cin) : 0))) + 4.0 * 9.0 * cin * cout, {
          if (dt) return k_conv3x3_bf16_fwd(ctx, CBF(m->Dv(name)), m->P(name + "/kernel"), nullptr, mask_in ? CBF(m->Av(in)) : nullptr, mask_in ? MASK_RELU : MASK_NONE, WBF(m->Dv(in)), ob.n, ob.h,
                                            ob.w, cout, cin, ACT_NONE, 0.0f, 0, WBF(static_cast<void*>(m->wsf(m->off_wt))), 1, s, CBF(static_cast<void*>(m->wsf(m->wprep_b.at(name)))));
          const auto pb = m->wprep_b.find(name);
          const auto so = mask_in ? m->sign_off.find(in) : m->sign_off.end();
          if (name == "c9b" && m->head_bwd_fused)
            return k_conv3x3_h2_dgrad_dzm(ctx, m->D(name), m->wsf(pb->second), so != m->sign_off.end() ? m->wsf(so->second) : mask_in ? m->A(in) : nullptr,
                                          so != m->sign_off.end() ? MASK_RELU_BITS : mask_in ? MASK_RELU : MASK_NONE, m->D(in), ob.n, ob.h, ob.w, cin, s);
          if (so != m->sign_off.end())
            return conv3x3_fwd_dispatch(ctx, m->D(name), m->P(name + "/kernel"), nullptr, m->wsf(so->second), MASK_RELU_BITS, m->D(in), ob.n, ob.h,
                                        ob.w, cout, cin, ACT_NONE, 0.0f, 0, algo, s, m->wsf(m->off_wt), 1, pb == m->wprep_b.end() ? nullptr : m->wsf(pb->second));
          return conv3x3_fwd_dispatch(ctx, m->D(name), m->P(name + "/kernel"), nullptr, mask_in ? m->A(in) : nullptr, mask_in ? MASK_RELU : MASK_NONE, m->D(in), ob.n, ob.h,
                                      ob.w, cout, cin, ACT_NONE, 0.0f, 0, algo, s, m->wsf(m->off_wt), 1, pb == m->wprep_b.end() ? nullptr : m->wsf(pb->second));
        });
      }
    };
    auto bn_bwd = [&](const std::string& name, const std::string& dyname, const std::string& xname, const std::string& dxname, int c, int mask,
                      bool stats_done) {
      const Buf gb = m->grad.at(dyname), xb = m->act.at(xname), db = m->grad.at(dxname);
      const int64_t pixels = (int64_t)xb.n * xb.h * xb.w;
      const size_t so = m->bn_bsum_off.at(name), bo = m->bnp_off.at(name);
      if (stats_done) {
        ADD_OP(BW, "bn_bwd_param_grads:" + name, 0, 0, {
          return unet_bn_bwd_param_grads(ctx, m->wsd(m->off_bn_bsums) + so, m->G(name + "/gamma"), m->G(name + "/beta"), c, s);
        });
      } else {
        ADD_OP(BW, "bn_bwd_stats:" + name, 0, 2 * eb * pixels * c, {
          int32_t r = dt ? unet_bn_bwd_stats_bf16(ctx, CBF(m->Dv(dyname)), gb.ld, CBF(m->Av(xname)), xb.ld, m->wsf(bo), m->wsd(m->off_bn_bsums) + so, pixels, c, s)
                         : unet_bn_bwd_stats(ctx, m->D(dyname), gb.ld, m->A(xname), xb.ld, m->wsf(bo), m->wsd(m->off_bn_bsums) + so, pixels, c, s);
          if (r) return r;
          return unet_bn_bwd_param_grads(ctx, m->wsd(m->off_bn_bsums) + so, m->G(name + "/gamma"), m->G(name + "/beta"), c, s);
        });
      }
      SY.push_back({(int)BW.size() - 1, 2, true, m->off_bn_bsums * 4 + so * 8, 2 * (int64_t)c});
      ADD_OP(BW, "bn_bwd_apply:" + name, 0, 3 * eb * pixels * c, {
        if (dt) return unet_bn_bwd_apply_bf16(ctx, CBF(m->Dv(dyname)), gb.ld, CBF(m->Av(xname)), xb.ld, m->wsf(bo), m->wsd(m->off_bn_bsums) + so, (double)pixels * gcount,
                                              mask ? MASK_RELU : MASK_NONE, 0.0f, 0, WBF(m->Dv(dxname)), db.ld, pixels, c, s);
        return unet_bn_bwd_apply(ctx, m->D(dyname), gb.ld, m->A(xname), xb.ld, m->wsf(bo), m->wsd(m->off_bn_bsums) + so, (double)pixels * gcount, mask ? MASK_RELU : MASK_NONE, 0.0f, 0,
                                 m->D(dxname), db.ld, pixels, c, s);
      });
    };
    auto bucket = [&](const std::string& first, const std::string& last_tensor) {
      const TInfo a = m->tinfo.at(first), b = m->tinfo.at(last_tensor);
      SY.push_back({(int)BW.size() - 1, 3, false, (size_t)a.off * 4, b.off + b.count - a.off});
    };
    bool enc_split = false;
    const int dec[4] = {256, 128, 64, 32};
    for (int k = 9; k >= 6; --k) {
      int c = dec[k - 6]; std::string ks = std::to_string(k);
      std::string prev = (k == 6) ? "c5b" : "c" + std::to_string(k - 1) + "b";
      int cprev = (k == 6) ? 512 : dec[k - 7];
      conv_bwd("c" + ks + "b", "c" + ks + "a", c, c, true, true, "", m->fold_c_off.count("c" + ks + "a") != 0);
      conv_bwd("c" + ks + "a", "bn" + ks, 2 * c, c, true, false, m->fold_off.count("c" + ks + "a") ? "cat" + ks : "");
      flush_def();
      if (!m->fold_c_off.count("c" + ks + "a")) bn_bwd("bn" + ks, "bn" + ks, "cat" + ks, "cat" + ks, 2 * c, 0, m->fold_off.count("c" + ks + "a") != 0);
      const Buf ib = m->act.at(prev), ug = m->grad.at("u" + ks);
      const std::string un = "u" + ks;
      ADD_OP(BW, "convT_wgrad:" + un, 2.0 * 4 * cprev * c * nel(ib) / ib.c, eb * (nel(ib) + nel(ug)), {
        if (dt) return k_convT_bf16_wgrad(ctx, CBF(m->Av(prev)), CBF(m->Dv(un)), ug.ld, m->G(un + "/kernel"), m->G(un + "/bias"), m->wsf(m->off_wgrad_ws), m->wgrad_ws_bytes, ib.n, ib.h,
                                          ib.w, cprev, c, s);
        return unet_convT2x2_bwd_weights(ctx, m->A(prev), m->D(un), ug.ld, m->G(un + "/kernel"), m->G(un + "/bias"), m->wsf(m->off_wgrad_ws), m->wgrad_ws_bytes,
                                         ib.n, ib.h, ib.w, cprev, c, algo, s);
      });
      ADD_OP(BW, "convT_dgrad:" + un, 2.0 * 4 * cprev * c * nel(ib) / ib.c, eb * (2 * nel(ib) + nel(ug)), {
        if (dt) return k_convT_bf16_dgrad(ctx, CBF(m->Dv(un)), ug.ld, m->P(un + "/kernel"), CBF(m->Av(prev)), WBF(m->Dv(prev)), ib.n, ib.h, ib.w, cprev, c, WBF(static_cast<void*>(m->wsf(m->off_wt))), s);
        const auto so = m->sign_off.find(prev);
        const auto pb = m->wprep_b.find(un);
        const void* img = pb == m->wprep_b.end() ? nullptr : m->wsf(pb->second);
        if (so != m->sign_off.end()) return k_convT_h2_dgrad(ctx, m->D(un), ug.ld, m->P(un + "/kernel"), m->wsf(so->second), m->D(prev), ib.n, ib.h, ib.w, cprev, c, s, 1, img);
        if (img) return k_convT_h2_dgrad(ctx, m->D(un), ug.ld, m->P(un + "/kernel"), m->A(prev), m->D(prev), ib.n, ib.h, ib.w, cprev, c, s, 0, img);
        return unet_convT2x2_bwd_data(ctx, m->D(un), ug.ld, m->P(un + "/kernel"), m->A(prev), m->D(prev), ib.n, ib.h, ib.w, cprev, c, algo, s);
      });
      if (k == 7) bucket("u7/kernel", "out/bias");
      if (k == 6) bucket("u6/kernel", "c6b/bias");
    }
    conv_bwd("c5b", "c5a", 512, 512, true, true);
    conv_bwd("c5a", "p4", 256, 512, true, false, "", ctx->opt_enc_bn_fused != 0);
    if (!ctx->opt_enc_bn_fused) bucket("c5a/kernel", "c5b/bias");
    for (int k = 4; k >= 1; --k) {
      int c = ENC[k - 1]; std::string ks = std::to_string(k);
      const Buf xb = m->act.at("bn" + ks), gb = m->grad.at("bn" + ks);
      const std::string bnn = "bn" + ks, pn = "p" + ks;
      const size_t so = m->bn_bsum_off.at(bnn);
      if (ctx->opt_enc_bn_fused) {
        const std::string dn = "bn" + std::to_string(10 - k), cb = "c" + ks + "b";
        const size_t sod = m->bn_bsum_off.at(dn), bod = m->bnp_off.at(dn), bo = m->bnp_off.at(bnn);
        const Buf cbuf = m->act.at(cb), cg = m->grad.at(cb);
        const int64_t pixels = (int64_t)xb.n * xb.h * xb.w;
        const bool sums_done = m->pool_sums_fused.count(pn) != 0;
        ADD_OP(BW, sums_done ? "pool_bwd_skip_term:" + pn : "pool_bwd_sums:" + pn, 0, sums_done ? 0.0 : eb * 0.5 * nel(xb), {
          int32_t r = sums_done ? UNET_OK : dt ? unet_maxpool2x2_dropout_bwd_sums_bf16(ctx, CBF(m->Av(pn)), CBF(m->Dv(pn)), m->P(bnn + "/gamma"), m->P(bnn + "/beta"), m->wsd(m->off_bn_bsums) + so, xb.n, xb.h,
                                                                 xb.w, xb.c, m->drop_rate, m->drop_seed + (uint64_t)k * 0x9E3779B97F4A7C15ull, s)
                         : unet_maxpool2x2_dropout_bwd_sums(ctx, m->A(pn), m->D(pn), m->P(bnn + "/gamma"), m->P(bnn + "/beta"), m->wsd(m->off_bn_bsums) + so, xb.n, xb.h, xb.w, xb.c,
                                                            m->drop_rate, m->drop_seed + (uint64_t)k * 0x9E3779B97F4A7C15ull, s);
          if (r) return r;
          if (sums_done)
            return k_enc_tail_finish(ctx, m->wsd(m->off_bn_bsums) + so, m->wsd(m->off_bn_bsums) + sod + 3 * (size_t)c, m->wsf(bod) + 7 * (size_t)c, m->P(dn + "/gamma") + c,
                                     m->P(bnn + "/gamma"), m->G(bnn + "/gamma"), m->G(bnn + "/beta"), c, 1.0 / gcount, s);
          r = unet_bn_bwd_skip_term(ctx, m->wsd(m->off_bn_bsums) + so, m->wsd(m->off_bn_bsums) + sod + 3 * (size_t)c, m->wsf(bod) + 7 * (size_t)c, m->P(dn + "/gamma") + c,
                                    m->P(bnn + "/gamma"), c, 1.0 / gcount, s);
          if (r) return r;
          return unet_bn_bwd_param_grads(ctx, m->wsd(m->off_bn_bsums) + so, m->G(bnn + "/gamma"), m->G(bnn + "/beta"), c, s);
        });
        SY.push_back({(int)BW.size() - 1, 2, true, m->off_bn_bsums * 4 + so * 8, 2 * (int64_t)c});
        const size_t syi = SY.size() - 1;
        flush_def();
        if (k == 4) bucket("c5a/kernel", "c5b/bias");
        if (k == 2) { bucket("c3a/kernel", "bn4/beta"); enc_split = true; }
        SY[syi].use_op = (int)BW.size();
        ADD_OP(BW, "bn_pool_bwd_apply:" + bnn, 0, eb * 3.25 * nel(xb), {
          if (dt) return unet_bn_maxpool_bwd_apply_bf16(ctx, CBF(m->Av(cb)), cbuf.ld, m->wsf(bo), m->wsd(m->off_bn_bsums) + so, (double)pixels * gcount, CBF(m->Dv(bnn)), gb.ld, CBF(m->Dv(pn)),
                                                        WBF(m->Dv(cb)), cg.ld, xb.n, xb.h, xb.w, xb.c, m->drop_rate, m->drop_seed + (uint64_t)k * 0x9E3779B97F4A7C15ull, s);
          const auto k1o = m->skip_k1_off.find(bnn);
          return k_bn_maxpool_bwd_apply_k1(ctx, m->A(cb), cbuf.ld, m->wsf(bo), m->wsd(m->off_bn_bsums) + so, (double)pixels * gcount, m->D(bnn), gb.ld,
                                           k1o == m->skip_k1_off.end() ? nullptr : m->wsf(k1o->second), m->D(pn), m->D(cb), cg.ld,
                                           xb.n, xb.h, xb.w, xb.c, m->drop_rate, m->drop_seed + (uint64_t)k * 0x9E3779B97F4A7C15ull, s);
        });
      } else {
      ADD_OP(BW, "pool_bwd_bnstats:" + pn, 0, eb * 3.25 * nel(xb), {
        if (dt) return unet_maxpool2x2_dropout_bwd_bnstats_bf16(ctx, CBF(m->Av(bnn)), xb.ld, CBF(m->Dv(pn)), WBF(m->Dv(bnn)), gb.ld, m->P(bnn + "/gamma"), m->P(bnn + "/beta"),
                                                                m->wsd(m->off_bn_bsums) + so, xb.n, xb.h, xb.w, xb.c, m->drop_rate,
                                                                m->drop_seed + (uint64_t)k * 0x9E3779B97F4A7C15ull, s);
        return unet_maxpool2x2_dropout_bwd_bnstats(ctx, m->A(bnn), xb.ld, m->D(pn), m->D(bnn), gb.ld, m->P(bnn + "/gamma"), m->P(bnn + "/beta"),
                                                   m->wsd(m->off_bn_bsums) + so, xb.n, xb.h, xb.w, xb.c, m->drop_rate,
                                                   m->drop_seed + (uint64_t)k * 0x9E3779B97F4A7C15ull, s);
      });
      bn_bwd(bnn, bnn, "c" + ks + "b", "c" + ks + "b", c, 1, true);
      }
      conv_bwd("c" + ks + "b", "c" + ks + "a", c, c, true, true);
      int cprev = (k == 1) ? m->in_ch : ENC[k - 2];
      conv_bwd("c" + ks + "a", k == 1 ? "" : "p" + std::to_string(k - 1), cprev, c, k > 1, false, "", k > 1 && ctx->opt_enc_bn_fused != 0);
    }
    flush_def();
    bucket("c1a/kernel", enc_split ? "bn2/beta" : "bn4/beta");
  }
#undef CBF
#undef WBF
}

struct PPNode { const char* name; int c; const char* src; std::vector<const char*> skips; };
const std::vector<PPNode>& pp_nodes() {
  static const std::vector<PPNode> v = {{"x1_2", 32, "c2", {"c1"}}, {"x2_2", 64, "c3", {"c2"}}, {"x1_3", 32, "x2_2", {"c1", "x1_2"}},
                                        {"x3_2", 128, "c4", {"c3"}}, {"x2_3", 64, "x3_2", {"c2", "x2_2"}},
                                        {"x1_4", 32, "x2_3", {"c1", "x1_2", "x1_3"}}};
  return v;
}
int pp_width(const std::string& t) {
  if (t[0] == 'c') return ENC[t[1] - '1'];
  for (auto& n : pp_nodes()) if (t == n.name) return n.c;
  return 0;
}
int pp_level(const std::string& t) { return t[1] - '1'; }
constexpr float PP_ENC_DROP = 0.2f, PP_BLOCK_DROP = 0.4f;
const char* PP_ORDER[10] = {"e1", "e2", "x1_2", "e3", "x2_2", "x1_3", "e4", "x3_2", "x2_3", "x1_4"};

void build_layers_pp(unet_model* m) {
  auto& L = m->layers;
  for (const char* item : PP_ORDER) {
    std::string it = item;
    if (it[0] == 'e') {
      int k = it[1] - '0', c = ENC[k - 1], cin = k == 1 ? m->in_ch : ENC[k - 2];
      std::string ks = std::to_string(k);
      L.push_back({"c" + ks + "a", 0, cin, c}); L.push_back({"c" + ks + "b", 0, c, c}); L.push_back({"bn" + ks, 2, c, c});
    } else {
      const PPNode* nd = nullptr;
      for (auto& n : pp_nodes()) if (it == n.name) nd = &n;
      int ctot = nd->c; for (auto sk : nd->skips) ctot += pp_width(sk);
      L.push_back({"u" + it.substr(1), 1, pp_width(nd->src), nd->c});
      L.push_back({it + "a", 0, ctot, nd->c}); L.push_back({it + "abn", 2, nd->c, nd->c});
      L.push_back({it + "b", 0, nd->c, nd->c}); L.push_back({it + "bbn", 2, nd->c, nd->c});
    }
  }
  L.push_back({"out", 3, 32, 1});
  assign_param_offsets(m);
}

void plan_workspace_pp(unet_model* m) {
  Carver cv; cv.dt = m->dt;
  const int N = m->N;
  plan_scratch(m, cv);
  auto dims = [&](int lvl, int& hh, int& ww) { hh = m->H >> lvl; ww = m->W >> lvl; };
  int hh, ww;
  size_t wt0 = 0, wgb = 0, tmp_up = 0;
  for (int k = 1; k <= 4; ++k) {
    dims(k - 1, hh, ww); std::string ks = std::to_string(k); int c = ENC[k - 1];
    m->act["c" + ks + "a"] = mk(cv, N, hh, ww, c); m->act["c" + ks + "b"] = mk(cv, N, hh, ww, c);
    m->act["c" + ks] = mk(cv, N, hh, ww, c); m->act["bn" + ks] = m->act["c" + ks];
    if (k <= 3) m->act["p" + ks] = mk(cv, N, hh / 2, ww / 2, c);
  }
  for (auto& nd : pp_nodes()) {
    std::string nm = nd.name; dims(pp_level(nm), hh, ww);
    int ctot = nd.c; for (auto sk : nd.skips) ctot += pp_width(sk);
    Buf cat = mk(cv, N, hh, ww, ctot);
    m->act["cat_" + nm] = cat; m->act["u" + nm.substr(1)] = slice(cat, 0, nd.c);
    m->act[nm + "a"] = mk(cv, N, hh, ww, nd.c); m->act[nm + "abn"] = mk(cv, N, hh, ww, nd.c);
    m->act[nm + "b"] = mk(cv, N, hh, ww, nd.c); m->act[nm] = mk(cv, N, hh, ww, nd.c); m->act[nm + "bbn"] = m->act[nm];
  }
  for (auto& l : m->layers) if (l.kind == 0) wt0 = std::max(wt0, unet_conv3x3_w_ws_floats(l.cin, l.cout));
  m->off_wt = cv.take(wt0);
  if (m->ctx->opt_bn_fold >= 2) {
    for (auto& nd : pp_nodes()) {
      const std::string nm = nd.name; const int c = nd.c;
      if (!wgrad_bn_fold_supported(c)) continue;
      if (m->dt) { if (!bf16_conv3x3_supported(c, c)) continue; }
      else if (!h2_conv3x3_selected(m->algo, c, c) || (c % 32)) continue;
      m->fold_off[nm + "b"] = cv.take(bn_fold_scratch_floats(c, c));
      m->folded_bn[nm + "abn"] = {nm + "a", c};
    }
  }
  m->ws_floats_infer = cv.cur;
  for (auto& kv : m->fold_off) { const int c = m->act.at(kv.first).c; m->fold_g_off[kv.first] = cv.take(wgrad_bn_fold_scratch_floats(N, c)); m->fold_c_off[kv.first] = cv.take((size_t)3 * c); }
  std::map<size_t, std::string> seen;
  for (auto& kv : m->act) {
// ... 746 lines not shown
  if (!unet_loss_sel_ok(sel, nullptr, false) || (m->arch == UNET_ARCH_CLASSIFIER && loss != UNET_LOSS_BCE))
    UNET_FAIL(m->ctx, UNET_E_ARG, "model_set_loss: loss %d (alpha %g, beta %g) is not one of this graph's", loss, alpha, beta);
  if (m->arch == UNET_ARCH_CLASSIFIER) return UNET_OK;
  if ((loss == UNET_LOSS_WEIGHTED_BCE_DICE) == m->weighted()) { m->loss = sel; return UNET_OK; }
  unet_model* t = new unet_model();
  t->ctx = m->ctx; t->arch = m->arch; t->in_ch = m->in_ch; t->N = m->N; t->H = m->H; t->W = m->W; t->world = m->world; t->algo = m->algo; t->dt = m->dt; t->loss = sel;
  build_model(t);
  const size_t need = (m->grads ? t->ws_floats_train : t->ws_floats_infer) * sizeof(float);
  delete t;
  if (m->ws && m->ws_bytes < need)
    UNET_FAIL(m->ctx, UNET_E_STATE, "model_set_loss: the bound workspace (%zu bytes) is too small for loss %d (%zu bytes): bind a larger one first", m->ws_bytes, loss, need);
  unet_model keep = std::move(*m);
  *m = unet_model();
  m->ctx = keep.ctx; m->arch = keep.arch; m->in_ch = keep.in_ch; m->N = keep.N; m->H = keep.H; m->W = keep.W; m->world = keep.world; m->algo = keep.algo; m->dt = keep.dt;
  m->loss = sel;
  build_model(m);
  m->params = keep.params; m->grads = keep.grads; m->adam_m = keep.adam_m; m->adam_v = keep.adam_v; m->state = keep.state; m->ws = keep.ws; m->ws_bytes = keep.ws_bytes;
  m->x = keep.x; m->yt = keep.yt; m->pout = keep.pout; m->loss_out2 = keep.loss_out2; m->drop_rate = keep.drop_rate; m->drop_seed = keep.drop_seed;
  m->cw0 = keep.cw0; m->cw1 = keep.cw1;
  if (m->ws) resolve_sync(m);
  return UNET_OK;
}

int32_t unet_model_num_ops(const unet_model* m, int32_t prog) { return (!m || prog < 0 || prog > 2) ? UNET_E_ARG : (int32_t)m->prog[prog].size(); }

int32_t unet_model_sync_points(const unet_model* m, int32_t prog, unet_sync_point* out, int32_t cap) {
  if (!m || prog < 0 || prog > 2) return UNET_E_ARG;
  int n = (int)m->sync[prog].size();
  if (out) for (int i = 0; i < n && i < cap; ++i) out[i] = m->sync[prog][i];
  return n;
}

int32_t unet_model_run(unet_model* m, int32_t prog, int32_t begin, int32_t end, void* stream) {
  if (!m || prog < 0 || prog > 2) return UNET_E_ARG;
  unet_ctx* ctx = m->ctx;
  auto& P = m->prog[prog];
  if (begin < 0 || end > (int)P.size() || begin > end) UNET_FAIL(ctx, UNET_E_ARG, "model_run: bad op range [%d,%d) of %zu", begin, end, P.size());
  if (!m->ws || !m->params) UNET_FAIL(ctx, UNET_E_STATE, "model_run: buffers not bound");
  if (prog == UNET_PROG_BWD && !m->grads) UNET_FAIL(ctx, UNET_E_STATE, "model_run: backward needs a grads buffer");
  if (!m->x) UNET_FAIL(ctx, UNET_E_STATE, "model_run: input not set");
  hipStream_t s = as_stream(stream);
  hipEvent_t e0 = nullptr, e1 = nullptr;
  if (ctx->profiling) { UNET_HIP(ctx, hipEventCreate(&e0)); UNET_HIP(ctx, hipEventCreate(&e1)); }
  if (begin == 0 && prog != UNET_PROG_BWD) { ctx->stats_req_c = 0; ctx->stats_in_slots = nullptr; ctx->stats_in_slots_c = 0; ctx->signs_req = nullptr; ctx->k_slices_ok = 0; }
  for (int i = begin; i < end; ++i) {
    if (ctx->profiling) UNET_HIP(ctx, hipEventRecord(e0, s));
    const int32_t r = P[i].run(s);
    if (r) { ctx->err = P[i].name + ": " + ctx->err; if (ctx->profiling) { (void)hipEventDestroy(e0); (void)hipEventDestroy(e1); } return r; }
    if (ctx->profiling) {
      UNET_HIP(ctx, hipEventRecord(e1, s));
      UNET_HIP(ctx, hipEventSynchronize(e1));
      float ms = 0; UNET_HIP(ctx, hipEventElapsedTime(&ms, e0, e1));
      P[i].ms += ms; P[i].calls += 1;
    }
  }
  if (ctx->profiling) { (void)hipEventDestroy(e0); (void)hipEventDestroy(e1); }
  return UNET_OK;
}

const float* unet_model_loss_ptr(const unet_model* m) { return (m && m->ws) ? m->wsf(m->off_loss_out) : nullptr; }

int32_t unet_model_tap(const unet_model* m, const char* name, int32_t grad, const void** ptr, int32_t* ld, int32_t* n, int32_t* h,
                       int32_t* w, int32_t* c) {
  if (!m || !name || !m->ws) return UNET_E_ARG;
  auto& mp = grad ? m->grad : m->act;
  auto it = mp.find(name);
  if (it == mp.end()) return UNET_E_ARG;
  const Buf& b = it->second;
  const auto fb = m->folded_bn.find(name);
  if (grad && fb != m->folded_bn.end()) {
    const std::string nm = name;
    std::string conv = nm.rfind("bn", 0) == 0 ? "c" + nm.substr(2) + "a" : nm.substr(0, nm.size() - 3) + "b";
    if (m->arch == UNET_ARCH_CLASSIFIER) conv = "c" + nm.substr(2, 1) + "b";
    if (m->fold_c_off.count(conv)) return UNET_E_STATE;
  }
  const std::string nm_ = name;
  if (!grad && m->c9b_virtual && nm_ == "c9b") {
    const Buf& xb = m->act.at("c9a");
    int32_t r = k_conv3x3_h2_fwd(m->ctx, m->A("c9a"), m->wsf(m->wprep_f.at("c9b")), m->P("c9b/bias"), nullptr, MASK_NONE, const_cast<float*>(m->A("c9b")), xb.n, xb.h, xb.w, xb.c, b.c, ACT_RELU,
                                 0.0f, 0, nullptr);
    if (r) return r;
    if (hipStreamSynchronize(nullptr) != hipSuccess) return UNET_E_HIP;
  }
  if (grad && m->head_bwd_fused && nm_ == "c9b") return UNET_E_STATE;
  if (!grad && m->skip_raw && nm_.size() == 3 && nm_[0] == 'b' && nm_[2] >= '1' && nm_[2] <= '4') {
    const std::string cb = std::string("c") + nm_[2] + "b";
    const Buf& xb = m->act.at(cb);
    int32_t r = unet_bn_apply(m->ctx, m->A(cb), xb.ld, m->wsf(m->bnp_off.at(name)), const_cast<float*>(m->A(name)), b.ld, (int64_t)b.n * b.h * b.w, b.c, nullptr);
    if (r) return r;
    if (hipStreamSynchronize(nullptr) != hipSuccess) return UNET_E_HIP;
  }
  if (!grad && fb != m->folded_bn.end()) {
    const Buf& xb = m->act.at(fb->second.first);
    const float* bnp_ = m->skip_raw && m->bn_comp_off.count(name) ? m->wsf(m->bn_comp_off.at(name)) : m->wsf(m->bnp_off.at(name));
    int32_t r = m->dt ? unet_bn_apply_bf16(m->ctx, static_cast<const unet_bf16*>(m->Av(fb->second.first)), xb.ld, m->wsf(m->bnp_off.at(name)), static_cast<unet_bf16*>(m->Av(name)), b.ld,
                                           (int64_t)b.n * b.h * b.w, fb->second.second, nullptr)
                      : unet_bn_apply(m->ctx, m->A(fb->second.first), xb.ld, bnp_, const_cast<float*>(m->A(name)), b.ld, (int64_t)b.n * b.h * b.w, fb->second.second, nullptr);
    if (r) return r;
    if (hipStreamSynchronize(nullptr) != hipSuccess) return UNET_E_HIP;
  }
  if (ptr) *ptr = m->bufptr(b);
  if (ld) *ld = b.ld; if (n) *n = b.n; if (h) *h = b.h; if (w) *w = b.w; if (c) *c = b.c;
  return UNET_OK;
}

int32_t unet_model_tap_elem_bytes(const unet_model* m, const char* name, int32_t grad) {
  if (!m || !name) return UNET_E_ARG;
  auto& mp = grad ? m->grad : m->act;
  auto it = mp.find(name);
  return it == mp.end() ? UNET_E_ARG : m->elem_bytes(it->second);
}

int32_t unet_model_op_info(const unet_model* m, int32_t prog, int32_t op, const char** name, double* flops, double* bytes, double* ms,
                           int64_t* calls) {
  if (!m || prog < 0 || prog > 2 || op < 0 || op >= (int)m->prog[prog].size()) return UNET_E_ARG;
  const Op& o = m->prog[prog][op];
  if (name) *name = o.name.c_str();
  if (flops) *flops = o.flops; if (bytes) *bytes = o.bytes; if (ms) *ms = o.ms; if (calls) *calls = o.calls;
  return UNET_OK;
}

int32_t unet_model_reset_timers(unet_model* m) {
  if (!m) return UNET_E_ARG;
  for (auto& P : m->prog) for (auto& o : P) { o.ms = 0; o.calls = 0; }
  return UNET_OK;
}

}
```

Measured before the change: 1042 images/sec.

## Fuse first-layer weight gradient into c1b data-gradient persistent conv kernel

The c1b data-gradient persistent kernel now also computes the c1a weight and bias gradients. It loads the single-channel input image halo into LDS and accumulates the outer products with small fp32 MFMAs in the epilogue slots. The separate c1a wgrad pass, which re-read the full-resolution 32-channel dy, is skipped, and a shared reduction helper produces the final dw/db. In exchange the kernel needs more LDS and registers, does extra epilogue work, and the gradient buffer for c1a is only produced on demand for inspection.

```diff
diff --git a/include/unet_hip.h b/include/unet_hip.h
--- a/include/unet_hip.h
+++ b/include/unet_hip.h
@@ -24,7 +24,7 @@
 const char* unet_last_error(const unet_ctx* ctx);
 int32_t unet_ctx_set_profiling(unet_ctx* ctx, int32_t on);
 enum { UNET_OPT_RELU_BITS = 1, UNET_OPT_BN_FOLD = 2, UNET_OPT_ENC_BN_FUSED = 3, UNET_OPT_BN_CONCAT_ANALYTIC = 4, UNET_OPT_BN_FUSE_STATS = 5, UNET_OPT_DETERMINISTIC = 6,
-       UNET_OPT_HEAD_FUSED = 7, UNET_OPT_SKIP_RAW = 8, UNET_OPT_POOL_SUMS_FUSED = 9, UNET_OPT_HEAD_BWD_FUSED = 10, UNET_OPT_CONV_PP = 13 };
+       UNET_OPT_HEAD_FUSED = 7, UNET_OPT_SKIP_RAW = 8, UNET_OPT_POOL_SUMS_FUSED = 9, UNET_OPT_HEAD_BWD_FUSED = 10, UNET_OPT_CONV_PP = 13, UNET_OPT_C1_WGRAD_FUSED = 14 };
 int32_t unet_ctx_set_option(unet_ctx* ctx, int32_t option, int32_t value);
 int32_t unet_ctx_get_option(unet_ctx* ctx, int32_t option);
 
@@ -141,6 +141,10 @@
 int32_t unet_conv3x3_bwd_data_pool_sums_supported(unet_ctx*, int32_t algo, int32_t wd, int32_t cin, int32_t cout);
 int32_t unet_conv3x3_bwd_data_pool_sums(unet_ctx*, const float* dy, const float* w, const float* pooled, const float* gamma, const float* beta, float rate,
                                         float* dx, double* sums, float* wt_ws, int32_t n, int32_t h, int32_t wd, int32_t cin, int32_t cout, void* stream);
+
+size_t unet_conv3x3_bwd_data_c1wgrad_ws_bytes(void);
+int32_t unet_conv3x3_bwd_data_c1wgrad(unet_ctx*, const float* dy, const float* w, const void* relu_bits, const float* x_image, float* dw1, float* db1, void* ws, size_t ws_bytes,
+                                      int32_t n, int32_t h, int32_t wd, void* stream);
 
 int32_t unet_conv3x3_head_supported(unet_ctx*, int32_t algo, int32_t w, int32_t cin, int32_t cout);
 int32_t unet_conv3x3_head_fwd(unet_ctx*, const float* x, const float* w, const float* bias, float* y, const float* w_head, const float* b_head, float* p,
diff --git a/one-stop-for-covid-19-infection-and-lung-segmentation-plus-classification_amd/_lib.py b/one-stop-for-covid-19-infection-and-lung-segmentation-plus-classification_amd/_lib.py
--- a/one-stop-for-covid-19-infection-and-lung-segmentation-plus-classification_amd/_lib.py
+++ b/one-stop-for-covid-19-infection-and-lung-segmentation-plus-classification_amd/_lib.py
@@ -9,7 +9,7 @@
 COMM_HANDLE_BYTES, COMM_MAX_WORLD, COMM_MAX_DOUBLES = 64, 8, 2048
 
 ALGO_AUTO, ALGO_NAIVE, ALGO_MFMA = 0, 1, 2
-OPTIONS = {"relu_bits": 1, "bn_fold": 2, "enc_bn_fused": 3, "bn_concat_analytic": 4, "bn_fuse_stats": 5, "deterministic": 6, "head_fused": 7, "skip_raw": 8, "pool_sums_fused": 9, "head_bwd_fused": 10, "conv_pp": 13}
+OPTIONS = {"relu_bits": 1, "bn_fold": 2, "enc_bn_fused": 3, "bn_concat_analytic": 4, "bn_fuse_stats": 5, "deterministic": 6, "head_fused": 7, "skip_raw": 8, "pool_sums_fused": 9, "head_bwd_fused": 10, "conv_pp": 13, "c1_wgrad_fused": 14}
 ARCH_UNET, ARCH_UNETPP, ARCH_CLASSIFIER = 0, 1, 2
 LOSSES = {"bce_dice_loss": 0, "binary_crossentropy": 1, "dice_loss": 2, "tversky_loss": 3, "weighted_bce_dice_loss": 4}
 DTYPE_F32, DTYPE_BF16 = 0, 1
@@ -144,6 +144,8 @@
     "unet_head_dzm": (i32, [vp, vp, vp, vp, f64, vp, vp, vp, vp, vp, i32, i32, i32, vp]),
     "unet_head_dy_ex": (i32, [vp, vp, vp, vp, f64, vp, i32, f32, f32, vp, vp, vp, vp, vp, vp, vp, i32, i32, i32, vp]),
     "unet_head_dzm_ex": (i32, [vp, vp, vp, vp, f64, vp, i32, f32, f32, vp, vp, vp, vp, vp, i32, i32, i32, vp]),
+    "unet_conv3x3_bwd_data_c1wgrad_ws_bytes": (sz, []),
+    "unet_conv3x3_bwd_data_c1wgrad": (i32, [vp, vp, vp, vp, vp, vp, vp, vp, sz, i32, i32, i32, vp]),
     "unet_conv3x3_bwd_data_dzm": (i32, [vp, vp, vp, vp, vp, vp, vp, i32, i32, i32, i32, vp]),
     "unet_conv3x3_bwd_weights_dzm": (i32, [vp, vp, vp, vp, vp, vp, vp, sz, i32, i32, i32, i32, vp]),
     "unet_zero": (i32, [vp, vp, sz, vp]),
diff --git a/one-stop-for-covid-19-infection-and-lung-segmentation-plus-classification_amd/csrc/common.h b/one-stop-for-covid-19-infection-and-lung-segmentation-plus-classification_amd/csrc/common.h
--- a/one-stop-for-covid-19-infection-and-lung-segmentation-plus-classification_amd/csrc/common.h
+++ b/one-stop-for-covid-19-infection-and-lung-segmentation-plus-classification_amd/csrc/common.h
@@ -28,6 +28,7 @@
   int opt_skip_raw = 1;
   int opt_head_fused = 1;
   int opt_head_bwd_fused = 1;
+  int opt_c1_wgrad_fused = 1;
   int opt_conv_pp = 1;
   int opt_deterministic = 0;
   double* bn_slots = nullptr;
@@ -254,6 +255,9 @@
 bool pp_conv3x3_selected(const unet_ctx* ctx, int K, int M, int n, int h, int wd, const float* mask, int mask_mode, int act, float rate, int ldy);
 int32_t k_conv3x3_pp_fwd(unet_ctx*, const float* x, const void* wimg, const float* bias, const float* mask, int mask_mode, float* y, int ldy, int n, int h, int wd, int K, int M,
                          int act, hipStream_t s, bool vdy = false);
+bool pp_c1_wgrad_selected(const unet_ctx* ctx, int n, int h, int wd);
+int32_t k_conv3x3_pp_dgrad_c1_wgrad(unet_ctx*, const float* dy, const void* wimg, const float* relu_bits, const float* ximg, float* dw1, float* db1, void* ws, size_t ws_bytes,
+                                    int n, int h, int wd, hipStream_t s);
 size_t h2_wimg_bytes(int K, int M);
 int32_t k_h2_weights(unet_ctx*, const float* w, void* img, int cin, int cout, int flip, hipStream_t s, const float* cs = nullptr);
 int32_t k_h2_weights_multi(unet_ctx*, const float* const* w, void* const* img, const int* cin, const int* cout, const int* flip, int count, hipStream_t s);
@@ -307,6 +311,7 @@
 int32_t k_conv3x3_c1_fwd(unet_ctx*, const float* x, const float* w, const float* bias, float* y, int n, int h,
                          int wd, int cout, int act, float rate, uint64_t seed, hipStream_t s);
 size_t c1_wgrad_ws_bytes(int cout);
+int32_t k_reduce_c1(unet_ctx*, float* part, int blocks, int cout, float* dw, float* db, hipStream_t s);
 int32_t k_conv3x3_c1_wgrad(unet_ctx*, const float* x, const float* dy, float* dw, float* db, void* ws, size_t ws_bytes, int n, int h,
                            int wd, int cout, hipStream_t s);
 int32_t k_flip_transpose_w3x3(unet_ctx*, const float* w, float* wt, int cin, int cout, hipStream_t s);
diff --git a/one-stop-for-covid-19-infection-and-lung-segmentation-plus-classification_amd/csrc/kernels_conv_naive.hip b/one-stop-for-covid-19-infection-and-lung-segmentation-plus-classification_amd/csrc/kernels_conv_naive.hip
--- a/one-stop-for-covid-19-infection-and-lung-segmentation-plus-classification_amd/csrc/kernels_conv_naive.hip
+++ b/one-stop-for-covid-19-infection-and-lung-segmentation-plus-classification_amd/csrc/kernels_conv_naive.hip
@@ -435,6 +435,15 @@
 
 size_t c1_wgrad_ws_bytes(int cout) { return (size_t)(C1_BLOCKS + 32) * 10 * cout * sizeof(float); }
 
+int32_t k_reduce_c1(unet_ctx* ctx, float* part, int blocks, int cout, float* dw, float* db, hipStream_t s) {
+  if (blocks < 1 || blocks > C1_BLOCKS) UNET_FAIL(ctx, UNET_E_ARG, "reduce_c1: %d partials", blocks);
+  float* part2 = part + (size_t)C1_BLOCKS * 10 * cout;
+  const int ngroups = (blocks + 31) / 32;
+  hipLaunchKernelGGL(reduce_c1_kernel, dim3((10 * cout + 127) / 128, ngroups), dim3(128), 0, s, part, part2, nullptr, blocks, 32, cout, 0);
+  hipLaunchKernelGGL(reduce_c1_kernel, dim3((10 * cout + 127) / 128, 1), dim3(128), 0, s, part2, dw, db, ngroups, ngroups, cout, 1);
+  UNET_CHECK_LAUNCH(ctx, "conv3x3_c1_wgrad"); return UNET_OK;
+}
+
 template <typename T>
 static int32_t c1_wgrad_impl(unet_ctx* ctx, const float* x, const T* dy, float* dw, float* db, void* ws, size_t ws_bytes, int n, int h,
                            int wd, int cout, hipStream_t s) {
@@ -444,11 +453,7 @@
   int blocks = (int)std::min<long long>(C1_BLOCKS, std::max<long long>(groups, 1));
   if ((wd & 3) == 0) hipLaunchKernelGGL((conv3x3_c1_wgrad_kernel<T, true>), dim3(blocks), dim3(TPB), 0, s, x, dy, static_cast<float*>(ws), n, h, wd, cout);
   else hipLaunchKernelGGL((conv3x3_c1_wgrad_kernel<T, false>), dim3(blocks), dim3(TPB), 0, s, x, dy, static_cast<float*>(ws), n, h, wd, cout);
-  float* part = static_cast<float*>(ws); float* part2 = part + (size_t)C1_BLOCKS * 10 * cout;
-  const int ngroups = (blocks + 31) / 32;
-  hipLaunchKernelGGL(reduce_c1_kernel, dim3((10 * cout + 127) / 128, ngroups), dim3(128), 0, s, part, part2, nullptr, blocks, 32, cout, 0);
-  hipLaunchKernelGGL(reduce_c1_kernel, dim3((10 * cout + 127) / 128, 1), dim3(128), 0, s, part2, dw, db, ngroups, ngroups, cout, 1);
-  UNET_CHECK_LAUNCH(ctx, "conv3x3_c1_wgrad"); return UNET_OK;
+  return k_reduce_c1(ctx, static_cast<float*>(ws), blocks, cout, dw, db, s);
 }
 int32_t k_conv3x3_c1_wgrad(unet_ctx* ctx, const float* x, const float* dy, float* dw, float* db, void* ws, size_t ws_bytes, int n, int h, int wd, int cout,
                            hipStream_t s) { return c1_wgrad_impl(ctx, x, dy, dw, db, ws, ws_bytes, n, h, wd, cout, s); }
diff --git a/one-stop-for-covid-19-infection-and-lung-segmentation-plus-classification_amd/csrc/kernels_conv_pp.hip b/one-stop-for-covid-19-infection-and-lung-segmentation-plus-classification_amd/csrc/kernels_conv_pp.hip
--- a/one-stop-for-covid-19-infection-and-lung-segmentation-plus-classification_amd/csrc/kernels_conv_pp.hip
+++ b/one-stop-for-covid-19-infection-and-lung-segmentation-plus-classification_amd/csrc/kernels_conv_pp.hip
@@ -32,11 +32,12 @@
 __device__ __forceinline__ f16x8 pp_frag(const char* p) { return *reinterpret_cast<const f16x8*>(p); }
 __device__ __forceinline__ int pp_cell(int p, int c) { return p * 128 + ((c ^ (p & 7)) << 4); }
 
-template <int KC, bool BITS, bool VDY>
+template <int KC, bool BITS, bool VDY, bool C1W = false>
 __global__ __launch_bounds__(512, 2) void conv_pp_kernel(const float* __restrict__ x, const unet_bf16* __restrict__ wimg_hdr, const float* __restrict__ bias,
                                                          const float* __restrict__ mask, float* __restrict__ y, int ldy, int N, int H, int W, int act, int mask_mode,
                                                          int tiles_x, int tiles_y, int total_tiles, double* __restrict__ stats, int stats_c,
-                                                         unsigned long long* __restrict__ signs, int xs) {
+                                                         unsigned long long* __restrict__ signs, int xs, const float* __restrict__ ximg, float* __restrict__ part) {
+  static_assert(!C1W || (BITS && !VDY && KC == 2), "the first-layer rider: the one-bit-mask data gradient, one epilogue slice per step");
   constexpr int RW = 2, TH = 8, PWD = 34, NPIX = (TH + 2) * PWD, K = 16 * KC, M = 32;
   constexpr int HS = NPIX * 16;
   constexpr int PLANE = 2 * HS, CHUNK = 2 * PLANE + 32;
@@ -55,6 +56,8 @@
   float* const s_bias = reinterpret_cast<float*>(smem + W_ALL + 2 * IN_HALF + 4 * 4096) + 8;
   float* const s_stat = s_bias + 32;
   float* const s_tab = s_stat + 8 * 2 * 32;
+  constexpr int IMS = 40, IMG_W = 4 * IMS + 2 * 72;
+  float* const s_img = s_tab + 16 * 32 + wave8 * IMG_W;
 
   const int per = gridDim.x >> 3, xcd = blockIdx.x & 7, j = blockIdx.x >> 3;
   const int tpx = (total_tiles + 7) >> 3;
@@ -142,6 +145,17 @@
   const bool tab_mask = !BITS && mask_mode == MASK_BIAS_TAB;
   unsigned mpre[BITS ? RW : 1][4];
   const __amdgpu_buffer_rsrc_t rs_m = make_rsrc(mask, BITS ? (long long)N * H * (W >> 3) * 32 : 0);
+  unsigned ipre[C1W ? 3 : 1];
+  const __amdgpu_buffer_rsrc_t rs_i = make_rsrc(ximg - (W + 1), C1W ? ((long long)N * H * W + W + 1) * 4 : 0);
+  typedef float f32x4_t __attribute__((ext_vector_type(4)));
+  f32x4_t cacc[2] = {{0.f, 0.f, 0.f, 0.f}, {0.f, 0.f, 0.f, 0.f}};
+  float c1a_ = 0.f; f32x4_t c1b_ = {0.f, 0.f, 0.f, 0.f};
+  const int c1_boff = (lane >> 4) * 128 + ((((lane & 15) >> 1) ^ (lane >> 4)) << 4) + (lane & 1) * 8;
+  const int c1_tap = lane & 15;
+  const int c1_aoff = c1_tap < 9 ? (c1_tap / 3) * IMS + (c1_tap % 3) + (lane >> 4) : c1_tap == 9 ? 4 * IMS : 4 * IMS + 72;
+  if (C1W) {
+    for (int i = lane; i < 144; i += 64) s_img[4 * IMS + i] = i < 72 ? 1.f : 0.f;
+  }
   float4 t4s[4];
   int sg_lo = 0, sg_hi = 0;
 
@@ -154,6 +168,13 @@
 #pragma unroll
       for (int qq = 0; qq < 4; ++qq)
         *reinterpret_cast<float4*>(s_out + pp_cell(l31, hi * 4 + qq)) = make_float4(vprev[r][qq * 4], vprev[r][qq * 4 + 1], vprev[r][qq * 4 + 2], vprev[r][qq * 4 + 3]);
+      if (C1W) return;
+    } else if (C1W) {
+      if (px0 + (q - 1) * 4 < W) {
+        cacc[0] = __builtin_amdgcn_mfma_f32_16x16x4f32(c1a_, c1b_[0], cacc[0], 0, 0, 0);
+        cacc[1] = __builtin_amdgcn_mfma_f32_16x16x4f32(c1a_, c1b_[1], cacc[1], 0, 0, 0);
+      }
+      return;
     } else if (q == 1) {
 #pragma unroll
       for (int jj = 0; jj < 4; ++jj) t4s[jj] = *reinterpret_cast<const float4*>(s_out + pp_cell(jj * 8 + (lane >> 3), lane & 7));
@@ -187,6 +208,15 @@
     }
   };
 
+  auto epre = [&](const int sl) __attribute__((always_inline)) {
+    const int r = sl < 9 ? 0 : 1, q = sl - r * 9;
+    if (q == 0) return;
+    const int ks = q - 1;
+    const uint2 b2 = *reinterpret_cast<const uint2*>(s_out + (c1_boff ^ ((ks & 1) << 6)) + ks * 512);
+    c1b_[0] = __uint_as_float(b2.x); c1b_[1] = __uint_as_float(b2.y);
+    c1a_ = s_img[c1_aoff + r * IMS + ks * 4];
+  };
+
   auto mphase = [&](auto HC_, auto HP_, const int it) __attribute__((always_inline)) {
     constexpr bool HC = decltype(HC_)::value, HP = decltype(HP_)::value;
     f16x8 px[2][RW + 2], wf[2][2];
@@ -216,6 +246,7 @@
           if (ky1 == 0) { ld_row(ch1, kx1, 0); ld_row(ch1, kx1, 1); }
           else ld_row(ch1, kx1, ky1 + 1);
         }
+        if (C1W && HP) epre(s_);
 #pragma unroll
         for (int pr = 0; pr < 3; ++pr) {
           constexpr int PW[3] = {0, 1, 0}, PX[3] = {1, 0, 0};
@@ -223,6 +254,7 @@
           for (int r = 0; r < RW; ++r) acc[r] = __builtin_amdgcn_mfma_f32_32x32x16_f16(wf[s_ & 1][PW[pr]], px[PX[pr]][r + ky], acc[r], 0, 0, 0);
         }
       }
+      if (C1W && HP && !HC) epre(s_);
       if (HP) eslice(s_ * 18 / (9 * KC));
       __builtin_amdgcn_sched_barrier(0);
       if (s_ == PP_MID) {
@@ -296,6 +328,13 @@
     __builtin_amdgcn_s_barrier();
     PP_STAMP(2);
     if (BITS && have_prev) output_values();
+    if (C1W && have_prev) {
+#pragma unroll
+      for (int k = 0; k < 3; ++k) {
+        const int idx = lane + k * 64, row = idx / 34;
+        if (idx < 136) s_img[row * IMS + idx - row * 34] = __uint_as_float(ipre[k]);
+      }
+    }
     if (have_cur) {
       const float4 m4 = *reinterpret_cast<const float4*>(s_amax);
       const float mx = fmaxf(fmaxf(m4.x, m4.y), fmaxf(m4.z, m4.w));
@@ -330,6 +369,16 @@
         const int mo = ok ? (((p_cur.n * H + py) * (W >> 3) + (p_cur.x0 >> 3) + (l31 >> 3)) * 32 + ((l31 >> 2) & 1) * 4) : UNET_OOB;
 #pragma unroll
         for (int k = 0; k < 4; ++k) mpre[BITS ? r : 0][k] = __builtin_amdgcn_raw_buffer_load_b32(rs_m, mo, k * 8, 0);
+      }
+    }
+    if (C1W && have_cur) {
+      const int wy = p_cur.y0 + wave * RW;
+      const int soff = ((p_cur.n * H + wy) * W + p_cur.x0) * 4;
+#pragma unroll
+      for (int k = 0; k < 3; ++k) {
+        const int idx = lane + k * 64, row = idx / 34, col = idx - row * 34;
+        const bool ok = idx < 136 && (unsigned)(wy - 1 + row) < (unsigned)H && (unsigned)(p_cur.x0 - 1 + col) < (unsigned)W;
+        ipre[k] = __builtin_amdgcn_raw_buffer_load_b32(rs_i, ok ? (row * W + col) * 4 : UNET_OOB, soff, 0);
       }
     }
     __builtin_amdgcn_sched_barrier(0);
@@ -356,6 +405,25 @@
   for (int it = 0; it <= iters; ++it) body(it, pregA);
   if (!half) { __builtin_amdgcn_s_barrier(); __builtin_amdgcn_s_barrier(); }
 
+  if (C1W) {
+    __syncthreads();
+    float* const s_red = reinterpret_cast<float*>(smem);
+#pragma unroll
+    for (int v = 0; v < 2; ++v)
+#pragma unroll
+      for (int r = 0; r < 4; ++r) {
+        const int i = (lane >> 4) * 4 + r;
+        if (i < 10) s_red[(wave8 * 10 + i) * 32 + (lane & 15) * 2 + v] = cacc[v][r];
+      }
+    __syncthreads();
+    if (threadIdx.x < 320) {
+      float t = 0.f;
+#pragma unroll
+      for (int wv = 0; wv < 8; ++wv) t += s_red[wv * 320 + threadIdx.x];
+      part[(size_t)blockIdx.x * 320 + threadIdx.x] = t;
+    }
+  }
+
   if (stats) {
     float sv[8] = {st1.x, st1.y, st1.z, st1.w, st2.x, st2.y, st2.z, st2.w};
 #pragma unroll
@@ -421,7 +489,34 @@
   unet_note_kernel(ctx, reinterpret_cast<const void*>(kern));
   const unsigned grid = (unsigned)(ctx->num_cu & ~7);
   hipLaunchKernelGGL(kern, dim3(grid), dim3(512), smem, s, x, static_cast<const unet_bf16*>(wimg), bias, mask, y, ldy, n, h, wd, act, mask_mode, tiles_x, tiles_y, (int)total, stats,
-                     stats_c, signs, ctx->opt_deterministic ? 1 : 0);
+                     stats_c, signs, ctx->opt_deterministic ? 1 : 0, nullptr, nullptr);
   UNET_CHECK_LAUNCH(ctx, "conv_pp");
   return UNET_OK;
 }
+
+bool pp_c1_wgrad_selected(const unet_ctx* ctx, int n, int h, int wd) {
+  static const float some_mask = 0.f;
+  return pp_conv3x3_selected(ctx, 32, 32, n, h, wd, &some_mask, MASK_RELU_BITS, ACT_NONE, 0.0f, 32) && (ctx->num_cu & ~7) >= 8 && (ctx->num_cu & ~7) <= 1024;
+}
+
+int32_t k_conv3x3_pp_dgrad_c1_wgrad(unet_ctx* ctx, const float* dy, const void* wimg, const float* relu_bits, const float* ximg, float* dw1, float* db1, void* ws, size_t ws_bytes,
+                                    int n, int h, int wd, hipStream_t s) {
+  if (!dy || !wimg || !relu_bits || !ximg || !dw1 || !db1) UNET_FAIL(ctx, UNET_E_ARG, "conv pp + c1 wgrad: bad args");
+  if (!pp_c1_wgrad_selected(ctx, n, h, wd)) UNET_FAIL(ctx, UNET_E_SHAPE, "conv pp + c1 wgrad: the persistent schedule does not take n=%d h=%d w=%d", n, h, wd);
+  if (!ws || ws_bytes < c1_wgrad_ws_bytes(32)) UNET_FAIL(ctx, UNET_E_ARG, "conv pp + c1 wgrad: workspace too small");
+  constexpr int KC = 2;
+  ctx->k_slices_ok = 0;
+  ctx->stats_req_c = 0; ctx->signs_req = nullptr;
+  const int tiles_x = (wd + 31) / 32, tiles_y = (h + 7) / 8;
+  const long long total = (long long)tiles_x * tiles_y * n;
+  constexpr int NPIX = 340, CHUNK = 4 * NPIX * 16 + 32;
+  constexpr size_t smem = (size_t)KC * 9 * 2048 + 2 * (size_t)KC * CHUNK + 4 * 4096 + 32 + 128 + 8 * 2 * 32 * 4 + 16 * 32 * 4 + 8 * (4 * 40 + 2 * 72) * 4;
+  auto kern = conv_pp_kernel<KC, true, false, true>;
+  UNET_BIG_LDS(ctx, kern, smem, "conv_pp_c1w");
+  unet_note_kernel(ctx, reinterpret_cast<const void*>(kern));
+  const unsigned grid = (unsigned)(ctx->num_cu & ~7);
+  hipLaunchKernelGGL(kern, dim3(grid), dim3(512), smem, s, dy, static_cast<const unet_bf16*>(wimg), static_cast<const float*>(nullptr), relu_bits, static_cast<float*>(nullptr), 32, n, h, wd,
+                     (int)ACT_NONE, (int)MASK_RELU_BITS, tiles_x, tiles_y, (int)total, static_cast<double*>(nullptr), 0, static_cast<unsigned long long*>(nullptr), 0, ximg, static_cast<float*>(ws));
+  UNET_CHECK_LAUNCH(ctx, "conv_pp_c1w");
+  return k_reduce_c1(ctx, static_cast<float*>(ws), (int)grid, 32, dw1, db1, s);
+}
diff --git a/one-stop-for-covid-19-infection-and-lung-segmentation-plus-classification_amd/csrc/model.hip b/one-stop-for-covid-19-infection-and-lung-segmentation-plus-classification_amd/csrc/model.hip
--- a/one-stop-for-covid-19-infection-and-lung-segmentation-plus-classification_amd/csrc/model.hip
+++ b/one-stop-for-covid-19-infection-and-lung-segmentation-plus-classification_amd/csrc/model.hip
@@ -58,6 +58,7 @@
     case UNET_OPT_POOL_SUMS_FUSED: return &ctx->opt_pool_sums_fused;
     case UNET_OPT_HEAD_BWD_FUSED: return &ctx->opt_head_bwd_fused;
     case UNET_OPT_CONV_PP: return &ctx->opt_conv_pp;
+    case UNET_OPT_C1_WGRAD_FUSED: return &ctx->opt_c1_wgrad_fused;
     default: return nullptr;
   }
 }
@@ -274,6 +275,18 @@
                                          as_stream(stream), wt_ws, 1);
   ctx->k_slices_ok = 0;
   return r;
+}
+
+size_t unet_conv3x3_bwd_data_c1wgrad_ws_bytes(void) { return c1_wgrad_ws_bytes(32) + unet_conv3x3_w_ws_floats(32, 32) * sizeof(float); }
+int32_t unet_conv3x3_bwd_data_c1wgrad(unet_ctx* ctx, const float* dy, const float* w, const void* relu_bits, const float* x_image, float* dw1, float* db1, void* ws, size_t ws_bytes,
+                                      int32_t n, int32_t h, int32_t wd, void* stream) {
+  if (!ctx || !dy || !w || !relu_bits || !x_image || !dw1 || !db1 || !ws || n < 1 || h < 1 || wd < 1) UNET_FAIL(ctx, UNET_E_ARG, "conv3x3_bwd_data_c1wgrad: bad args");
+  if (ws_bytes < unet_conv3x3_bwd_data_c1wgrad_ws_bytes()) UNET_FAIL(ctx, UNET_E_ARG, "conv3x3_bwd_data_c1wgrad: workspace too small (unet_conv3x3_bwd_data_c1wgrad_ws_bytes)");
+  if (!pp_c1_wgrad_selected(ctx, n, h, wd)) UNET_FAIL(ctx, UNET_E_SHAPE, "conv3x3_bwd_data_c1wgrad: the persistent schedule does not take n=%d h=%d w=%d (UNET_OPT_CONV_PP)", n, h, wd);
+  float* img = reinterpret_cast<float*>(static_cast<char*>(ws) + c1_wgrad_ws_bytes(32));
+  int32_t r = k_h2_weights(ctx, w, img, 32, 32, 1, as_stream(stream));
+  if (r) return r;
+  return k_conv3x3_pp_dgrad_c1_wgrad(ctx, dy, img, static_cast<const float*>(relu_bits), x_image, dw1, db1, ws, c1_wgrad_ws_bytes(32), n, h, wd, as_stream(stream));
 }
 
 int32_t unet_conv3x3_bwd_data_pool_sums_supported(unet_ctx* ctx, int32_t algo, int32_t wd, int32_t cin, int32_t cout) { return ctx && h2_pool_sums_selected(ctx, algo, wd, cout, cin) ? 1 : 0; }
@@ -454,6 +467,7 @@
   bool skip_raw = false; std::map<std::string, size_t> bn_comp_off; size_t off_tap_tmp = 0;
   std::set<std::string> pool_sums_fused;
   bool c9b_virtual = false;
+  bool c1_wgrad_fused = false;
   bool head_bwd_fused = false;
   size_t off_head_sums = 0; bool head_fused = false;
   std::map<std::string, size_t> sign_off;
@@ -998,6 +1012,7 @@
       const std::string xsrc = xraw.empty() ? in : xraw;
       auto& WV = (defer_wgrad && xraw.empty()) ? DEF : BW;
       const bool hstream = name == "c9b" && m->head_bwd_fused;
+      const bool c1w = name == "c1b" && m->c1_wgrad_fused;
       ADD_OP(WV, "conv3x3_wgrad:" + name, 2.0 * 9 * cin * cout * px, (hstream ? eb * px * cin + 8.0 * px : eb * px * (cin + cout)) + 4.0 * 9.0 * cin * cout, {
         if (dt) {
           if (in.empty()) return first_conv_wgrad_bf16(ctx, m, name, ob, cout, s);
@@ -1056,6 +1071,12 @@
           (void)so;
           return k_conv3x3_h2_dgrad_pool_sums(ctx, m->D(name), m->wsf(m->wprep_b.at(name)), m->A(in), m->P(bnn + "/gamma"), m->P(bnn + "/beta"), m->drop_rate, m->D(in),
                                               nullptr, ob.n, ob.h, ob.w, cout, cin, s);
+        });
+      } else
+      if (want_dx && c1w) {
+        ADD_OP(BW, "conv3x3_dgrad:" + name, 2.0 * 9 * cin * cout * px, eb * px * (cout + cin / 32.0 + 1.0) + 4.0 * 9.0 * cin * cout, {
+          return k_conv3x3_pp_dgrad_c1_wgrad(ctx, m->D(name), m->wsf(m->wprep_b.at(name)), m->wsf(m->sign_off.at(in)), m->x, m->G(in + "/kernel"), m->G(in + "/bias"), m->wsf(m->off_wgrad_ws),
+                                             m->wgrad_ws_bytes, ob.n, ob.h, ob.w, s);
         });
       } else
       if (want_dx) {
@@ -1188,8 +1209,11 @@
       });
       bn_bwd(bnn, bnn, "c" + ks + "b", "c" + ks + "b", c, 1, true);
       }
+      if (k == 1) m->c1_wgrad_fused = !dt && ctx->opt_c1_wgrad_fused && m->arch == UNET_ARCH_UNET && m->in_ch == 1 && c == 32 && m->sign_off.count("c1a") && m->wprep_b.count("c1b") &&
+                                      h2_conv3x3_selected(algo, c, c) && pp_c1_wgrad_selected(ctx, m->N, m->H, m->W) && m->wgrad_ws_bytes >= c1_wgrad_ws_bytes(32);
       conv_bwd("c" + ks + "b", "c" + ks + "a", c, c, true, true);
       int cprev = (k == 1) ? m->in_ch : ENC[k - 2];
+      if (!(k == 1 && m->c1_wgrad_fused))
       conv_bwd("c" + ks + "a", k == 1 ? "" : "p" + std::to_string(k - 1), cprev, c, k > 1, false, "", k > 1 && ctx->opt_enc_bn_fused != 0);
     }
     flush_def();
@@ -2102,6 +2126,11 @@
     if (r) return r;
     if (hipStreamSynchronize(nullptr) != hipSuccess) return UNET_E_HIP;
   }
+  if (grad && m->c1_wgrad_fused && nm_ == "c1a") {
+    int32_t r = k_conv3x3_h2_fwd(m->ctx, m->D("c1b"), m->wsf(m->wprep_b.at("c1b")), nullptr, m->wsf(m->sign_off.at("c1a")), MASK_RELU_BITS, m->D("c1a"), b.n, b.h, b.w, 32, 32, ACT_NONE, 0.0f, 0, nullptr);
+    if (r) return r;
+    if (hipStreamSynchronize(nullptr) != hipSuccess) return UNET_E_HIP;
+  }
   if (grad && m->head_bwd_fused && nm_ == "c9b") return UNET_E_STATE;
   if (!grad && m->skip_raw && nm_.size() == 3 && nm_[0] == 'b' && nm_[2] >= '1' && nm_[2] <= '4') {
     const std::string cb = std::string("c") + nm_[2] + "b";
```

After: 1047 images/sec, median of 6. No clear change (+0.6%).
